# ai4colonoscopy/PraNet-V2

Hardware: AMD Instinct MI355X
Metric: images/sec (train fwd+bwd) at 352x352 bs=32/GPU (higher is better)
Workload: dtype bf16; 1 GPU; PraNet-V2 Res2Net50 training step (fwd+4x structure_loss+bwd+clamp+Adam), bs=32/GPU 352x352, random-init, synthetic ellipse masks; global_batch=32, parallelism=dp1, launch=hipGraph replay

## Files before the change

### include/pn2.h

```cpp
#ifndef PN2_H
#define PN2_H
#ifdef __cplusplus
extern "C" {
#endif

#define PN2_F32 0
#define PN2_BF16 1
#define PN2_F32F 2
#define PN2_F32X3 3
#define PN2_CONV_STATS 1
#define PN2_CONV_ACCUM 2
#define PN2_CONV_SPLITK(n) ((n) << 16)
#define PN2_CONV_ROWGATE 8
#define PN2_CONV_AFFINE 16
#define PN2_CONV_RELU 32
#define PN2_CONV_RELU6 64
#define PN2_CONV_BIAS 4

typedef struct pn2_conv_desc {
    int N, H, W;
    int OH, OW;
    int Cin_p, ld_in;
    int Cout, ld_out;
    int KH, KW, stride, pad_h, pad_w, dil_h, dil_w;
    int transposed;
    int Kp;
    int flags;
} pn2_conv_desc;

typedef struct pn2_wgrad_desc {
    int N, H, W, OH, OW;
    int Cin_p, ld_x;
    int Cout_p, ld_dy;
    int KH, KW, stride, pad_h, pad_w, dil_h, dil_w;
    int Rp, Kp;
    int tune;
} pn2_wgrad_desc;

typedef struct pn2_pack_desc {
    int Cout, Cin, KH, KW;
    int Cout_p, gw_out, gwp_out;
    int Cin_p, gw_in, gwp_in;
    int Rp, Kp;
    int transposed;
    int ld, koff;
} pn2_pack_desc;

int pn2_conv_tile_n(int cout);
int pn2_wgrad_tile_co(int cout_p);
int pn2_conv_tile_m(int m, int cout, int dtype);
int pn2_conv_stat_blocks(int m, int cout, int dtype);
int pn2_conv_gemm(int dtype, const void* in, const void* wp, void* out, float* psum, float* psq, const pn2_conv_desc* d, void* stream);
#define PN2_BNB_STATS 1
#define PN2_BNB_MASK_RAW 2
#define PN2_BNB_MASK_Y 4
#define PN2_BNB_STORE_MASKED 8
int pn2_conv_gemm_gated(int dtype, const void* in, const void* wp, void* out, float* psum, float* psq, const pn2_conv_desc* d, const float* gate, void* stream);
int pn2_conv_gemm_affine(int dtype, const void* in, const void* wp, void* out, const float* scale, const float* shift, const void* res, int ld_res,
                         const pn2_conv_desc* d, void* stream);
typedef struct pn2_bnb_target {
    void* out; int ld_out;
    int mode;
    const void* raw; int ld_raw;
    const void* y; int ld_y;
    const float* par; int ps;
    int split;
    const void* raw2; const float* par2;
    float* p1; float* p2; int ldp;
} pn2_bnb_target;
typedef struct pn2_conv_ep { pn2_bnb_target a, b; const void* pool; int ld_pool; int pad_; pn2_bnb_target c; } pn2_conv_ep;
int pn2_conv_gemm_ep(int dtype, const void* in, const void* wp, void* out, const pn2_conv_desc* d, const pn2_conv_ep* ep, void* stream);
typedef struct pn2_conv_job { const void* in; const void* wp; void* out; float* psum; float* psq; pn2_conv_desc d; int pad_; pn2_conv_ep ep; } pn2_conv_job;
int pn2_conv_gemm_tile(int dtype, const pn2_conv_desc* d);
int pn2_conv_gemm_job_blocks(int dtype, const pn2_conv_job* j, int bm, int bn);
int pn2_conv_gemm_multi(int dtype, int bm, int bn, int ep, const pn2_conv_job* jobs_dev, const int* block_start_dev, int njobs, int total_blocks, void* stream);
int pn2_conv_splitk_reduce(int dtype, const float* ws, int ksplit, int M, int Cout, void* out, int ld_out, const float* bias, float* psum, float* psq,
                           int accumulate, void* stream);
int pn2_conv_wgrad(int dtype, const void* dy, const void* x, float* slab, const pn2_wgrad_desc* d, int nsplit, void* stream);
typedef struct pn2_wgrad_job { const void* dy; const void* x; float* slab; pn2_wgrad_desc d; int nsplit;
    int rot;
} pn2_wgrad_job;
int pn2_conv_wgrad_variant(int dtype, const pn2_wgrad_desc* d);
int pn2_conv_wgrad_blocks(const pn2_wgrad_desc* d, int nsplit);
int pn2_conv_wgrad_multi(int dtype, int variant, const pn2_wgrad_job* jobs_dev, const int* block_start_dev, int njobs, int total_blocks, void* stream);
int pn2_pack_weight(int dtype, const float* w_oihw, void* wp, const pn2_pack_desc* p, void* stream);
int pn2_wgrad_reduce(const float* slab, float* gw_oihw, const pn2_pack_desc* p, int nsplit, int accumulate, void* stream);
int pn2_pack_patch_weight(int dtype, const float* w_oihw, void* wp, int Cout, int Cin, int KH, int KW, int Cin_p, int Rp, int Kp, void* stream);
int pn2_depth_to_space(int dtype, const void* t, int ld_t, void* dx, int ld_dx, int N, int H, int W, int OH, int OW, int S, int C, int accumulate, void* stream);
int pn2_conv_dgrad_small_cin(int dtype, const void* dy, int ld_dy, const float* w_oihw, void* dx, int ld_dx, int N, int H, int W, int OH, int OW,
                             int Cout, int Cin, int KH, int KW, int stride, int pad, int accumulate, void* stream);
typedef struct pn2_pack_job { const float* w; void* wp; pn2_pack_desc d; } pn2_pack_job;
int pn2_pack_blocks(const pn2_pack_desc* p);
int pn2_pack_weights_multi(int dtype, const pn2_pack_job* jobs_dev, const int* block_start_dev, int njobs, int total_blocks, void* stream);
typedef struct pn2_reduce_job { const float* slab; float* gw; pn2_pack_desc d; int nsplit; int accumulate; } pn2_reduce_job;
int pn2_wgrad_reduce_blocks(const pn2_pack_desc* p);
int pn2_wgrad_reduce_multi(const pn2_reduce_job* jobs_dev, const int* block_start_dev, int njobs, int total_blocks, void* stream);

typedef struct pn2_bn_desc {
    int M;
    int Cp;
    int C, gw, gwp;
    float eps, momentum;
    int ldp;
    int tile_rows;
} pn2_bn_desc;
int pn2_bn_finalize(const float* psum, const float* psq, int nblk, const pn2_bn_desc* d, const float* gamma, const float* beta,
                    float* running_mean, float* running_var, float* scale, float* shift, float* mean, float* invstd, void* stream);
int pn2_bn_eval_prepare(const pn2_bn_desc* d, const float* gamma, const float* beta, const float* running_mean, const float* running_var,
                        float* scale, float* shift, void* stream);
typedef struct pn2_bnprep_job { const float* gamma; const float* beta; const float* running_mean; const float* running_var; float* scale; float* shift; pn2_bn_desc d; int pad_; } pn2_bnprep_job;
int pn2_bn_eval_prepare_multi(const pn2_bnprep_job* jobs_dev, const int* block_start_dev, int njobs, int total_blocks, void* stream);
int pn2_affine_act(int dt_in, const void* x, int ld_x, int dt_out, void* y, int ld_y, int M, int Cout,
                   const float* scale, const float* shift, const void* res, int ld_res, int relu, void* stream);
int pn2_affine_act_sum(int dt, const void* x, int ld_x, void* y, int ld_y, int M, int C, const float* scale, const float* shift, int relu,
                       const void* add, int ld_add, void* y2, int ld_y2, void* stream);
int pn2_affine_act_tee(int dt, const void* x, int ld_x, void* y, int ld_y, int M, int C, const float* scale, const float* shift, int relu,
                       void* y3, int ld_y3, int c_lo, void* stream);
int pn2_bn_relu_maxpool_fwd(int dt, const void* raw, int ld_raw, const float* scale, const float* shift, void* y, int ld_y, unsigned char* idx,
                            int N, int H, int W, int C, int OH, int OW, void* stream);
int pn2_pool_bn_bwd_reduce(int dt, const void* dpool, int ld_dp, const unsigned char* idx, const void* raw, int ld_raw, int N, int H, int W, int C, int OH, int OW,
                           const float* mean, const float* invstd, const float* mask_scale, const float* mask_shift, float* p1, float* p2, int nblk, void* stream);
int pn2_pool_bn_bwd_apply(int dt, const void* dpool, int ld_dp, const unsigned char* idx, const void* raw, int ld_raw, int N, int H, int W, int C, int OH, int OW,
                          const float* mean, const float* invstd, const float* coef, const float* mask_scale, const float* mask_shift, void* dz, int ld_dz, void* stream);
int pn2_bn_bwd_reduce(int dt, int dt_dy, const void* dy, int ld_dy, int Cdy, const void* y, int ld_y, int dt_y, const void* x, int ld_x,
                      int M, int Cp, const float* mean, const float* invstd, float* p1, float* p2, int nblk,
                      const float* mask_scale, const float* mask_shift, int relu6, void* stream);
int pn2_bn_bwd_blocks(int M, int Cp, int dtype);
int pn2_bn_bwd_finalize(const float* p1, const float* p2, int nblk, const pn2_bn_desc* d, const float* gamma, const float* invstd,
                        float* dgamma, float* dbeta, int accumulate, float* coef, void* stream);
typedef struct pn2_bn_segs { int nseg; int c0[4]; int nblk[4]; int ldp[4]; const float* p1[4]; const float* p2[4]; } pn2_bn_segs;
int pn2_bn_bwd_finalize_seg(const pn2_bn_segs* segs, const pn2_bn_desc* d, const float* gamma, const float* invstd,
                            float* dgamma, float* dbeta, int accumulate, float* coef, void* stream);
typedef struct pn2_bnfin_job { const float* psum; const float* psq; const float* gamma; const float* beta; float* running_mean; float* running_var;
                               float* scale; float* shift; float* mean; float* invstd; pn2_bn_desc d; int nblk; int cpb; int pad_; } pn2_bnfin_job;
int pn2_bn_finalize_job_blocks(pn2_bnfin_job* j);
int pn2_bn_finalize_multi(const pn2_bnfin_job* jobs_dev, const int* block_start_dev, int njobs, int total_blocks, void* stream);
typedef struct pn2_affine_job { const void* x; void* y; const float* scale; const float* shift; const void* res; const void* add; void* y2;
                                int ld_x, ld_y, ld_res, ld_add, ld_y2, M, C, relu, rows_per_blk, cvp; } pn2_affine_job;
int pn2_affine_job_blocks(int dt, pn2_affine_job* j);
int pn2_affine_multi(int dt, const pn2_affine_job* jobs_dev, const int* block_start_dev, int njobs, int total_blocks, void* stream);
typedef struct pn2_bnbfin_job { pn2_bn_segs sg; const float* gamma; const float* invstd; float* dgamma; float* dbeta; float* coef; pn2_bn_desc d;
                                int accumulate; int cpb; int pad_; } pn2_bnbfin_job;
int pn2_bn_bwd_finalize_job_blocks(pn2_bnbfin_job* j);
int pn2_bn_bwd_finalize_multi(const pn2_bnbfin_job* jobs_dev, const int* block_start_dev, int njobs, int total_blocks, void* stream);
typedef struct pn2_bnapply_job { const void* dy; const void* y; const void* x; const float* mean; const float* invstd; const float* coef; void* dx; void* dres;
                                 const float* msc; const float* msh; int ld_dy, ld_y, ld_x, ld_dx, ld_dres, M, Cp, dres_accum, r6, rows_per_blk, cvp, pad_; } pn2_bnapply_job;
int pn2_bn_bwd_apply_job_blocks(int dt, pn2_bnapply_job* j);
#define PN2_MULTI_F32DY 0x200
#define PN2_MULTI_F32OUT 0x200
#define PN2_MULTI_LEAN 0x100
int pn2_bn_bwd_apply_multi(int dt, const pn2_bnapply_job* jobs_dev, const int* block_start_dev, int njobs, int total_blocks, void* stream);
typedef struct pn2_bnreduce_job { const void* dy; const void* y; const void* x; const float* mean; const float* invstd; float* p1; float* p2;
                                  const float* msc; const float* msh; int ld_dy, ld_y, ld_x, M, Cp, nblk, rows_per_blk, cvp, r6, pad_; } pn2_bnreduce_job;
int pn2_bn_bwd_reduce_job_blocks(int dt, pn2_bnreduce_job* j);
int pn2_bn_bwd_reduce_multi(int dt, const pn2_bnreduce_job* jobs_dev, const int* block_start_dev, int njobs, int total_blocks, void* stream);
int pn2_bn_bwd_apply(int dt, int dt_dy, const void* dy, int ld_dy, int Cdy, const void* y, int ld_y, int dt_y, const void* x, int ld_x,
                     int M, int Cp, const float* mean, const float* invstd, const float* coef, void* dx, int ld_dx,
                     void* dres, int ld_dres, int dres_accum, const float* mask_scale, const float* mask_shift, int relu6, void* stream);

int pn2_maxpool3x3s2_fwd(int dt, const void* x, int ld_x, void* y, int ld_y, unsigned char* idx, int N, int H, int W, int C, int OH, int OW, void* stream);
int pn2_maxpool3x3s2_bwd(int dt, const void* dy, int ld_dy, const unsigned char* idx, void* dx, int ld_dx, int N, int H, int W, int C, int OH, int OW, void* stream);
int pn2_avgpool_fwd(int dt, const void* x, int ld_x, void* y, int ld_y, int N, int H, int W, int C, int OH, int OW,
                    int k, int stride, int pad, int count_include_pad, void* stream);
int pn2_avgpool_bwd(int dt, const void* dy, int ld_dy, void* dx, int ld_dx, int N, int H, int W, int C, int OH, int OW,
                    int k, int stride, int pad, int count_include_pad, int accumulate, void* stream);

int pn2_bilinear_fwd(int dt, const void* x, int ld_x, void* y, int ld_y, int N, int H, int W, int C, int OH, int OW,
                     int align_corners, float rh, float rw, void* stream);
int pn2_bilinear_bwd(int dt, const void* dy, int ld_dy, void* dx, int ld_dx, int N, int H, int W, int C, int OH, int OW,
                     int align_corners, float rh, float rw, int accumulate, void* stream);

int pn2_dsra_fuse_fwd(const float* fg, const float* crop_fg, const float* crop_bg, float* out, int M, int K, int use_softmax, void* stream);
int pn2_dsra_fuse_bwd(const float* fg, const float* crop_fg, const float* crop_bg, const float* dout, float* dfg, float* dcrop_fg,
                      float* dcrop_bg, int M, int K, int use_softmax, void* stream);
int pn2_ra_gate_fwd(int dt, const void* x, int ld_x, const float* crop, void* out, int ld_out, int M, int C, void* stream);
int pn2_ra_gate_bwd(int dt, const void* x, int ld_x, const float* crop, const void* dout, int ld_dout, void* dx, int ld_dx, int dx_accum,
                    float* dcrop, int M, int C, void* stream);
int pn2_ra_gate_post_bwd(int dt, const void* raw, int ld_raw, const float* crop, const void* dz, int ld_dz, void* dzg, int ld_dzg, float* dcrop,
                         int M, int C, void* stream);

int pn2_loss_weights(const float* mask, float* weit, int N, int H, int W, int ksize, void* stream);
int pn2_loss_weights_clear(const float* mask, float* weit, int N, int H, int W, int ksize, long long* clear, int nclear, void* stream);
int pn2_loss_blocks(int HW);
int pn2_structure_loss_fwd(const float* preds, long long map_stride, int P, const float* mask, const float* weit, float* partial,
                           float* sums, float* wsum, float* loss, int N, int HW, void* stream);
int pn2_structure_loss_bwd(const float* preds, float* dpreds, long long map_stride, int P, const float* mask, const float* weit,
                           const float* wsum, const float* sums, float gscale, int N, int HW, void* stream);
int pn2_structure_loss_bwd_dev(const float* preds, float* dpreds, long long map_stride, long long dmap_stride, int P, const float* mask, const float* weit,
                               const float* wsum, const float* sums, const float* gscale_dev, float gscale, int N, int HW, void* stream);

#define PN2_TAIL_MAX_MAPS 16
typedef struct pn2_tail_map {
    const float* src;
    float* dsrc;
    int h, w;
    float rh, rw;
    int accumulate;
    int pad_;
} pn2_tail_map;
typedef struct pn2_tail_desc {
    int N, OH, OW, P, align_corners, pad_;
    pn2_tail_map maps[PN2_TAIL_MAX_MAPS];
} pn2_tail_desc;
int pn2_dsra_tail_blocks(int OH);
int pn2_dsra_tail_fwd(const pn2_tail_desc* d, float* lat, const float* mask, const float* weit, float* partial,
                      float* sums, float* wsum, float* loss, void* stream);
int pn2_dsra_tail_scratch(const pn2_tail_desc* d);
int pn2_dsra_tail_bwd(const pn2_tail_desc* d, const float* mask, const float* weit, const float* wsum, const float* sums,
                      float gscale, float* scratch, long long scratch_floats, void* stream);
int pn2_dsra_tail_fused_ok(const pn2_tail_desc* d);
int pn2_dsra_tail_fused_scratch(const pn2_tail_desc* d);
int pn2_dsra_tail_fwd_bwd(const pn2_tail_desc* d, float* lat, const float* mask, const float* weit, float* partial, float* sums, float* wsum,
                          float* per, float* loss, float gscale, float* scratch, long long scratch_floats, long long* isum, void* stream);

int pn2_layernorm_fwd(int dt, const void* x, int ld_x, void* y, int ld_y, int M, int C, const float* gamma, const float* beta, float eps,
                      float* mean, float* rstd, void* stream);
int pn2_ln_slots(int dt, int C);
int pn2_rows_blocks(int M, int unit);
int pn2_layernorm_bwd(int dt, const void* dy, int ld_dy, const void* x, int ld_x, int M, int C, const float* gamma, const float* mean, const float* rstd,
                      void* dx, int ld_dx, int accumulate_dx, float* pg, float* pb, int nblk, void* stream);
int pn2_colsum_unit(int dt, int C);
int pn2_colsum(int dt, const void* dy, int ld, int M, int C, float* partial, int nblk, void* stream);
int pn2_colsum_finalize(const float* partial, int nblk, int C, int ld, float* out, int accumulate, void* stream);
typedef struct pn2_colsum_in_job { const void* dy; float* partial; int ld, M, C, rows, cvp, pad_; } pn2_colsum_in_job;
int pn2_colsum_job_blocks(int dt, pn2_colsum_in_job* job);
int pn2_colsum_multi(int dt, const pn2_colsum_in_job* jobs_dev, const int* block_start_dev, int njobs, int total_blocks, void* stream);
typedef struct pn2_colsum_job { const float* partial; float* out; int nblk, C, ld, accumulate; } pn2_colsum_job;
int pn2_colsum_finalize_blocks(int C);
int pn2_colsum_finalize_multi(const pn2_colsum_job* jobs_dev, const int* block_start_dev, int njobs, int total_blocks, void* stream);
int pn2_dwconv3x3(int dt, const void* x, const float* w, const float* b, void* z, void* y_gelu, int N, int H, int W, int C, int flip, int accumulate, void* stream);
int pn2_dwconv3x3_colsum_blocks(int dt, int N, int H, int W, int C);
int pn2_dwconv3x3_colsum(int dt, const void* x, const float* w, const float* b, void* z, int N, int H, int W, int C, int flip, float* cpart, int nblk, void* stream);
int pn2_gelu_bwd(int dt, const void* dy, const void* z, void* dz, long long n, void* stream);
int pn2_dwconv3x3_wgrad_blocks(int dt, int N, int H, int W, int C);
int pn2_dwconv3x3_wgrad(int dt, const void* dz, const void* x, float* partial, int nblk, int N, int H, int W, int C, const void* zpre, void* dz_out, void* stream);
int pn2_scale_samples(int dt, const void* x, void* y, const float* scale, const void* res, int N, long long per_sample, void* stream);
int pn2_attn_fwd(int dt, const void* q, int ld_q, const void* kv, int ld_kv, void* out, int ld_o, float* lse, int B, int Nq, int Nkv, int heads, int head_dim,
                 float scale, void* stream);
int pn2_attn_bwd_blocks(int dt, int B, int heads, int Nq);
int pn2_attn_bwd(int dt, const void* q, int ld_q, const void* kv, int ld_kv, const void* out, int ld_o, const void* dout, int ld_do, const float* lse, void* dq, int ld_dq,
                 void* dkv, int ld_dkv, float* partial, float* delta, int B, int Nq, int Nkv, int heads, int head_dim, float scale, void* stream);

int pn2_dwconv_blocks(int dt, int N, int H, int W, int C, int K, int wgrad);
int pn2_dwconv(int dt, const void* x, const float* w, void* z, int N, int H, int W, int C, int K, int flip, int accumulate, float* psum, float* psq, void* stream);
int pn2_dwconv_wgrad(int dt, const void* dz, const void* x, float* partial, int N, int H, int W, int C, int K, void* stream);
int pn2_pairconv_blocks(int dt, int N, int H, int W, int F);
int pn2_pairconv3x3_fwd(int dt, const void* x, const float* w, void* z, int N, int H, int W, int F, float* psum, float* psq, void* stream);
int pn2_pairconv3x3_dgrad(int dt, const void* dz, const float* w, void* dx, int N, int H, int W, int F, int accumulate, void* stream);
int pn2_pairconv3x3_wgrad(int dt, const void* dz, const void* x, float* partial, int N, int H, int W, int F, void* stream);
// ... 64 lines not shown
```

### pranet-v2_amd/csrc/pn2_common.h

```cpp
#pragma once
#include <hip/hip_runtime.h>
#include <stdint.h>
#include <type_traits>
#include "../../include/pn2.h"

typedef unsigned short bf16_t;
typedef __attribute__((ext_vector_type(8))) short bf16x8_t;
typedef __attribute__((ext_vector_type(4))) short s16x4_t;
typedef __attribute__((ext_vector_type(4))) float f32x4_t;
typedef __attribute__((ext_vector_type(4))) double f64x4_t;

struct f32f_t { float v; };
struct f32x3_t { float v; };

__device__ __forceinline__ float bf2f(bf16_t h) { return __uint_as_float(((unsigned)h) << 16); }
__device__ __forceinline__ bf16_t f2bf(float f) {
    unsigned r;
    asm("v_cvt_pk_bf16_f32 %0, %1, %1" : "=v"(r) : "v"(f));
    return (bf16_t)r;
}

template <typename T> struct TT;
template <> struct TT<float> {
    static constexpr int VEC = 4;
    static constexpr int DT = PN2_F32;
    __device__ static __forceinline__ float ld(const float* p) { return *p; }
    __device__ static __forceinline__ void st(float* p, float v) { *p = v; }
    __device__ static __forceinline__ float round(float v) { return v; }
    __device__ static __forceinline__ void unpack(const uint4& v, float* f) {
        f[0] = __uint_as_float(v.x); f[1] = __uint_as_float(v.y); f[2] = __uint_as_float(v.z); f[3] = __uint_as_float(v.w);
    }
    __device__ static __forceinline__ uint4 pack(const float* f) {
        return make_uint4(__float_as_uint(f[0]), __float_as_uint(f[1]), __float_as_uint(f[2]), __float_as_uint(f[3]));
    }
};
template <> struct TT<f32f_t> : TT<float> {
    static constexpr int DT = PN2_F32F;
    __device__ static __forceinline__ float ld(const f32f_t* p) { return p->v; }
    __device__ static __forceinline__ void st(f32f_t* p, float v) { p->v = v; }
};
template <> struct TT<f32x3_t> : TT<float> {
    static constexpr int DT = PN2_F32X3;
    __device__ static __forceinline__ float ld(const f32x3_t* p) { return p->v; }
    __device__ static __forceinline__ void st(f32x3_t* p, float v) { p->v = v; }
};
template <> struct TT<bf16_t> {
    static constexpr int VEC = 8;
    static constexpr int DT = PN2_BF16;
    __device__ static __forceinline__ float ld(const bf16_t* p) { return bf2f(*p); }
    __device__ static __forceinline__ void st(bf16_t* p, float v) { *p = f2bf(v); }
    __device__ static __forceinline__ float round(float v) { return bf2f(f2bf(v)); }
    __device__ static __forceinline__ void unpack(const uint4& v, float* f) {
        f[0] = __uint_as_float(v.x << 16); f[1] = __uint_as_float(v.x & 0xffff0000u);
        f[2] = __uint_as_float(v.y << 16); f[3] = __uint_as_float(v.y & 0xffff0000u);
        f[4] = __uint_as_float(v.z << 16); f[5] = __uint_as_float(v.z & 0xffff0000u);
        f[6] = __uint_as_float(v.w << 16); f[7] = __uint_as_float(v.w & 0xffff0000u);
    }
    __device__ static __forceinline__ unsigned cvt2(float lo, float hi) {
        unsigned r;
        asm("v_cvt_pk_bf16_f32 %0, %1, %2" : "=v"(r) : "v"(lo), "v"(hi));
        return r;
    }
    __device__ static __forceinline__ uint4 pack(const float* f) {
        return make_uint4(cvt2(f[0], f[1]), cvt2(f[2], f[3]), cvt2(f[4], f[5]), cvt2(f[6], f[7]));
    }
};

__device__ __forceinline__ int phys2log(int p, int gw, int gwp, int C) {
    int g = p / gwp, o = p - g * gwp;
    int c = g * gw + o;
    return (o < gw && c < C) ? c : -1;
}

__device__ __forceinline__ int xcd_remap(int bid, int nblk) {
    const int q = nblk >> 3, r = nblk & 7, x = bid & 7;
    return (x < r ? x * (q + 1) : r * (q + 1) + (x - r) * q) + (bid >> 3);
}

__device__ __forceinline__ size_t divmod_idx(size_t idx, int d, int& rem) {
    if (idx >> 32) { const size_t q = idx / (size_t)d; rem = (int)(idx - q * (size_t)d); return q; }
    const unsigned i = (unsigned)idx, q = i / (unsigned)d;
    rem = (int)(i - q * (unsigned)d);
    return q;
}

__device__ __forceinline__ int find_job(const int* __restrict__ bstart, int njobs, int b) {
    int lo = 0, hi = njobs;
    while (hi - lo > 1) { const int mid = (lo + hi) >> 1; if (bstart[mid] <= b) lo = mid; else hi = mid; }
    return lo;
}

__device__ __forceinline__ float wave_sum(float v) {
#pragma unroll
    for (int o = 32; o > 0; o >>= 1) v += __shfl_xor(v, o);
    return v;
}

__device__ __forceinline__ void bl_src(int o, float r, int ac, int In, int& i0, int& i1, float& l0, float& l1) {
    float s = ac ? r * (float)o : fmaxf(r * ((float)o + 0.5f) - 0.5f, 0.f);
    i0 = (int)s; if (i0 > In - 1) i0 = In - 1;
    i1 = i0 + (i0 < In - 1 ? 1 : 0);
    l1 = s - (float)i0; l0 = 1.f - l1;
}

__device__ __forceinline__ void bl_range(int i, float r, int ac, int On, int& lo, int& hi) {
    float a, b;
    if (ac) { if (r <= 0.f) { lo = 0; hi = On - 1; return; } a = ((float)i - 1.f) / r; b = ((float)i + 1.f) / r; }
    else { a = ((float)i - 0.5f) / r - 0.5f; b = ((float)i + 1.5f) / r - 0.5f; }
    lo = (int)floorf(a) - 1; hi = (int)ceilf(b) + 1;
    if (lo < 0) lo = 0; if (hi > On - 1) hi = On - 1;
}

#define PN2_CHECK_LAUNCH() do { hipError_t e_ = hipGetLastError(); if (e_ != hipSuccess) return (int)e_; } while (0)

template <auto K>
inline void pn2_lds_opt_in(int lds_cap) {
    static bool done = false;
    if (!done) { (void)hipFuncSetAttribute(reinterpret_cast<const void*>(K), hipFuncAttributeMaxDynamicSharedMemorySize, lds_cap); done = true; }
}
template <auto K, typename... A>
inline int pn2_launch(dim3 grid, dim3 block, size_t lds, int lds_cap, hipStream_t st, const A&... args) {
    if (lds_cap > 64 * 1024) pn2_lds_opt_in<K>(lds_cap);
    hipLaunchKernelGGL(K, grid, block, lds, st, args...);
    PN2_CHECK_LAUNCH();
    return 0;
}

template <typename T> struct Ty { using type = T; };
template <typename X> using type_of = typename X::type;
template <int N> using Int = std::integral_constant<int, N>;
template <bool B> using Bool = std::integral_constant<bool, B>;
template <typename F>
int with_dtype(int dtype, F f) {
    if (dtype == PN2_BF16) return f(Ty<bf16_t>{});
    if (dtype == PN2_F32) return f(Ty<float>{});
    if (dtype == PN2_F32F) return f(Ty<f32f_t>{});
    if (dtype == PN2_F32X3) return f(Ty<f32x3_t>{});
    return -3;
}
template <typename F>
int with_storage_dtype(int dtype, F f) {
    if (dtype == PN2_BF16) return f(Ty<bf16_t>{});
    if (dtype == PN2_F32) return f(Ty<float>{});
    return -3;
}
template <typename F>
int with_dtype_pair(int dt, int dt_g, F f) {
    if (dt == PN2_BF16 && dt_g == PN2_BF16) return f(Ty<bf16_t>{}, Ty<bf16_t>{});
    if (dt == PN2_BF16 && dt_g == PN2_F32) return f(Ty<bf16_t>{}, Ty<float>{});
    if (dt == PN2_F32 && dt_g == PN2_F32) return f(Ty<float>{}, Ty<float>{});
    return -3;
}
inline int vec_of(int dt) { return dt == PN2_F32 ? 4 : 8; }
inline int pow2ceil(int v) { int p = 1; while (p < v) p <<= 1; return p; }
inline void rows_walk_geometry(int M, int CV, int min_mult, int max_mult, int& cvp, int& rows_per_blk, int& nblk) {
    cvp = pow2ceil(CV); if (cvp > 256) cvp = 256;
    const int R = 256 / cvp;
    constexpr int target = 1024;
    const int want = (M + target - 1) / target;
    rows_per_blk = ((want + R - 1) / R) * R;
    if (rows_per_blk < min_mult * R) rows_per_blk = min_mult * R;
    if (max_mult > 0 && rows_per_blk > max_mult * R) rows_per_blk = max_mult * R;
    nblk = (M + rows_per_blk - 1) / rows_per_blk;
}
inline bool table_ok(const void* jobs_dev, const int* block_start_dev, int njobs, int total_blocks) { return jobs_dev && block_start_dev && njobs >= 1 && total_blocks >= 1; }
namespace pn2_host {
inline int grid_for(size_t total, int cap) { size_t g = (total + 255) / 256; return (int)(g > (size_t)cap ? cap : (g < 1 ? 1 : g)); }
}
```

### pranet-v2_amd/csrc/pn2_conv.hip

```cpp
#include <cstring>
#include "pn2_common.h"
#include "../../include/pn2.h"

namespace {

constexpr int ROWB = 128;
constexpr int KSUB = ROWB / 64;
constexpr int RS = ROWB;

#ifdef PN2_STAMP
constexpr int PN2_STAMP_SLOTS = 16, PN2_STAMP_BLOCKS = 1 << 16;
__device__ unsigned long long pn2_stamp_buf[PN2_STAMP_BLOCKS * PN2_STAMP_SLOTS];
__device__ __forceinline__ void pn2_stamp(int i) {
    if (threadIdx.x == 0 && blockIdx.y == 0 && blockIdx.x < PN2_STAMP_BLOCKS) pn2_stamp_buf[blockIdx.x * PN2_STAMP_SLOTS + i] = __builtin_amdgcn_s_memtime();
}
__device__ __forceinline__ void pn2_stamp_hw() {
    if (threadIdx.x == 0 && blockIdx.y == 0 && blockIdx.x < PN2_STAMP_BLOCKS) {
        pn2_stamp_buf[blockIdx.x * PN2_STAMP_SLOTS + 10] = __builtin_amdgcn_s_getreg((31 << 11) | 4);
        pn2_stamp_buf[blockIdx.x * PN2_STAMP_SLOTS + 11] = __builtin_amdgcn_s_getreg((31 << 11) | 20);
    }
}
#define PN2_STAMP_AT(i) pn2_stamp(i)
#else
#define PN2_STAMP_AT(i)
// ... 1659 lines not shown
            xm[i] += PX;                                                                                               \
            __builtin_amdgcn_raw_ptr_buffer_load_lds(rs_x, (lptr_t)(sb_ + PX * RBY + (i * 256 + wch) * 16), 16, (int)vo_, 0, 0, 0); \
        }                                                                                                              \
    } while (0)

    f32x4_t acc[MT][NT];
#pragma unroll
    for (int i = 0; i < MT; ++i)
#pragma unroll
        for (int j = 0; j < NT; ++j) acc[i][j] = f32x4_t{0.f, 0.f, 0.f, 0.f};

    const unsigned lds0 = (unsigned)(size_t)(lptr_t)smem;
    const int prow = g * 4 + (l15 >> 2);
    const int keyy = (prow & KMY) << 1, keyx = (prow & KMX) << 1;
    unsigned offA[MT], offB[NT];
#pragma unroll
    for (int i = 0; i < MT; ++i) offA[i] = prow * RBY + ((((wm * WTM) >> 3) + i * 2 + ((l15 & 3) >> 1)) ^ keyy) * 16 + (l15 & 1) * 8;
#pragma unroll
    for (int j = 0; j < NT; ++j) offB[j] = PX * RBY + prow * RBX + ((((wn * WTN) >> 3) + j * 2 + ((l15 & 3) >> 1)) ^ keyx) * 16 + (l15 & 1) * 8;

    if (nsteps > 0) {
        PN2_WISSUE(s_begin, 0);
        if (nsteps > 1) PN2_WISSUE(s_begin + 1, 1);
        for (int t = 0; t < nsteps; ++t) {
            if (t + 1 < nsteps) asm volatile("s_waitcnt vmcnt(%0)" ::"n"(LPS) : "memory");
            else asm volatile("s_waitcnt vmcnt(0)" ::: "memory");
            __builtin_amdgcn_s_barrier();
            if (t + 2 < nsteps) {
                const int nb_ = (t + 2) % NS;
                PN2_WISSUE(s_begin + t + 2, nb_);
            }
            const unsigned sb = lds0 + (t % NS) * STAGE;
#pragma unroll
            for (int ks = 0; ks < PX / 32; ++ks) {
                u32x2_t a0[MT], a1[MT], b0[NT], b1[NT];
#pragma unroll
                for (int i = 0; i < MT; ++i) {
                    asm volatile("ds_read_b64_tr_b16 %0, %1" : "=v"(a0[i]) : "v"(sb + offA[i] + ks * 32 * RBY));
                    asm volatile("ds_read_b64_tr_b16 %0, %1" : "=v"(a1[i]) : "v"(sb + offA[i] + (ks * 32 + 16) * RBY));
                }
#pragma unroll
                for (int j = 0; j < NT; ++j) {
                    asm volatile("ds_read_b64_tr_b16 %0, %1" : "=v"(b0[j]) : "v"(sb + offB[j] + ks * 32 * RBX));
                    asm volatile("ds_read_b64_tr_b16 %0, %1" : "=v"(b1[j]) : "v"(sb + offB[j] + (ks * 32 + 16) * RBX));
                }
                asm volatile("s_waitcnt lgkmcnt(0)" ::: "memory");
                __builtin_amdgcn_sched_barrier(0);
#pragma unroll
                for (int i = 0; i < MT; ++i)
#pragma unroll
                    for (int j = 0; j < NT; ++j)
                        MMA<bf16_t>::run(acc[i][j], make_uint4(a0[i].x, a0[i].y, a1[i].x, a1[i].y), make_uint4(b0[j].x, b0[j].y, b1[j].x, b1[j].y));
            }
        }
    }
#undef PN2_WISSUE
    float* dst = slab + ((size_t)split * d.Rp + co0) * d.Kp + k0;
#pragma unroll
    for (int i = 0; i < MT; ++i)
#pragma unroll
        for (int j = 0; j < NT; ++j) {
            if (BNK > 128 && k0 + wn * WTN + j * 16 >= d.Kp) continue;
#pragma unroll
            for (int r = 0; r < 4; ++r)
                dst[(size_t)(wm * WTM + i * 16 + g * 4 + r) * d.Kp + wn * WTN + j * 16 + l15] = acc[i][j][r];
        }
}

template <typename T, int BMC, int BNK, int WM, int WN, bool PW>
__global__ __launch_bounds__(256) void conv_wgrad(const T* __restrict__ dy, const T* __restrict__ x, float* __restrict__ slab, pn2_wgrad_desc d, int nsplit) {
    conv_wgrad_body<T, BMC, BNK, WM, WN, PW>(dy, x, slab, d, nsplit, blockIdx.x);
}
template <typename T, int BMC, int BNK, int WM, int WN, bool PW>
__global__ __launch_bounds__(256) void conv_wgrad_tab(const pn2_wgrad_job* __restrict__ jobs, const int* __restrict__ bstart, int njobs) {
    const int total = bstart[njobs];
    for (int b = blockIdx.x; b < total; b += gridDim.x) {
        const int jb = find_job(bstart, njobs, b);
        const pn2_wgrad_job j = jobs[jb];
        const int bl = b - bstart[jb];
        conv_wgrad_body<T, BMC, BNK, WM, WN, PW>((const T*)j.dy, (const T*)j.x, j.slab, j.d, j.nsplit, (bl & ~7) | ((bl - j.rot) & 7));
        __syncthreads();
    }
}
template <int BMC, int WM, int WN, bool PW, int BNK = 128>
__global__ __launch_bounds__(256) void conv_wgrad_dma(const bf16_t* __restrict__ dy, const bf16_t* __restrict__ x, float* __restrict__ slab, pn2_wgrad_desc d, int nsplit) {
    conv_wgrad_dma_body<BMC, WM, WN, PW, BNK>(dy, x, slab, d, nsplit, blockIdx.x);
}
template <int BMC, int WM, int WN, bool PW, int BNK = 128>
__global__ __launch_bounds__(256) void conv_wgrad_dma_tab(const pn2_wgrad_job* __restrict__ jobs, const int* __restrict__ bstart, int njobs) {
    const int total = bstart[njobs];
    for (int b = blockIdx.x; b < total; b += gridDim.x) {
        const int jb = find_job(bstart, njobs, b);
        const pn2_wgrad_job j = jobs[jb];
        const int bl = b - bstart[jb];
        conv_wgrad_dma_body<BMC, WM, WN, PW, BNK>((const bf16_t*)j.dy, (const bf16_t*)j.x, j.slab, j.d, j.nsplit, (bl & ~7) | ((bl - j.rot) & 7));
        __syncthreads();
    }
}

template <int BMC, int WM, int WN, int BNK>
__global__ __launch_bounds__(256, 2) void conv_wgrad_dma_tab_mix(const pn2_wgrad_job* __restrict__ jobs, const int* __restrict__ bstart, int njobs) {
    const int total = bstart[njobs];
    for (int b = blockIdx.x; b < total; b += gridDim.x) {
        const int jb = find_job(bstart, njobs, b);
        const pn2_wgrad_job j = jobs[jb];
        const int bl = b - bstart[jb];
        const int lb = (bl & ~7) | ((bl - j.rot) & 7);
        if (j.d.KH == 1 && j.d.KW == 1 && j.d.stride == 1 && j.d.pad_h == 0 && j.d.pad_w == 0)
            conv_wgrad_dma_body<BMC, WM, WN, true, BNK>((const bf16_t*)j.dy, (const bf16_t*)j.x, j.slab, j.d, j.nsplit, lb);
        else
            conv_wgrad_dma_body<BMC, WM, WN, false, BNK>((const bf16_t*)j.dy, (const bf16_t*)j.x, j.slab, j.d, j.nsplit, lb);
        __syncthreads();
    }
}

template <typename T>
__global__ void pack_weight(const float* __restrict__ w, T* __restrict__ wp, pn2_pack_desc p) {
    const size_t total = (size_t)p.Rp * p.Kp;
    for (size_t idx = (size_t)blockIdx.x * blockDim.x + threadIdx.x; idx < total; idx += (size_t)gridDim.x * blockDim.x) {
        const int row = (int)(idx / p.Kp), k = (int)(idx - (size_t)row * p.Kp);
        const int taps = p.KH * p.KW;
        const int cg = p.transposed ? p.Cout_p : p.Cin_p;
        const int tap = k / cg, c = k - tap * cg;
        float v = 0.f;
        if (tap < taps) {
            int co, ci;
            if (!p.transposed) {
                co = row < p.Cout_p ? phys2log(row, p.gw_out, p.gwp_out, p.Cout) : -1;
                ci = phys2log(c, p.gw_in, p.gwp_in, p.Cin);
            } else {
                ci = row < p.Cin_p ? phys2log(row, p.gw_in, p.gwp_in, p.Cin) : -1;
                co = phys2log(c, p.gw_out, p.gwp_out, p.Cout);
            }
            if (co >= 0 && ci >= 0) v = w[((size_t)co * p.Cin + ci) * taps + tap];
        }
        TT<T>::st(wp + (size_t)row * (p.ld ? p.ld : p.Kp) + p.koff + k, v);
    }
}

__host__ __device__ inline int log2phys(int c, int gw, int gwp) { const int g = c / gw; return g * gwp + (c - g * gw); }

__host__ __device__ inline void pack_tile(int taps, int& CO, int& CI) {
    if (taps == 1) { CO = 64; CI = 64; }
    else if (taps <= 7) { CO = 32; CI = 32; }
    else if (taps <= 9) { CO = 16; CI = 32; }
    else if (taps <= 25) { CO = 16; CI = 16; }
    else { CO = 4; CI = 8; }
}
inline int pack_blocks(const pn2_pack_desc& p) {
    int CO, CI; pack_tile(p.KH * p.KW, CO, CI);
    return ((p.Cout + CO - 1) / CO) * ((p.Cin + CI - 1) / CI);
}

template <typename T>
__global__ __launch_bounds__(256) void pack_weight_multi(const pn2_pack_job* __restrict__ jobs, const int* __restrict__ bstart, int njobs) {
    __shared__ float tile[7296];
    const int jb = find_job(bstart, njobs, blockIdx.x);
    const pn2_pack_job j = jobs[jb];
    const pn2_pack_desc p = j.d;
    const float* __restrict__ w = j.w;
    T* __restrict__ wp = reinterpret_cast<T*>(j.wp);
    const int taps = p.KH * p.KW;
    int CO, CI; pack_tile(taps, CO, CI);
    const int local = blockIdx.x - bstart[jb];
    const int nci = (p.Cin + CI - 1) / CI;
    const int co0 = (local / nci) * CO, ci0 = (local - (local / nci) * nci) * CI;
    const int nco_t = min(CO, p.Cout - co0), nci_t = min(CI, p.Cin - ci0);
    const int run = nci_t * taps, rs = CI * taps + 1;
    const int tx = threadIdx.x & 63, ty = threadIdx.x >> 6;
    for (int col = ty; col < nco_t; col += 4) {
        const float* src = w + ((size_t)(co0 + col) * p.Cin + ci0) * taps;
        for (int r = tx; r < run; r += 64) tile[col * rs + r] = src[r];
    }
    __syncthreads();
    const size_t ld = p.ld ? p.ld : p.Kp;
    const float inv_gi = 1.f / (float)p.gw_in, inv_go = 1.f / (float)p.gw_out;
    auto phys_in = [&](int c) { const int g = (int)(((float)c + 0.5f) * inv_gi); return g * p.gwp_in + (c - g * p.gw_in); };
    auto phys_out = [&](int c) { const int g = (int)(((float)c + 0.5f) * inv_go); return g * p.gwp_out + (c - g * p.gw_out); };
    if (!p.transposed) {
        const int sh = 31 - __clz(CI);
        for (int col = ty; col < nco_t; col += 4) {
            T* dst = wp + (size_t)phys_out(co0 + col) * ld + p.koff;
            for (int cb = tx; cb < taps * CI; cb += 64) {
                const int tap = cb >> sh, cil = cb & (CI - 1);
                if (cil < nci_t) TT<T>::st(dst + tap * p.Cin_p + phys_in(ci0 + cil), tile[col * rs + cil * taps + tap]);
            }
        }
    } else {
        const int sh = 31 - __clz(CO);
        for (int cil = ty; cil < nci_t; cil += 4) {
            T* dst = wp + (size_t)phys_in(ci0 + cil) * ld + p.koff;
            for (int cb = tx; cb < taps * CO; cb += 64) {
                const int tap = cb >> sh, col = cb & (CO - 1);
                if (col < nco_t) TT<T>::st(dst + tap * p.Cout_p + phys_out(co0 + col), tile[col * rs + cil * taps + tap]);
            }
        }
    }
}

__device__ __forceinline__ void wgrad_reduce_body(const float* __restrict__ slab, float* __restrict__ gw, const pn2_pack_desc& p, int nsplit, int accumulate,
                                                  int blk, int nblk) {
    const int taps = p.KH * p.KW;
    const int ktot = taps * p.Cin_p;
    const int kv = ktot >> 2;
    const size_t total = (size_t)p.Cout_p * kv;
    const size_t sstride = (size_t)p.Rp * p.Kp;
    int S = 1;
    while (S < 16 && total * S < 32768 && 2 * S <= nsplit) S <<= 1;
    const int EPW = 64 / S;
    const int lane = threadIdx.x & 63, wave = threadIdx.x >> 6;
    const int sub = lane / EPW, ei = lane - sub * EPW;
    const size_t nwaves = (size_t)nblk * 4;
    for (size_t base = ((size_t)blk * 4 + wave) * EPW; base < total; base += nwaves * EPW) {
        const size_t idx = base + ei;
        const bool live = idx < total;
        const size_t ii = live ? idx : 0;
        const int prow = (int)(ii / kv), k = (int)(ii - (size_t)prow * kv) << 2;
        const float* s = slab + (size_t)prow * p.Kp + k;
        float4 v0 = make_float4(0.f, 0.f, 0.f, 0.f), v1 = v0, v2 = v0, v3 = v0;
        int i = sub;
        for (; i + 3 * S < nsplit; i += 4 * S) {
            const float4 a0 = *reinterpret_cast<const float4*>(s + (size_t)i * sstride), a1 = *reinterpret_cast<const float4*>(s + (size_t)(i + S) * sstride);
            const float4 a2 = *reinterpret_cast<const float4*>(s + (size_t)(i + 2 * S) * sstride), a3 = *reinterpret_cast<const float4*>(s + (size_t)(i + 3 * S) * sstride);
            v0.x += a0.x; v0.y += a0.y; v0.z += a0.z; v0.w += a0.w; v1.x += a1.x; v1.y += a1.y; v1.z += a1.z; v1.w += a1.w;
            v2.x += a2.x; v2.y += a2.y; v2.z += a2.z; v2.w += a2.w; v3.x += a3.x; v3.y += a3.y; v3.z += a3.z; v3.w += a3.w;
        }
        for (; i < nsplit; i += S) { const float4 a0 = *reinterpret_cast<const float4*>(s + (size_t)i * sstride); v0.x += a0.x; v0.y += a0.y; v0.z += a0.z; v0.w += a0.w; }
        float v[4] = {(v0.x + v1.x) + (v2.x + v3.x), (v0.y + v1.y) + (v2.y + v3.y), (v0.z + v1.z) + (v2.z + v3.z), (v0.w + v1.w) + (v2.w + v3.w)};
        for (int off = EPW; off < 64; off <<= 1) {
#pragma unroll
            for (int e = 0; e < 4; ++e) v[e] += __shfl_xor(v[e], off);
        }
        if (sub == 0 && live) {
            const int tap = k / p.Cin_p, pc = k - tap * p.Cin_p;
            const int co = phys2log(prow, p.gw_out, p.gwp_out, p.Cout);
            if (co >= 0) {
#pragma unroll
                for (int e = 0; e < 4; ++e) {
                    const int ci = phys2log(pc + e, p.gw_in, p.gwp_in, p.Cin);
                    if (ci >= 0) {
                        float* d = gw + ((size_t)co * p.Cin + ci) * taps + tap;
                        *d = accumulate ? *d + v[e] : v[e];
                    }
                }
            }
        }
    }
}

__global__ __launch_bounds__(256) void wgrad_reduce_unpack(const float* __restrict__ slab, float* __restrict__ gw, pn2_pack_desc p, int nsplit, int accumulate) {
    wgrad_reduce_body(slab, gw, p, nsplit, accumulate, blockIdx.x, gridDim.x);
}

__global__ __launch_bounds__(256) void wgrad_reduce_multi(const pn2_reduce_job* __restrict__ jobs, const int* __restrict__ bstart, int njobs) {
    const int jb = find_job(bstart, njobs, blockIdx.x);
    const pn2_reduce_job j = jobs[jb];
    wgrad_reduce_body(j.slab, j.gw, j.d, j.nsplit, j.accumulate, blockIdx.x - bstart[jb], bstart[jb + 1] - bstart[jb]);
}

inline int reduce_blocks(const pn2_pack_desc& p) {
    const size_t nthr = (size_t)p.Cout_p * p.Cin_p * p.KH * p.KW * 4;
    const size_t b = (nthr + 255) / 256;
    return (int)(b > 2048 ? 2048 : (b < 1 ? 1 : b));
}

constexpr int TUNE_KS2 = 0x40, TUNE_KS4 = 0x80;
constexpr int TILE_KS2 = 0x100;
inline int conv_tune(const pn2_conv_desc& d) { return (d.flags >> 8) & 0xff; }
inline int conv_ksplit(const pn2_conv_desc& d) { return (d.flags >> 16) & 15; }
inline bool conv_desc_ok(const pn2_conv_desc& d) {
    return !(d.Cin_p % 8 || d.ld_in % 8 || d.Kp % 128 || (d.stride != 1 && d.stride != 2 && d.stride != 4 && d.stride != 8));
}
template <typename D> inline bool is_pointwise(const D& d) { return d.KH == 1 && d.KW == 1 && d.stride == 1 && d.pad_h == 0 && d.pad_w == 0; }
inline int conv_grid(const pn2_conv_desc& d, int bm, int bn) { return ((d.N * d.OH * d.OW + bm - 1) / bm) * ((d.Cout + bn - 1) / bn); }

template <int BM, int BN>
inline int ep2_lds(const pn2_conv_desc& d, const pn2_conv_ep& ep) {
    bool stat_a, y_a, acc, stat_b;
    ep2_needs(d, ep, stat_a, y_a, acc, stat_b);
    return ep2_layout<BM, BN>(stat_a, y_a, acc, stat_b, ep2_stat_c(ep)).total;
}
template <int BM, int BN>
inline int ep2_lds(int bits) {
    if (!(bits & 15)) bits = 15;
    return ep2_layout<BM, BN>(bits & 1, bits & 2, bits & 4, bits & 8).total;
}
template <typename T, int BM, int BN, int WM>
struct ConvLds {
    static constexpr int stage = (BM + BN) * 128;
    static constexpr int gather = 2 * (BM + BN) * (RS + lo_row<T>);
    static constexpr int epi = BM * (BN * (int)sizeof(T) + 16) + 3 * WM * BN * 4;
    static constexpr int xch(int ks) { return (ks - 1) * BM * BN * 4; }
    static constexpr bool E2 = sizeof(T) == 2 && ep2_tile(BM, BN);
    template <bool EP, typename... Need>
    static int with_ep(int lds, const Need&... need) {
        if constexpr (EP && E2) { const int e2 = ep2_lds<BM, BN>(need...); return e2 > lds ? e2 : lds; }
        else if constexpr (EP) return lds < ep_lds_bytes(TT<T>::VEC) ? ep_lds_bytes(TT<T>::VEC) : lds;
        else return lds;
    }
};
constexpr int LDS_MAX = 160 * 1024;
constexpr int imax(int a, int b) { return a > b ? a : b; }

template <typename T, int BM, int BN, int WM, int WN, bool EP>
int launch_gemm(const void* in, const void* wp, void* out, float* psum, float* psq, const pn2_conv_desc& d, const pn2_conv_ep& ep, hipStream_t st) {
    using L = ConvLds<T, BM, BN, WM>;
    const int lds = L::template with_ep<EP>(imax(L::gather, L::epi), d, ep);
    if (lds > LDS_MAX) return -4;
    const int cap = EP && L::E2 ? LDS_MAX : lds;
    const dim3 grid(conv_grid(d, BM, BN));
    if (is_pointwise(d)) return pn2_launch<conv_gather_gemm<T, BM, BN, WM, WN, true, EP>>(grid, dim3(256), lds, cap, st, (const T*)in, (const T*)wp, (T*)out, psum, psq, d, ep);
    return pn2_launch<conv_gather_gemm<T, BM, BN, WM, WN, false, EP>>(grid, dim3(256), lds, cap, st, (const T*)in, (const T*)wp, (T*)out, psum, psq, d, ep);
}

template <bool EP, int BM, int BN, int WM, int WN, int NS = 3>
int launch_dma(const void* in, const void* wp, void* out, float* psum, float* psq, const pn2_conv_desc& d, const pn2_conv_ep& ep, hipStream_t st) {
    using L = ConvLds<bf16_t, BM, BN, WM>;
    const int ksteps = (d.KH * d.KW * d.Cin_p + 63) / 64;
    const int lds = L::template with_ep<EP>(imax((ksteps < NS ? ksteps : NS) * L::stage, L::epi), d, ep);
    if (lds > LDS_MAX) return -4;
    constexpr int cap = EP && L::E2 ? LDS_MAX : imax(NS * L::stage, L::epi);
    const int ksplit = conv_ksplit(d);
    const dim3 grid(conv_grid(d, BM, BN), ksplit > 1 ? ksplit : 1);
    if (is_pointwise(d)) return pn2_launch<conv_dma_gemm<BM, BN, WM, WN, true, NS, EP>>(grid, dim3(256), lds, cap, st, (const bf16_t*)in, (const bf16_t*)wp, (bf16_t*)out, psum, psq, d, ep);
    return pn2_launch<conv_dma_gemm<BM, BN, WM, WN, false, NS, EP>>(grid, dim3(256), lds, cap, st, (const bf16_t*)in, (const bf16_t*)wp, (bf16_t*)out, psum, psq, d, ep);
}

template <bool EP, int BM, int BN, int WM, int WN, int NS, int KS>
int launch_dma_ks(const void* in, const void* wp, void* out, float* psum, float* psq, const pn2_conv_desc& d, const pn2_conv_ep& ep, hipStream_t st) {
    using L = ConvLds<bf16_t, BM, BN, WM>;
    static_assert(KS * NS * L::stage <= LDS_MAX && L::xch(KS) <= LDS_MAX, "tile does not fit");
    const int lds = L::template with_ep<EP>(imax(imax(KS * NS * L::stage, L::epi), L::xch(KS)), d, ep);
    if (lds > LDS_MAX || conv_ksplit(d) > 1) return -4;
    const dim3 grid(conv_grid(d, BM, BN));
    if (is_pointwise(d)) return pn2_launch<conv_dma_gemm_ks<BM, BN, WM, WN, true, NS, EP, KS>>(grid, dim3(256 * KS), lds, LDS_MAX, st, (const bf16_t*)in, (const bf16_t*)wp, (bf16_t*)out, psum, psq, d, ep);
    return pn2_launch<conv_dma_gemm_ks<BM, BN, WM, WN, false, NS, EP, KS>>(grid, dim3(256 * KS), lds, LDS_MAX, st, (const bf16_t*)in, (const bf16_t*)wp, (bf16_t*)out, psum, psq, d, ep);
}

inline bool dma_extent_ok(const pn2_conv_desc& d) {
    return ((size_t)d.N * d.H * d.W - 1) * (size_t)d.ld_in * 2 + (size_t)d.Cin_p * 2 < 0x80000000ull;
}
inline void pick_tiles(int M, int cout, bool f32, int& bm, int& bn) {
    bn = pn2_conv_tile_n(cout);
    if (f32 && bn == 128) bn = 64;
    bm = 128;
    auto blocks = [&]() { return ((M + bm - 1) / bm) * ((cout + bn - 1) / bn); };
    if (blocks() < 384) bm = 64;
    if (blocks() < 256 && bn == 128) bn = 64;
    if (blocks() < 160 && bn == 64 && cout > 32) bn = 32;
}

template <int BM_, int BN_, int WM_, int WN_> struct Tile { static constexpr int BM = BM_, BN = BN_, WM = WM_, WN = WN_; };
template <typename F>
int with_tile(int bm, int bn, F f) {
    if (bm == 128 && bn == 128) return f(Tile<128, 128, 2, 2>{});
    if (bm == 128 && bn == 64) return f(Tile<128, 64, 2, 2>{});
    if (bm == 128 && bn == 32) return f(Tile<128, 32, 4, 1>{});
    if (bm == 64 && bn == 128) return f(Tile<64, 128, 2, 2>{});
    if (bm == 64 && bn == 64) return f(Tile<64, 64, 2, 2>{});
    if (bm == 64 && bn == 32) return f(Tile<64, 32, 4, 1>{});
    return -2;
}
template <typename F>
int with_wgrad_tile(int bmc, F f) {
    if (bmc == 128) return f(Tile<128, 0, 2, 2>{});
    if (bmc == 64) return f(Tile<64, 0, 2, 2>{});
    if (bmc == 32) return f(Tile<32, 0, 1, 4>{});
    return -2;
}

template <typename T, int BMC, int WM, int WN>
int launch_wgrad(const void* dy, const void* x, float* slab, const pn2_wgrad_desc& d, int nsplit, hipStream_t st) {
    constexpr int BNK = 128;
    constexpr int lds = 2 * wg_stage_bytes<T>(BMC, BNK), cap = X3<T> ? lds : 0;
    const dim3 grid(8 * ((nsplit + 7) / 8) * (d.Rp / BMC) * (d.Kp / BNK));
    if (is_pointwise(d)) return pn2_launch<conv_wgrad<T, BMC, BNK, WM, WN, true>>(grid, dim3(256), lds, cap, st, (const T*)dy, (const T*)x, slab, d, nsplit);
    return pn2_launch<conv_wgrad<T, BMC, BNK, WM, WN, false>>(grid, dim3(256), lds, cap, st, (const T*)dy, (const T*)x, slab, d, nsplit);
}

template <typename T>
void gemm_select(const pn2_conv_desc& d, int& kern, int& bm, int& bn) {
    pick_tiles(d.N * d.OH * d.OW, d.Cout, sizeof(T) == 4, bm, bn);
    const int tune = (sizeof(T) == 2 || !MMA<T>::F64ROWS) ? conv_tune(d) : 0;
    const int tk_ = dma_extent_ok(d) ? (tune & 3) : 1, tbm = (tune >> 2) & 3, tbn = (tune >> 4) & 3;
    if (tbm) bm = tbm == 1 ? 64 : 128;
    if (tbn) bn = tbn == 1 ? 32 : (tbn == 2 ? 64 : 128);
    kern = 0;
    if (sizeof(T) == 2) kern = tk_ == 3 ? 3 : ((tk_ ? tk_ == 2 : true) ? 2 : 0);
    if (sizeof(T) == 4 && bn == 128) bn = 64;
}

template <typename T, bool EP>
int gemm_dispatch(const void* in, const void* wp, void* out, float* psum, float* psq, const pn2_conv_desc& d, const pn2_conv_ep& ep, hipStream_t st) {
    int kern, bm, bn;
    gemm_select<T>(d, kern, bm, bn);
    return with_tile(bm, bn, [&](auto tile) {
        using L = decltype(tile);
        constexpr int BM = L::BM, BN = L::BN, WM = L::WM, WN = L::WN;
        if constexpr (sizeof(T) == 2) {
            const int ks = kern >= 2 ? conv_tune(d) & (TUNE_KS2 | TUNE_KS4) : 0;
            if constexpr (BM == 64 && BN == 64) {
                if (ks & TUNE_KS4) return launch_dma_ks<EP, 64, 64, 2, 2, 2, 4>(in, wp, out, psum, psq, d, ep, st);
            }
            if constexpr (BN >= 64) {
                if ((ks & TUNE_KS2) && kern == 3) return launch_dma_ks<EP, BM, BN, WM, WN, 2, 2>(in, wp, out, psum, psq, d, ep, st);
                if constexpr (BM == 128 && BN == 128) { if (ks & TUNE_KS2) return -4; }
                else if (ks & TUNE_KS2) return launch_dma_ks<EP, BM, BN, WM, WN, 3, 2>(in, wp, out, psum, psq, d, ep, st);
            }
            if (kern == 3) return launch_dma<EP, BM, BN, WM, WN, 2>(in, wp, out, psum, psq, d, ep, st);
            if (kern == 2) return launch_dma<EP, BM, BN, WM, WN>(in, wp, out, psum, psq, d, ep, st);
        }
        if constexpr (BN == 128 && MMA<T>::F64ROWS) return -2;
        else return launch_gemm<T, BM, BN, WM, WN, EP>(in, wp, out, psum, psq, d, ep, st);
    });
}

template <bool EP, int BM, int BN, int WM, int WN>
int launch_dma_tab(const pn2_conv_job* jobs, const int* bstart, int njobs, int total, int bits, hipStream_t st) {
// ... 318 lines not shown
int pn2_conv_gemm_affine(int dtype, const void* in, const void* wp, void* out, const float* scale, const float* shift, const void* res, int ld_res, const pn2_conv_desc* d,
                         void* stream) {
    if (!d || !scale || !shift) return -1;
    if (!(d->flags & PN2_CONV_AFFINE) || (d->flags & (PN2_CONV_STATS | PN2_CONV_BIAS | PN2_CONV_ACCUM | PN2_CONV_ROWGATE)) || conv_ksplit(*d) > 1) return -2;
    const int vec_ = dtype == PN2_BF16 ? 8 : 4;
    if (res && (d->Cout % vec_ || d->ld_out % vec_ || ld_res % vec_)) return -2;
    pn2_conv_ep ep;
    memset(&ep, 0, sizeof(ep));
    ep.a.y = res; ep.a.ld_y = ld_res;
    if (!in || !wp || !out) return -1;
    if (!conv_desc_ok(*d)) return -2;
    return with_dtype(dtype, [&](auto ty) {
        return gemm_dispatch<typename decltype(ty)::type, false>(in, wp, out, const_cast<float*>(scale), const_cast<float*>(shift), *d, ep, (hipStream_t)stream);
    });
}

int pn2_conv_gemm_gated(int dtype, const void* in, const void* wp, void* out, float* psum, float* psq, const pn2_conv_desc* d, const float* gate, void* stream) {
    if (!d || !gate) return -1;
    pn2_conv_desc dg = *d;
    dg.flags |= PN2_CONV_ROWGATE;
    pn2_conv_ep ep;
    memset(&ep, 0, sizeof(ep));
    ep.a.par = gate;
    return conv_gemm_impl(dtype, in, wp, out, psum, psq, &dg, ep, stream);
}

int pn2_conv_gemm_ep(int dtype, const void* in, const void* wp, void* out, const pn2_conv_desc* d, const pn2_conv_ep* ep, void* stream) {
    if (!d || !ep) return -1;
    const int vec = dtype == PN2_BF16 ? 8 : 4;
    if ((d->flags & (PN2_CONV_STATS | PN2_CONV_BIAS)) || conv_ksplit(*d) > 1) return -2;
    if (d->Cout % vec || d->ld_out % vec) return -2;
    if (ep->c.mode) {
        if (dtype != PN2_BF16 || ep->c.mode != PN2_BNB_STATS || !(ep->a.mode & PN2_BNB_STATS) || ep->b.out || ep->c.split) return -2;
        if (!ep->c.raw || !ep->c.par || !ep->c.p1 || !ep->c.p2 || ep->c.ldp < 1 || ep->c.ld_raw % vec || ep->c.ps < 1) return -1;
        int kern_, bm_, bn_;
        gemm_select<bf16_t>(*d, kern_, bm_, bn_);
        if (!ep2_tile(bm_, bn_)) return -2;
    }
    if (ep->pool && (!(d->flags & PN2_CONV_ACCUM) || !(ep->a.mode & PN2_BNB_STATS) || ep->b.out || (d->OH & 1) || (d->OW & 1) || ep->ld_pool % vec || ep->ld_pool < d->Cout)) return -2;
    int rc = bnb_check(ep->a, vec, false);
    if (rc) return rc;
    rc = bnb_check(ep->b, vec, true);
    if (rc) return rc;
    return conv_gemm_impl(dtype, in, wp, out, nullptr, nullptr, d, *ep, stream);
}

int pn2_conv_gemm_tile(int dtype, const pn2_conv_desc* d) {
    if (!d) return -1;
    if (!conv_desc_ok(*d)) return -2;
    if (conv_ksplit(*d) > 1) return -2;
    const int ksb = conv_tune(*d) & (TUNE_KS2 | TUNE_KS4);
    if (ksb & TUNE_KS4) return -2;
    int kern, bm, bn;
    const int rc = with_dtype(dtype, [&](auto ty) {
        using T = typename decltype(ty)::type;
        gemm_select<T>(*d, kern, bm, bn);
        return sizeof(T) == 2 && !dma_extent_ok(*d) ? -2 : 0;
    });
    if (rc) return rc;
    if (ksb) {
        if (dtype != PN2_BF16 || bn < 64 || (bm == 128 && bn == 128)) return -2;
        return ((bm | TILE_KS2) << 8) | bn;
    }
    return (bm << 8) | bn;
}

int pn2_conv_gemm_job_blocks(int dtype, const pn2_conv_job* j, int bm, int bn) {
    bm &= 0xff;
    if (!j || !j->in || !j->wp || !j->out || bm < 1 || bn < 1) return -1;
    const pn2_conv_desc& d = j->d;
    if ((d.flags & PN2_CONV_STATS) && (!j->psum || !j->psq)) return -1;
    if ((d.flags & PN2_CONV_BIAS) && !j->psum) return -1;
    if (d.flags & PN2_CONV_AFFINE) {
        const int v_ = dtype == PN2_BF16 ? 8 : 4;
        if (!j->psum || !j->psq || (d.flags & (PN2_CONV_STATS | PN2_CONV_BIAS | PN2_CONV_ACCUM | PN2_CONV_ROWGATE)) || j->ep.a.mode || j->ep.b.mode || j->ep.b.out) return -1;
        if (j->ep.a.y && (d.Cout % v_ || d.ld_out % v_ || j->ep.a.ld_y % v_)) return -2;
    }
    const bool use_ep = (j->ep.a.mode | j->ep.b.mode) != 0 || j->ep.b.out != nullptr;
    const int vec = dtype == PN2_BF16 ? 8 : 4;
    if (use_ep && (d.Cout % vec || d.ld_out % vec || (d.flags & (PN2_CONV_STATS | PN2_CONV_BIAS)))) return -2;
    return ((d.N * d.OH * d.OW + bm - 1) / bm) * ((d.Cout + bn - 1) / bn);
}

int pn2_conv_gemm_multi(int dtype, int bm, int bn, int ep, const pn2_conv_job* jobs_dev, const int* block_start_dev, int njobs, int total_blocks, void* stream) {
    if (!jobs_dev || !block_start_dev || njobs < 1 || total_blocks < 1) return -1;
    return (ep & 1) ? gemm_multi_dispatch<true>(dtype, bm, bn, ep >> 1, jobs_dev, block_start_dev, njobs, total_blocks, (hipStream_t)stream)
                    : gemm_multi_dispatch<false>(dtype, bm, bn, 0, jobs_dev, block_start_dev, njobs, total_blocks, (hipStream_t)stream);
}

int pn2_conv_wgrad(int dtype, const void* dy, const void* x, float* slab, const pn2_wgrad_desc* d, int nsplit, void* stream) {
    if (!dy || !x || !slab || !d || nsplit < 1) return -1;
    if (d->Cin_p % 8 || d->ld_x % 8 || d->ld_dy % 8 || d->Cout_p % 8) return -2;
    if (dtype != PN2_BF16 && d->tune >= 2) return -2;
    return with_dtype(dtype, [&](auto ty) { return wgrad_dispatch<typename decltype(ty)::type>(dy, x, slab, *d, nsplit, (hipStream_t)stream); });
}

int pn2_conv_wgrad_variant(int dtype, const pn2_wgrad_desc* d) {
    if (!d) return -1;
    return with_dtype(dtype, [&](auto ty) { return sizeof(typename decltype(ty)::type) == 2 ? wgrad_variant<bf16_t>(*d) : wgrad_variant<float>(*d); });
}

int pn2_conv_wgrad_blocks(const pn2_wgrad_desc* d, int nsplit) {
    if (!d || nsplit < 1) return -1;
    const int bmc = pn2_wgrad_tile_co(d->Cout_p);
    if (d->Rp % bmc || d->Kp % 128) return -2;
    return wgrad_blocks_t<bf16_t>(*d, nsplit);
}

int pn2_conv_wgrad_multi(int dtype, int variant, const pn2_wgrad_job* jobs_dev, const int* block_start_dev, int njobs, int total_blocks, void* stream) {
    if (!jobs_dev || !block_start_dev || njobs < 1 || total_blocks < 1 || variant < 0 || variant >= 15) return -1;
    return with_dtype(dtype, [&](auto ty) { return wgrad_multi_dispatch<typename decltype(ty)::type>(variant, jobs_dev, block_start_dev, njobs, total_blocks, (hipStream_t)stream); });
}

int pn2_pack_weight(int dtype, const float* w, void* wp, const pn2_pack_desc* p, void* stream) {
    if (!w || !wp || !p) return -1;
    const size_t total = (size_t)p->Rp * p->Kp;
    const int grid = (int)((total + 255) / 256 > 4096 ? 4096 : (total + 255) / 256);
    if (dtype == PN2_BF16) hipLaunchKernelGGL(pack_weight<bf16_t>, dim3(grid), dim3(256), 0, (hipStream_t)stream, w, (bf16_t*)wp, *p);
    else if (dtype == PN2_F32) hipLaunchKernelGGL(pack_weight<float>, dim3(grid), dim3(256), 0, (hipStream_t)stream, w, (float*)wp, *p);
    else return -3;
    PN2_CHECK_LAUNCH();
    return 0;
}

int pn2_pack_blocks(const pn2_pack_desc* p) { return (p && p->KH * p->KW <= 225) ? pack_blocks(*p) : -1; }

int pn2_pack_weights_multi(int dtype, const pn2_pack_job* jobs_dev, const int* block_start_dev, int njobs, int total_blocks, void* stream) {
    if (!jobs_dev || !block_start_dev || njobs < 1 || total_blocks < 1) return -1;
    if (dtype == PN2_BF16) hipLaunchKernelGGL(pack_weight_multi<bf16_t>, dim3(total_blocks), dim3(256), 0, (hipStream_t)stream, jobs_dev, block_start_dev, njobs);
    else if (dtype == PN2_F32) hipLaunchKernelGGL(pack_weight_multi<float>, dim3(total_blocks), dim3(256), 0, (hipStream_t)stream, jobs_dev, block_start_dev, njobs);
    else return -3;
    PN2_CHECK_LAUNCH();
    return 0;
}

int pn2_wgrad_reduce(const float* slab, float* gw, const pn2_pack_desc* p, int nsplit, int accumulate, void* stream) {
    if (!slab || !gw || !p) return -1;
    const int grid = reduce_blocks(*p);
    hipLaunchKernelGGL(wgrad_reduce_unpack, dim3(grid), dim3(256), 0, (hipStream_t)stream, slab, gw, *p, nsplit, accumulate);
    PN2_CHECK_LAUNCH();
    return 0;
}

int pn2_wgrad_reduce_blocks(const pn2_pack_desc* p) { return p ? reduce_blocks(*p) : -1; }

int pn2_wgrad_reduce_multi(const pn2_reduce_job* jobs_dev, const int* block_start_dev, int njobs, int total_blocks, void* stream) {
    if (!jobs_dev || !block_start_dev || njobs < 1 || total_blocks < 1) return -1;
    hipLaunchKernelGGL(wgrad_reduce_multi, dim3(total_blocks), dim3(256), 0, (hipStream_t)stream, jobs_dev, block_start_dev, njobs);
    PN2_CHECK_LAUNCH();
    return 0;
}


int pn2_pack_patch_weight(int dtype, const float* w_oihw, void* wp, int Cout, int Cin, int KH, int KW, int Cin_p, int Rp, int Kp, void* stream) {
    if (!w_oihw || !wp || Cin_p < Cin || Rp < KH * KW * Cin_p || Kp < Cout) return -1;
    const size_t total = (size_t)Rp * Kp;
    const unsigned grid = (unsigned)((total + 255) / 256 > 4096 ? 4096 : (total + 255) / 256);
    if (dtype == PN2_BF16) hipLaunchKernelGGL(pack_patch_k<bf16_t>, dim3(grid), dim3(256), 0, (hipStream_t)stream, w_oihw, (bf16_t*)wp, Cout, Cin, KH, KW, Cin_p, Rp, Kp);
    else if (dtype == PN2_F32) hipLaunchKernelGGL(pack_patch_k<float>, dim3(grid), dim3(256), 0, (hipStream_t)stream, w_oihw, (float*)wp, Cout, Cin, KH, KW, Cin_p, Rp, Kp);
    else return -3;
    PN2_CHECK_LAUNCH();
    return 0;
}

int pn2_depth_to_space(int dtype, const void* t, int ld_t, void* dx, int ld_dx, int N, int H, int W, int OH, int OW, int S, int C, int accumulate, void* stream) {
    if (!t || !dx || N < 1 || S < 1) return -1;
    const int V = dtype == PN2_F32 ? 4 : 8;
    if (C % V || ld_t % V || ld_dx % V || OH * S > H || OW * S > W) return -2;
    const size_t total = (size_t)N * H * W * (C / V);
    const unsigned grid = (unsigned)((total + 255) / 256 > 16384 ? 16384 : (total + 255) / 256);
    if (dtype == PN2_BF16) hipLaunchKernelGGL(depth_to_space_k<bf16_t>, dim3(grid), dim3(256), 0, (hipStream_t)stream, (const bf16_t*)t, ld_t, (bf16_t*)dx, ld_dx, N, H, W, OH, OW, S, C, accumulate);
    else if (dtype == PN2_F32) hipLaunchKernelGGL(depth_to_space_k<float>, dim3(grid), dim3(256), 0, (hipStream_t)stream, (const float*)t, ld_t, (float*)dx, ld_dx, N, H, W, OH, OW, S, C, accumulate);
    else return -3;
    PN2_CHECK_LAUNCH();
    return 0;
}


int pn2_conv_dgrad_small_cin(int dtype, const void* dy, int ld_dy, const float* w_oihw, void* dx, int ld_dx, int N, int H, int W, int OH, int OW,
                             int Cout, int Cin, int KH, int KW, int stride, int pad, int accumulate, void* stream) {
    if (!dy || !w_oihw || !dx || N < 1 || stride < 1) return -1;
    const int V = dtype == PN2_F32 ? 4 : 8;
    const size_t lds = (size_t)KH * KW * Cout * sizeof(float4);
    if (Cin < 1 || Cin > 4 || Cout % V || ld_dy % V || ld_dx % V || ld_dx < V || lds > 64 * 1024) return -2;
    const size_t M = (size_t)N * H * W;
    const int pix = 1024;
    const unsigned grid = (unsigned)((M + pix - 1) / pix);
    if (dtype == PN2_BF16) hipLaunchKernelGGL(dgrad_small_cin_k<bf16_t>, dim3(grid), dim3(256), lds, (hipStream_t)stream, (const bf16_t*)dy, ld_dy, w_oihw, (bf16_t*)dx, ld_dx,
                                              N, H, W, OH, OW, Cout, Cin, KH, KW, stride, pad, accumulate, pix);
    else if (dtype == PN2_F32) hipLaunchKernelGGL(dgrad_small_cin_k<float>, dim3(grid), dim3(256), lds, (hipStream_t)stream, (const float*)dy, ld_dy, w_oihw, (float*)dx, ld_dx,
                                                  N, H, W, OH, OW, Cout, Cin, KH, KW, stride, pad, accumulate, pix);
    else return -3;
    PN2_CHECK_LAUNCH();
    return 0;
}


int pn2_conv_splitk_reduce(int dtype, const float* ws, int ksplit, int M, int Cout, void* out, int ld_out, const float* bias, float* psum, float* psq, int accumulate,
                           void* stream) {
    if (!ws || !out || ksplit < 1 || M < 1 || Cout < 1 || ((psum == nullptr) != (psq == nullptr))) return -1;
    if (Cout % 4) return -2;
    int lanes = 1; while (lanes < Cout / 4 && lanes < 16) lanes <<= 1;
    if (dtype == PN2_BF16 && ld_out % 4) return -2;
    const dim3 grid((M + 63) / 64, (Cout / 4 + lanes - 1) / lanes);
    if (dtype == PN2_BF16) hipLaunchKernelGGL(splitk_reduce_k<bf16_t>, grid, dim3(256), 0, (hipStream_t)stream, ws, ksplit, M, Cout, (bf16_t*)out, ld_out, bias, psum, psq, accumulate, lanes);
    else if (dtype == PN2_F32) hipLaunchKernelGGL(splitk_reduce_k<float>, grid, dim3(256), 0, (hipStream_t)stream, ws, ksplit, M, Cout, (float*)out, ld_out, bias, psum, psq, accumulate, lanes);
    else return -3;
    PN2_CHECK_LAUNCH();
    return 0;
}

}

#ifdef PN2_STAMP
extern "C" int pn2_debug_stamps(unsigned long long* dst_host, int nblk) {
    if (nblk > PN2_STAMP_BLOCKS) nblk = PN2_STAMP_BLOCKS;
    return (int)hipMemcpyFromSymbol(dst_host, HIP_SYMBOL(pn2_stamp_buf), (size_t)nblk * PN2_STAMP_SLOTS * sizeof(unsigned long long));
}
#endif
```

### pranet-v2_amd/csrc/pn2_tail.hip

```cpp
#include "pn2_common.h"
#include "../../include/pn2.h"

namespace {

constexpr int MAXK = 32;
inline int grid_for(size_t total, int cap = 16384) { size_t g = (total + 255) / 256; return (int)(g > (size_t)cap ? cap : (g < 1 ? 1 : g)); }

__device__ __forceinline__ float sigmoidf_(float x) { return 1.f / (1.f + __expf(-x)); }

__global__ __launch_bounds__(256) void dsra_fwd_k(const float* __restrict__ fg, const float* __restrict__ cf, const float* __restrict__ cb,
                                                  float* __restrict__ out, int M, int K, int sm) {
    for (int m = blockIdx.x * 256 + threadIdx.x; m < M; m += gridDim.x * 256) {
        const size_t o = (size_t)m * K;
        if (sm) {
            float mx = -INFINITY;
            for (int k = 0; k < K; ++k) mx = fmaxf(mx, cf[o + k] - cb[o + k]);
            float e[MAXK], s = 0.f;
            for (int k = 0; k < K; ++k) { e[k] = expf(cf[o + k] - cb[o + k] - mx); s += e[k]; }
            for (int k = 0; k < K; ++k) { const float f = fg[o + k]; out[o + k] = f + f * (e[k] / s); }
        } else
            for (int k = 0; k < K; ++k) { const float f = fg[o + k]; out[o + k] = f + f * (cf[o + k] - cb[o + k]); }
    }
}

// ... 922 lines not shown
            const float a3 = row16_sum(A3.x + A3.y);
            if (rlead) red[p * 4 + 3][rrow] = a3;
        }
        __syncthreads();
        {
            const int mag = A.mag[p], nrows_ = A.shp[p] == p ? 18 : 12;
            if (mag == 8) tail_gather<2>(cc, sbt + p * TRB, R, RPT, LV, w, mag, nrows_, pb + A.poff[p]);
            else if (mag == 16) tail_gather<4>(cc, sbt + p * TRB, R, RPT, LV, w, mag, nrows_, pb + A.poff[p]);
            else tail_gather<8>(cc, sbt + p * TRB, R, RPT, LV, w, mag, nrows_, pb + A.poff[p]);
        }
        __syncthreads();
    }
    if (threadIdx.x < 5 * P) {
        const int p = threadIdx.x / 5, k = threadIdx.x - p * 5;
        auto tot = [&](int row) { float s_ = red[row][0]; for (int i = 1; i < nrow; ++i) s_ += red[row][i]; return s_; };
        const float HW_ = tot(4 * P), C1_ = tot(4 * P + 1), MW_ = HW_ - C1_;
        float val;
        if (k == 0) val = tot(p * 4);
        else if (k == 1) val = tot(p * 4 + 3);
        else if (k == 2) val = 0.5f * MW_ + (tot(p * 4 + 1) - tot(p * 4 + 2));
        else if (k == 3) val = (HW_ + 2.f * tot(p * 4 + 1)) + MW_;
        else val = 2.f * HW_;
        partial[(((size_t)p * d.N + n) * nb + band) * 5 + k] = val;
        if (isum) tail_isum_add(isum + (((size_t)p * d.N + n) * 5 + k) * 2, val);
    }
}

constexpr int TLB_MAXPN = 1024;
__device__ __forceinline__ void tail_loss_block(const pn2_tail_desc& d, const long long* __restrict__ isum, float* __restrict__ loss) {
    __shared__ float s_per[TLB_MAXPN], s_lp[8];
    const int P = d.P, N = d.N, PN = P * N;
    for (int pair = threadIdx.x; pair < PN; pair += 256) {
        const long long* a = isum + (size_t)pair * 10;
        const double a0 = tail_isum_get(a), a1 = tail_isum_get(a + 2), a2 = tail_isum_get(a + 4), a3 = tail_isum_get(a + 6), a4 = tail_isum_get(a + 8);
        const float wbce = (float)(a0 / a4), wbce2 = (float)(a1 / a4);
        const float wiou = 1.f - ((float)a2 + 1.f) / ((float)a3 - (float)a2 + 1.f);
        s_per[pair] = wbce + wiou + 0.8f * wbce2;
    }
    __syncthreads();
    if ((int)threadIdx.x < P) {
        const int p = threadIdx.x;
        float s_ = 0.f;
        for (int i = 0; i < N; ++i) s_ += s_per[p * N + i];
        s_lp[p] = s_ / (float)N; loss[p] = s_lp[p];
    }
    __syncthreads();
    if (threadIdx.x == 0) { float tot = 0.f; for (int k = 0; k < P; ++k) tot += s_lp[k]; loss[P] = tot; }
}

constexpr int TFI = 64;
__global__ __launch_bounds__(256) void tail_one_fin_k(pn2_tail_desc d, tail_one_aux A, const float* __restrict__ pbuf, const float* __restrict__ partial,
                                                      float gscale, float* __restrict__ sums_out, float* __restrict__ wsum_out, float* __restrict__ per, float* __restrict__ loss,
                                                      const long long* __restrict__ isum) {
    const int lossrow = (int)gridDim.y == 2 * d.P + 1 ? 1 : 0;
    if (lossrow && blockIdx.y == 0) {
        if (blockIdx.x == 0) tail_loss_block(d, isum, loss);
        return;
    }
    __shared__ double s_d[TFI * 5];
    const int j = (int)blockIdx.y - lossrow, P = d.P, p = j >= P ? j - P : j, nb = A.nb;
    const pn2_tail_map& mp = d.maps[j];
    const int h = mp.h, w = mp.w, hw_ = h * w, total = d.N * hw_;
    const int first = blockIdx.x * 256;
    if (first >= total) return;
    const int last = min(first + 255, total - 1), n0 = first / hw_, n1 = last / hw_, ni = n1 - n0 + 1;
    const int local = min(first + (int)threadIdx.x, total - 1);
    const int n = local / hw_, rem = local - n * hw_, y = rem / w, x = rem - y * w;
    float t1 = 0.f, t2 = 0.f, t3 = 0.f, th = 0.f, tc = 0.f;
    {
        int oy0, oy1;
        bl_range(y, mp.rh, 0, d.OH, oy0, oy1);
        for (int b = oy0 / TRB; b <= oy1 / TRB; ++b) {
            const int oyA = b * TRB, oyB = min(oyA + TRB - 1, d.OH - 1);
            int ylo, yhi, t; float u0, u1;
            bl_src(oyA, mp.rh, 0, h, ylo, t, u0, u1);
            bl_src(oyB, mp.rh, 0, h, t, yhi, u0, u1);
            if (y >= ylo && y <= yhi) {
                const float* bq = pbuf + ((size_t)n * nb + b) * A.ptot + (y - ylo) * w + x;
                const float* q = bq + A.poff[p]; const float* qs = bq + A.poff[A.shp[p]];
                const int cs = 3 * w;
                if (j < P) { t1 += q[0]; t2 += q[cs]; t3 += q[2 * cs]; th += qs[4 * cs]; } else t1 += q[3 * cs];
                tc += qs[5 * cs];
            }
        }
    }
    if (isum) {
        for (int c = threadIdx.x; c < 5 * ni; c += 256) s_d[c] = tail_isum_get(isum + (((size_t)p * d.N + n0) * 5 + c) * 2);
    } else {
        const int grp = threadIdx.x >> 4, l = threadIdx.x & 15;
        for (int c = grp; c < 5 * ni; c += 16) {
            const int i = c / 5, k = c - i * 5;
            const float* src = partial + ((size_t)p * d.N + (n0 + i)) * nb * 5 + k;
            double a = 0.0;
            for (int b0 = l; b0 < nb; b0 += 128) {
                float vv[8];
#pragma unroll
                for (int u = 0; u < 8; ++u) { const int b = b0 + 16 * u; vv[u] = b < nb ? src[(size_t)b * 5] : 0.f; }
#pragma unroll
                for (int u = 0; u < 8; ++u) a += (double)vv[u];
            }
            a += __shfl_xor(a, 8); a += __shfl_xor(a, 4); a += __shfl_xor(a, 2); a += __shfl_xor(a, 1);
            if (l == 0) s_d[c] = a;
        }
    }
    __syncthreads();
    if (j < P && (int)threadIdx.x < ni) {
        const int ni_ = n0 + threadIdx.x;
        if (ni_ * hw_ >= first) {
            const double* a = s_d + threadIdx.x * 5;
            float* so = sums_out + ((size_t)p * d.N + ni_) * 4;
            so[0] = (float)a[0]; so[1] = (float)a[1]; so[2] = (float)a[2]; so[3] = (float)a[3];
            if (p == 0) wsum_out[ni_] = (float)a[4];
            const float wbce = (float)(a[0] / a[4]), wbce2 = (float)(a[1] / a[4]);
            const float wiou = 1.f - ((float)a[2] + 1.f) / ((float)a[3] - (float)a[2] + 1.f);
            per[(size_t)p * d.N + ni_] = wbce + wiou + 0.8f * wbce2;
        }
    }
    if (first + (int)threadIdx.x >= total) return;
    const double* a = s_d + (n - n0) * 5;
    const float gs_ = gscale / (float)d.N, I = (float)a[2], U = (float)a[3], D = U - I + 1.f;
    const float gw = gs_ / (float)a[4], cA = gs_ * (I + 1.f) / (D * D), cB = gs_ / D;
    const float g = j < P ? gw * (2.f * t1 + tc) + cA * (0.5f * th - 2.f * t2) - (cA + cB) * (0.25f * (th - tc) - t2 + t3)
                          : 0.8f * gw * (2.f * t1 - tc);
    float* dst = mp.dsrc + local;
    *dst = mp.accumulate ? *dst + g : g;
}

__global__ void loss_total_k(const float* __restrict__ per, int P, int N, float* __restrict__ loss) {
    __shared__ float lp[8];
    const int p = threadIdx.x;
    if (p < P) {
        float s = 0.f;
        int i = 0;
        for (; i + 8 <= N; i += 8) {
            float v[8];
#pragma unroll
            for (int u = 0; u < 8; ++u) v[u] = per[(size_t)p * N + i + u];
#pragma unroll
            for (int u = 0; u < 8; ++u) s += v[u];
        }
        for (; i < N; ++i) s += per[(size_t)p * N + i];
        lp[p] = s / (float)N; loss[p] = lp[p];
    }
    __syncthreads();
    if (p == 0) { float tot = 0.f; for (int k = 0; k < P; ++k) tot += lp[k]; loss[P] = tot; }
}

__global__ void adam_tick_k(float* bc, float b1, float b2) {
    bc[2] *= b1; bc[3] *= b2; bc[0] = 1.f - bc[2]; bc[1] = 1.f - bc[3];
}

__global__ __launch_bounds__(256) void clamp_adam_k(float* __restrict__ p, float* __restrict__ g, float* __restrict__ m, float* __restrict__ v, long long n,
                                                    float lr, float b1, float b2, float eps, float clip, float gsc, const float* __restrict__ bc, float wd) {
    if (bc[7] != 0.f) { lr = bc[4]; clip = bc[5]; wd = bc[6]; }
    const float step = lr / bc[0], rs2 = 1.f / sqrtf(bc[1]), keep = 1.f - lr * wd;
    const long long n4 = n >> 2;
    for (long long i = (long long)blockIdx.x * 256 + threadIdx.x; i < n4; i += (long long)gridDim.x * 256) {
        float4 P = reinterpret_cast<float4*>(p)[i], G = reinterpret_cast<float4*>(g)[i], Mv = reinterpret_cast<float4*>(m)[i], V = reinterpret_cast<float4*>(v)[i];
        float* pp = &P.x; float* gg = &G.x; float* mm = &Mv.x; float* vv = &V.x;
#pragma unroll
        for (int e = 0; e < 4; ++e) {
            const float ge = fminf(fmaxf(gg[e] * gsc, -clip), clip);
            gg[e] = ge;
            mm[e] = b1 * mm[e] + (1.f - b1) * ge;
            vv[e] = b2 * vv[e] + (1.f - b2) * ge * ge;
            pp[e] = pp[e] * keep - step * mm[e] / (sqrtf(vv[e]) * rs2 + eps);
        }
        reinterpret_cast<float4*>(p)[i] = P; reinterpret_cast<float4*>(g)[i] = G; reinterpret_cast<float4*>(m)[i] = Mv; reinterpret_cast<float4*>(v)[i] = V;
    }
    for (long long i = (n4 << 2) + (long long)blockIdx.x * 256 + threadIdx.x; i < n; i += (long long)gridDim.x * 256) {
        const float ge = fminf(fmaxf(g[i] * gsc, -clip), clip);
        g[i] = ge;
        m[i] = b1 * m[i] + (1.f - b1) * ge;
        v[i] = b2 * v[i] + (1.f - b2) * ge * ge;
        p[i] = p[i] * keep - step * m[i] / (sqrtf(v[i]) * rs2 + eps);
    }
}

__global__ __launch_bounds__(256) void eval_hist_k(const unsigned char* __restrict__ pred, const float* __restrict__ gt, long long n, unsigned* __restrict__ hist) {
    __shared__ unsigned h[512];
    h[threadIdx.x] = 0; h[threadIdx.x + 256] = 0;
    __syncthreads();
    for (long long i = (long long)blockIdx.x * 256 + threadIdx.x; i < n; i += (long long)gridDim.x * 256) {
        const unsigned v = pred[i];
        atomicAdd(&h[v], 1u);
        if (gt[i] > 0.5f) atomicAdd(&h[256 + v], 1u);
    }
    __syncthreads();
    if (h[threadIdx.x]) atomicAdd(&hist[threadIdx.x], h[threadIdx.x]);
    if (h[threadIdx.x + 256]) atomicAdd(&hist[threadIdx.x + 256], h[threadIdx.x + 256]);
}

__global__ __launch_bounds__(256) void minmax_k(const float* __restrict__ x, long long n, float* __restrict__ part) {
    __shared__ float smn[4], smx[4];
    float mn = INFINITY, mx = -INFINITY;
    for (long long i = (long long)blockIdx.x * 256 + threadIdx.x; i < n; i += (long long)gridDim.x * 256) {
        const float s = 1.f / (1.f + expf(-x[i])); mn = fminf(mn, s); mx = fmaxf(mx, s);
    }
    for (int o = 32; o > 0; o >>= 1) { mn = fminf(mn, __shfl_xor(mn, o)); mx = fmaxf(mx, __shfl_xor(mx, o)); }
    if ((threadIdx.x & 63) == 0) { smn[threadIdx.x >> 6] = mn; smx[threadIdx.x >> 6] = mx; }
    __syncthreads();
    if (threadIdx.x == 0) {
        part[2 + blockIdx.x * 2] = fminf(fminf(smn[0], smn[1]), fminf(smn[2], smn[3]));
        part[3 + blockIdx.x * 2] = fmaxf(fmaxf(smx[0], smx[1]), fmaxf(smx[2], smx[3]));
    }
}
__global__ void minmax_final_k(float* part, int nb) {
    if (threadIdx.x == 0) {
        float mn = INFINITY, mx = -INFINITY;
        for (int b = 0; b < nb; ++b) { mn = fminf(mn, part[2 + 2 * b]); mx = fmaxf(mx, part[3 + 2 * b]); }
        part[0] = mn; part[1] = mx;
    }
}
__global__ __launch_bounds__(256) void eval_u8_k(const float* __restrict__ x, unsigned char* __restrict__ out, const float* __restrict__ mm, long long n) {
    const float mn = mm[0], den = mm[1] - mm[0] + 1e-8f;
    for (long long i = (long long)blockIdx.x * 256 + threadIdx.x; i < n; i += (long long)gridDim.x * 256) {
        const float s = 1.f / (1.f + expf(-x[i]));
        out[i] = (unsigned char)(((s - mn) / den) * 255.f);
    }
}

}

extern "C" {

int pn2_dsra_fuse_fwd(const float* fg, const float* cf, const float* cb, float* out, int M, int K, int sm, void* stream) {
    if (!fg || !cf || !cb || !out) return -1;
    if (K > MAXK) return -2;
    hipLaunchKernelGGL(dsra_fwd_k, dim3(grid_for(M)), dim3(256), 0, (hipStream_t)stream, fg, cf, cb, out, M, K, sm);
    PN2_CHECK_LAUNCH();
    return 0;
}
int pn2_dsra_fuse_bwd(const float* fg, const float* cf, const float* cb, const float* dout, float* dfg, float* dcf, float* dcb, int M, int K, int sm, void* stream) {
    if (!fg || !cf || !cb || !dout || !dfg || !dcf || !dcb) return -1;
    if (K > MAXK) return -2;
    hipLaunchKernelGGL(dsra_bwd_k, dim3(grid_for(M)), dim3(256), 0, (hipStream_t)stream, fg, cf, cb, dout, dfg, dcf, dcb, M, K, sm);
    PN2_CHECK_LAUNCH();
    return 0;
}

int pn2_ra_gate_fwd(int dt, const void* x, int ld_x, const float* crop, void* out, int ld_out, int M, int C, void* stream) {
    if (!x || !crop || !out) return -1;
    if (C % 8 || ld_x % 8 || ld_out % 8) return -2;
    hipStream_t st = (hipStream_t)stream;
    if (dt == PN2_BF16) hipLaunchKernelGGL(ra_gate_fwd_k<bf16_t>, dim3(grid_for((size_t)M * C / 8)), dim3(256), 0, st, (const bf16_t*)x, ld_x, crop, (bf16_t*)out, ld_out, M, C);
    else if (dt == PN2_F32) hipLaunchKernelGGL(ra_gate_fwd_k<float>, dim3(grid_for((size_t)M * C / 4)), dim3(256), 0, st, (const float*)x, ld_x, crop, (float*)out, ld_out, M, C);
    else return -3;
    PN2_CHECK_LAUNCH();
    return 0;
}
int pn2_ra_gate_bwd(int dt, const void* x, int ld_x, const float* crop, const void* dout, int ld_dout, void* dx, int ld_dx, int dx_accum, float* dcrop, int M, int C, void* stream) {
    if (!x || !crop || !dout || !dx || !dcrop) return -1;
    if (C % 8 || ld_x % 8 || ld_dout % 8 || ld_dx % 8) return -2;
    hipStream_t st = (hipStream_t)stream;
    const int grid = (M + 3) / 4 > 8192 ? 8192 : (M + 3) / 4;
    if (dt == PN2_BF16) hipLaunchKernelGGL((ra_gate_bwd_k<bf16_t, false>), dim3(grid), dim3(256), 0, st, (const bf16_t*)x, ld_x, crop, (const bf16_t*)dout, ld_dout, (bf16_t*)dx, ld_dx, dx_accum, dcrop, M, C);
    else if (dt == PN2_F32) hipLaunchKernelGGL((ra_gate_bwd_k<float, false>), dim3(grid), dim3(256), 0, st, (const float*)x, ld_x, crop, (const float*)dout, ld_dout, (float*)dx, ld_dx, dx_accum, dcrop, M, C);
    else return -3;
    PN2_CHECK_LAUNCH();
    return 0;
}
int pn2_ra_gate_post_bwd(int dt, const void* raw, int ld_raw, const float* crop, const void* dz, int ld_dz, void* dzg, int ld_dzg, float* dcrop, int M, int C, void* stream) {
    if (!raw || !crop || !dz || !dzg || !dcrop) return -1;
    if (C % 8 || ld_raw % 8 || ld_dz % 8 || ld_dzg % 8) return -2;
    hipStream_t st = (hipStream_t)stream;
    const int grid = (M + 3) / 4 > 8192 ? 8192 : (M + 3) / 4;
    if (dt == PN2_BF16) hipLaunchKernelGGL((ra_gate_bwd_k<bf16_t, true>), dim3(grid), dim3(256), 0, st, (const bf16_t*)raw, ld_raw, crop, (const bf16_t*)dz, ld_dz, (bf16_t*)dzg, ld_dzg, 0, dcrop, M, C);
    else if (dt == PN2_F32) hipLaunchKernelGGL((ra_gate_bwd_k<float, true>), dim3(grid), dim3(256), 0, st, (const float*)raw, ld_raw, crop, (const float*)dz, ld_dz, (float*)dzg, ld_dzg, 0, dcrop, M, C);
    else return -3;
    PN2_CHECK_LAUNCH();
    return 0;
}

static constexpr size_t loss_weights_lds(int ks) { return (size_t)((LTY + ks - 1) * ((LTX + ks - 1) | 1) + (LTY + ks - 1) * (LTX + 1)) * 4; }

int pn2_loss_weights_clear(const float* mask, float* weit, int N, int H, int W, int ksize, long long* clear, int nclear, void* stream) {
    if (!mask || !weit || (nclear > 0 && !clear) || nclear < 0) return -1;
    if (ksize < 1 || !(ksize & 1) || ksize > 63) return -2;
    return pn2_launch<loss_weights_k>(dim3((W + LTX - 1) / LTX, (H + LTY - 1) / LTY, N), dim3(256), loss_weights_lds(ksize), (int)loss_weights_lds(63), (hipStream_t)stream,
                                      mask, weit, H, W, ksize, clear, nclear);
}

int pn2_loss_weights(const float* mask, float* weit, int N, int H, int W, int ksize, void* stream) {
    return pn2_loss_weights_clear(mask, weit, N, H, W, ksize, nullptr, 0, stream);
}

int pn2_loss_blocks(int HW) { int b = (HW + 4095) / 4096; return b > 64 ? 64 : (b < 1 ? 1 : b); }

int pn2_structure_loss_fwd(const float* preds, long long map_stride, int P, const float* mask, const float* weit, float* partial,
                           float* sums, float* wsum, float* loss, int N, int HW, void* stream) {
    if (!preds || !mask || !weit || !partial || !sums || !wsum || !loss) return -1;
    if (P * N > 512 || P > 8) return -2;
    const int nb = pn2_loss_blocks(HW);
    hipLaunchKernelGGL(loss_fwd_k, dim3(nb, N, P), dim3(256), 0, (hipStream_t)stream, preds, map_stride, P, mask, weit, partial, N, HW);
    hipLaunchKernelGGL(loss_finalize_k, dim3(1), dim3(1024), 0, (hipStream_t)stream, partial, P, N, nb, sums, wsum, loss);
    PN2_CHECK_LAUNCH();
    return 0;
}

int pn2_structure_loss_bwd(const float* preds, float* dpreds, long long map_stride, int P, const float* mask, const float* weit, const float* wsum,
                           const float* sums, float gscale, int N, int HW, void* stream) {
    if (!preds || !dpreds || !mask || !weit || !wsum || !sums) return -1;
    int nb = (HW + 1023) / 1024; if (nb > 256) nb = 256;
    hipLaunchKernelGGL(loss_bwd_k, dim3(nb, N, P), dim3(256), 0, (hipStream_t)stream, preds, dpreds, map_stride, P, mask, weit, wsum, sums, gscale, N, HW);
    PN2_CHECK_LAUNCH();
    return 0;
}

int pn2_structure_loss_bwd_dev(const float* preds, float* dpreds, long long map_stride, long long dmap_stride, int P, const float* mask, const float* weit, const float* wsum,
                               const float* sums, const float* gscale_dev, float gscale, int N, int HW, void* stream) {
    if (!preds || !dpreds || !mask || !weit || !wsum || !sums) return -1;
    if (map_stride < 0 || dmap_stride < 0) return -2;
    int nb = (HW + 1023) / 1024; if (nb > 256) nb = 256;
    hipLaunchKernelGGL(loss_bwd_k, dim3(nb, N, P), dim3(256), 0, (hipStream_t)stream, preds, dpreds, map_stride, P, mask, weit, wsum, sums, gscale, N, HW, dmap_stride, gscale_dev);
    PN2_CHECK_LAUNCH();
    return 0;
}

int pn2_adam_tick(float* bc, float beta1, float beta2, void* stream) {
    if (!bc) return -1;
    hipLaunchKernelGGL(adam_tick_k, dim3(1), dim3(1), 0, (hipStream_t)stream, bc, beta1, beta2);
    PN2_CHECK_LAUNCH();
    return 0;
}

int pn2_clamp_adam(float* param, float* grad, float* exp_avg, float* exp_avg_sq, long long n, float lr, float beta1, float beta2,
                   float eps, float clip, float grad_scale, const float* bias_corr, float weight_decay, void* stream) {
    if (!param || !grad || !exp_avg || !exp_avg_sq || !bias_corr) return -1;
    if (((uintptr_t)param | (uintptr_t)grad | (uintptr_t)exp_avg | (uintptr_t)exp_avg_sq) & 15) return -2;
// ... 223 lines not shown
```

### pranet-v2_amd/pn2/capi.py

```python
import ctypes as C
import os

_HERE = os.path.dirname(os.path.abspath(__file__))
LIB_PATH = os.environ.get("PN2_LIB") or os.path.join(os.path.dirname(_HERE), "csrc", "libpn2_hip.so")

F32, BF16 = 0, 1
F32F = 2
F32X3 = 3
CONV_STATS, CONV_ACCUM, CONV_BIAS = 1, 2, 4
CONV_AFFINE, CONV_RELU, CONV_RELU6 = 16, 32, 64


class ConvDesc(C.Structure):
    _fields_ = [(n, C.c_int) for n in ("N", "H", "W", "OH", "OW", "Cin_p", "ld_in", "Cout", "ld_out", "KH", "KW", "stride",
                                       "pad_h", "pad_w", "dil_h", "dil_w", "transposed", "Kp", "flags")]


class WgradDesc(C.Structure):
    _fields_ = [(n, C.c_int) for n in ("N", "H", "W", "OH", "OW", "Cin_p", "ld_x", "Cout_p", "ld_dy", "KH", "KW", "stride",
                                       "pad_h", "pad_w", "dil_h", "dil_w", "Rp", "Kp", "tune")]


class PackDesc(C.Structure):
    _fields_ = [(n, C.c_int) for n in ("Cout", "Cin", "KH", "KW", "Cout_p", "gw_out", "gwp_out", "Cin_p", "gw_in", "gwp_in",
                                       "Rp", "Kp", "transposed", "ld", "koff")]


class PackJob(C.Structure):
    _fields_ = [("w", C.c_void_p), ("wp", C.c_void_p), ("d", PackDesc)]


class WgradJob(C.Structure):
    _fields_ = [("dy", C.c_void_p), ("x", C.c_void_p), ("slab", C.c_void_p), ("d", WgradDesc), ("nsplit", C.c_int), ("rot", C.c_int)]


class ReduceJob(C.Structure):
    _fields_ = [("slab", C.c_void_p), ("gw", C.c_void_p), ("d", PackDesc), ("nsplit", C.c_int), ("accumulate", C.c_int)]


class ColsumInJob(C.Structure):
    _fields_ = [("dy", C.c_void_p), ("partial", C.c_void_p), ("ld", C.c_int), ("M", C.c_int), ("C", C.c_int), ("rows", C.c_int), ("cvp", C.c_int), ("pad_", C.c_int)]


class ColsumJob(C.Structure):
    _fields_ = [("partial", C.c_void_p), ("out", C.c_void_p), ("nblk", C.c_int), ("C", C.c_int), ("ld", C.c_int), ("accumulate", C.c_int)]


class TailMap(C.Structure):
    _fields_ = [("src", C.c_void_p), ("dsrc", C.c_void_p), ("h", C.c_int), ("w", C.c_int), ("rh", C.c_float), ("rw", C.c_float),
                ("accumulate", C.c_int), ("pad_", C.c_int)]


class TailDesc(C.Structure):
    _fields_ = [("N", C.c_int), ("OH", C.c_int), ("OW", C.c_int), ("P", C.c_int), ("align_corners", C.c_int), ("pad_", C.c_int),
                ("maps", TailMap * 16)]


class BnDesc(C.Structure):
    _fields_ = [("M", C.c_int), ("Cp", C.c_int), ("C", C.c_int), ("gw", C.c_int), ("gwp", C.c_int),
                ("eps", C.c_float), ("momentum", C.c_float), ("ldp", C.c_int), ("tile_rows", C.c_int)]


BNB_STATS, BNB_MASK_RAW, BNB_MASK_Y, BNB_STORE_MASKED = 1, 2, 4, 8


class BnbTarget(C.Structure):
    _fields_ = [("out", C.c_void_p), ("ld_out", C.c_int), ("mode", C.c_int), ("raw", C.c_void_p), ("ld_raw", C.c_int),
                ("y", C.c_void_p), ("ld_y", C.c_int), ("par", C.c_void_p), ("ps", C.c_int), ("split", C.c_int),
                ("raw2", C.c_void_p), ("par2", C.c_void_p), ("p1", C.c_void_p), ("p2", C.c_void_p), ("ldp", C.c_int)]


class ConvEp(C.Structure):
    _fields_ = [("a", BnbTarget), ("b", BnbTarget), ("pool", C.c_void_p), ("ld_pool", C.c_int), ("pad_", C.c_int), ("c", BnbTarget)]


class BnSegs(C.Structure):
    _fields_ = [("nseg", C.c_int), ("c0", C.c_int * 4), ("nblk", C.c_int * 4), ("ldp", C.c_int * 4), ("p1", C.c_void_p * 4), ("p2", C.c_void_p * 4)]


class CopyJob(C.Structure):
    _fields_ = [("src", C.c_void_p), ("dst", C.c_void_p), ("ld_s", C.c_int), ("ld_d", C.c_int), ("M", C.c_int), ("C", C.c_int), ("accumulate", C.c_int), ("pad_", C.c_int)]


class ConvJob(C.Structure):
    _fields_ = [("in_", C.c_void_p), ("wp", C.c_void_p), ("out", C.c_void_p), ("psum", C.c_void_p), ("psq", C.c_void_p), ("d", ConvDesc), ("pad_", C.c_int), ("ep", ConvEp)]


class BnFinJob(C.Structure):
    _fields_ = [(n, C.c_void_p) for n in ("psum", "psq", "gamma", "beta", "running_mean", "running_var", "scale", "shift", "mean", "invstd")] + \
               [("d", BnDesc), ("nblk", C.c_int), ("cpb", C.c_int), ("pad_", C.c_int)]


class BnPrepJob(C.Structure):
    _fields_ = [(n, C.c_void_p) for n in ("gamma", "beta", "running_mean", "running_var", "scale", "shift")] + [("d", BnDesc), ("pad_", C.c_int)]


class AffineJob(C.Structure):
    _fields_ = [(n, C.c_void_p) for n in ("x", "y", "scale", "shift", "res", "add", "y2")] + \
               [(n, C.c_int) for n in ("ld_x", "ld_y", "ld_res", "ld_add", "ld_y2", "M", "C", "relu", "rows_per_blk", "cvp")]


class BnBFinJob(C.Structure):
    _fields_ = [("sg", BnSegs)] + [(n, C.c_void_p) for n in ("gamma", "invstd", "dgamma", "dbeta", "coef")] + \
               [("d", BnDesc), ("accumulate", C.c_int), ("cpb", C.c_int), ("pad_", C.c_int)]


class BnApplyJob(C.Structure):
    _fields_ = [(n, C.c_void_p) for n in ("dy", "y", "x", "mean", "invstd", "coef", "dx", "dres", "msc", "msh")] + \
               [(n, C.c_int) for n in ("ld_dy", "ld_y", "ld_x", "ld_dx", "ld_dres", "M", "Cp", "dres_accum", "r6", "rows_per_blk", "cvp", "pad_")]


class BnReduceJob(C.Structure):
    _fields_ = [(n, C.c_void_p) for n in ("dy", "y", "x", "mean", "invstd", "p1", "p2", "msc", "msh")] + \
               [(n, C.c_int) for n in ("ld_dy", "ld_y", "ld_x", "M", "Cp", "nblk", "rows_per_blk", "cvp", "r6", "pad_")]


P, I, LL, FL = C.c_void_p, C.c_int, C.c_longlong, C.c_float

SIGNATURES = {
    "pn2_conv_tile_n": [I],
    "pn2_wgrad_tile_co": [I],
    "pn2_conv_tile_m": [I, I, I],
    "pn2_conv_stat_blocks": [I, I, I],
    "pn2_conv_gemm": [I, P, P, P, P, P, C.POINTER(ConvDesc), P],
    "pn2_conv_gemm_ep": [I, P, P, P, C.POINTER(ConvDesc), C.POINTER(ConvEp), P],
    "pn2_conv_gemm_tile": [I, C.POINTER(ConvDesc)],
    "pn2_conv_gemm_job_blocks": [I, C.POINTER(ConvJob), I, I],
    "pn2_conv_gemm_multi": [I, I, I, I, P, P, I, I, P],
    "pn2_bn_finalize_job_blocks": [C.POINTER(BnFinJob)],
    "pn2_bn_finalize_multi": [P, P, I, I, P],
    "pn2_affine_job_blocks": [I, C.POINTER(AffineJob)],
    "pn2_affine_multi": [I, P, P, I, I, P],
    "pn2_bn_bwd_finalize_job_blocks": [C.POINTER(BnBFinJob)],
    "pn2_bn_bwd_finalize_multi": [P, P, I, I, P],
    "pn2_bn_bwd_apply_job_blocks": [I, C.POINTER(BnApplyJob)],
    "pn2_bn_bwd_apply_multi": [I, P, P, I, I, P],
    "pn2_bn_bwd_reduce_job_blocks": [I, C.POINTER(BnReduceJob)],
    "pn2_bn_bwd_reduce_multi": [I, P, P, I, I, P],
    "pn2_conv_wgrad": [I, P, P, P, C.POINTER(WgradDesc), I, P],
    "pn2_conv_wgrad_variant": [I, C.POINTER(WgradDesc)],
    "pn2_conv_wgrad_blocks": [C.POINTER(WgradDesc), I],
    "pn2_conv_wgrad_multi": [I, I, P, P, I, I, P],
    "pn2_pack_weight": [I, P, P, C.POINTER(PackDesc), P],
    "pn2_conv_dgrad_small_cin": [I, P, I, P, P, I, I, I, I, I, I, I, I, I, I, I, I, I, P],
    "pn2_conv_splitk_reduce": [I, P, I, I, I, P, I, P, P, P, I, P],
    "pn2_pack_patch_weight": [I, P, P, I, I, I, I, I, I, I, P],
    "pn2_depth_to_space": [I, P, I, P, I, I, I, I, I, I, I, I, I, P],
    "pn2_wgrad_reduce": [P, P, C.POINTER(PackDesc), I, I, P],
    "pn2_pack_blocks": [C.POINTER(PackDesc)],
    "pn2_pack_weights_multi": [I, P, P, I, I, P],
    "pn2_wgrad_reduce_blocks": [C.POINTER(PackDesc)],
    "pn2_wgrad_reduce_multi": [P, P, I, I, P],
    "pn2_bn_finalize": [P, P, I, C.POINTER(BnDesc), P, P, P, P, P, P, P, P, P],
    "pn2_bn_eval_prepare": [C.POINTER(BnDesc), P, P, P, P, P, P, P],
    "pn2_bn_eval_prepare_multi": [P, P, I, I, P],
    "pn2_affine_act_sum": [I, P, I, P, I, I, I, P, P, I, P, I, P, I, P],
    "pn2_affine_act_tee": [I, P, I, P, I, I, I, P, P, I, P, I, I, P],
    "pn2_bn_relu_maxpool_fwd": [I, P, I, P, P, P, I, P, I, I, I, I, I, I, P],
    "pn2_pool_bn_bwd_reduce": [I, P, I, P, P, I, I, I, I, I, I, I, P, P, P, P, P, P, I, P],
    "pn2_pool_bn_bwd_apply": [I, P, I, P, P, I, I, I, I, I, I, I, P, P, P, P, P, P, I, P],
    "pn2_affine_act": [I, P, I, I, P, I, I, I, P, P, P, I, I, P],
    "pn2_bn_bwd_reduce": [I, I, P, I, I, P, I, I, P, I, I, I, P, P, P, P, I, P, P, I, P],
    "pn2_bn_bwd_blocks": [I, I, I],
    "pn2_bn_bwd_finalize": [P, P, I, C.POINTER(BnDesc), P, P, P, P, I, P, P],
    "pn2_bn_bwd_finalize_seg": [C.POINTER(BnSegs), C.POINTER(BnDesc), P, P, P, P, I, P, P],
    "pn2_bn_bwd_apply": [I, I, P, I, I, P, I, I, P, I, I, I, P, P, P, P, I, P, I, I, P, P, I, P],
    "pn2_maxpool3x3s2_fwd": [I, P, I, P, I, P, I, I, I, I, I, I, P],
    "pn2_maxpool3x3s2_bwd": [I, P, I, P, P, I, I, I, I, I, I, I, P],
    "pn2_avgpool_fwd": [I, P, I, P, I, I, I, I, I, I, I, I, I, I, I, P],
    "pn2_avgpool_bwd": [I, P, I, P, I, I, I, I, I, I, I, I, I, I, I, I, P],
    "pn2_bilinear_fwd": [I, P, I, P, I, I, I, I, I, I, I, I, FL, FL, P],
    "pn2_bilinear_bwd": [I, P, I, P, I, I, I, I, I, I, I, I, FL, FL, I, P],
    "pn2_dsra_fuse_fwd": [P, P, P, P, I, I, I, P],
    "pn2_dsra_fuse_bwd": [P, P, P, P, P, P, P, I, I, I, P],
    "pn2_ra_gate_fwd": [I, P, I, P, P, I, I, I, P],
    "pn2_ra_gate_bwd": [I, P, I, P, P, I, P, I, I, P, I, I, P],
    "pn2_ra_gate_post_bwd": [I, P, I, P, P, I, P, I, P, I, I, P],
    "pn2_conv_gemm_gated": [I, P, P, P, P, P, P, P, P],
    "pn2_conv_gemm_affine": [I, P, P, P, P, P, P, I, P, P],
    "pn2_loss_weights": [P, P, I, I, I, I, P],
    "pn2_loss_weights_clear": [P, P, I, I, I, I, P, I, P],
    "pn2_loss_blocks": [I],
    "pn2_structure_loss_fwd": [P, LL, I, P, P, P, P, P, P, I, I, P],
    "pn2_structure_loss_bwd": [P, P, LL, I, P, P, P, P, FL, I, I, P],
    "pn2_structure_loss_bwd_dev": [P, P, LL, LL, I, P, P, P, P, P, FL, I, I, P],
    "pn2_dsra_tail_blocks": [I],
    "pn2_dsra_tail_fwd": [C.POINTER(TailDesc), P, P, P, P, P, P, P, P],
    "pn2_dsra_tail_scratch": [C.POINTER(TailDesc)],
    "pn2_dsra_tail_bwd": [C.POINTER(TailDesc), P, P, P, P, FL, P, LL, P],
    "pn2_dsra_tail_fused_ok": [C.POINTER(TailDesc)],
    "pn2_dsra_tail_fused_scratch": [C.POINTER(TailDesc)],
    "pn2_dsra_tail_fwd_bwd": [C.POINTER(TailDesc), P, P, P, P, P, P, P, P, FL, P, LL, P, P],
    "pn2_layernorm_fwd": [I, P, I, P, I, I, I, P, P, FL, P, P, P],
    "pn2_ln_slots": [I, I],
    "pn2_rows_blocks": [I, I],
    "pn2_layernorm_bwd": [I, P, I, P, I, I, I, P, P, P, P, I, I, P, P, I, P],
    "pn2_colsum_unit": [I, I],
    "pn2_colsum": [I, P, I, I, I, P, I, P],
    "pn2_colsum_finalize": [P, I, I, I, P, I, P],
    "pn2_colsum_job_blocks": [I, C.POINTER(ColsumInJob)],
    "pn2_colsum_multi": [I, P, P, I, I, P],
    "pn2_colsum_finalize_blocks": [I],
    "pn2_colsum_finalize_multi": [P, P, I, I, P],
    "pn2_dwconv3x3": [I, P, P, P, P, P, I, I, I, I, I, I, P],
    "pn2_dwconv3x3_colsum_blocks": [I, I, I, I, I],
    "pn2_dwconv3x3_colsum": [I, P, P, P, P, I, I, I, I, I, P, I, P],
    "pn2_gelu_bwd": [I, P, P, P, LL, P],
    "pn2_dwconv3x3_wgrad_blocks": [I, I, I, I, I],
    "pn2_dwconv3x3_wgrad": [I, P, P, P, I, I, I, I, I, P, P, P],
    "pn2_scale_samples": [I, P, P, P, P, I, LL, P],
    "pn2_attn_fwd": [I, P, I, P, I, P, I, P, I, I, I, I, I, FL, P],
    "pn2_attn_bwd_blocks": [I, I, I, I],
    "pn2_attn_bwd": [I, P, I, P, I, P, I, P, I, P, P, I, P, I, P, P, I, I, I, I, I, FL, P],
    "pn2_dwconv_blocks": [I, I, I, I, I, I, I],
    "pn2_dwconv": [I, P, P, P, I, I, I, I, I, I, I, P, P, P],
    "pn2_dwconv_wgrad": [I, P, P, P, I, I, I, I, I, P],
    "pn2_pairconv_blocks": [I, I, I, I, I],
    "pn2_pairconv3x3_fwd": [I, P, P, P, I, I, I, I, P, P, P],
    "pn2_pairconv3x3_dgrad": [I, P, P, P, I, I, I, I, I, P],
    "pn2_pairconv3x3_wgrad": [I, P, P, P, I, I, I, I, P],
    "pn2_gate_mul": [I, P, P, P, I, I, I, I, I, P],
    "pn2_gate_blocks": [I, I, I],
    "pn2_gate_bwd": [I, P, P, P, I, I, I, I, P],
    "pn2_global_pool": [I, P, P, P, P, I, I, I, P],
    "pn2_global_pool_bwd": [I, P, P, P, P, I, I, I, I, P],
    "pn2_chan_stats": [I, P, P, P, LL, I, P],
    "pn2_chan_stats_bwd": [I, P, P, P, LL, I, I, P],
    "pn2_upsample_nearest2x": [I, P, P, I, I, I, I, P],
    "pn2_upsample_nearest2x_bwd": [I, P, P, I, I, I, I, I, P],
    "pn2_gather_sum": [I, P, P, P, P, P, LL, I, P],
    "pn2_sigmoid": [I, P, I, I, P, LL, P],
    "pn2_sigmoid_bwd": [I, P, P, P, I, I, LL, I, P],
    "pn2_mutation_loss_blocks": [LL],
    "pn2_mutation_loss_width": [I],
    "pn2_mutation_loss_fwd": [P, P, P, P, I, LL, I, FL, FL, FL, P, P, P, P],
    "pn2_mutation_loss_bwd": [P, P, P, P, P, P, I, LL, I, FL, FL, FL, P, FL, P],
    "pn2_seg_loss_width": [I],
    "pn2_seg_loss_fwd": [P, C.c_uint, P, I, LL, I, FL, FL, P, P, P, P],
    "pn2_seg_loss_bwd": [P, P, C.c_uint, P, I, LL, I, FL, FL, P, FL, P],
    "pn2_binary": [I, I, P, I, P, I, P, I, I, I, I, P],
    "pn2_mul_bwd": [I, P, I, P, I, P, I, P, I, I, P, I, I, I, I, P],
    "pn2_copy": [I, P, I, I, P, I, I, I, I, P],
    "pn2_copy_job_blocks": [I, C.POINTER(CopyJob)],
    "pn2_copy_multi": [I, P, P, I, I, P],
    "pn2_nchw_to_nhwc": [I, P, P, I, I, I, I, I, P],
    "pn2_bias_grad": [P, I, I, P, I, P],
    "pn2_resize_ksize": [I, I],
    "pn2_resize_coeffs": [I, I, P, P, P],
    "pn2_resize_u8_pass": [P, P, I, I, I, I, I, P, P, P, I, P],
    "pn2_u8_to_tensor": [P, P, I, I, I, P, P, P],
    "pn2_clamp_adam": [P, P, P, P, LL, FL, FL, FL, FL, FL, FL, P, FL, P],
    "pn2_adam_tick": [P, FL, FL, P],
    "pn2_eval_tail": [P, P, P, LL, P],
    "pn2_eval_hist": [P, P, LL, P, P],
    "pn2_eval_region_sums": [P, P, I, I, P, P],
    "pn2_eval_wfm_blocks": [I, I],
    "pn2_eval_wfm": [P, P, I, I, P, C.c_double, P, P, P, P],
    "pn2_seg_labels": [P, I, I, I, I, I, I, P, P],
    "pn2_seg_counts": [P, P, LL, I, P, P],
    "pn2_seg_surface_workspace": [I, I, I, I, C.POINTER(LL)],
    "pn2_seg_surface_hist_len": [I, I, I],
    "pn2_seg_surface_hist": [P, P, I, I, I, I, I, P, P, P, P],
}
_VALUE_FUNCS = {"pn2_copy_job_blocks", "pn2_conv_gemm_tile", "pn2_conv_gemm_job_blocks", "pn2_bn_finalize_job_blocks", "pn2_affine_job_blocks", "pn2_bn_bwd_finalize_job_blocks",
                "pn2_bn_bwd_apply_job_blocks", "pn2_bn_bwd_reduce_job_blocks", "pn2_dwconv3x3_colsum_blocks", "pn2_resize_ksize", "pn2_colsum_job_blocks", "pn2_colsum_finalize_blocks", "pn2_dwconv3x3_wgrad_blocks", "pn2_conv_tile_n", "pn2_wgrad_tile_co", "pn2_conv_stat_blocks", "pn2_conv_tile_m", "pn2_bn_bwd_blocks", "pn2_loss_blocks",
                "pn2_pack_blocks", "pn2_wgrad_reduce_blocks", "pn2_conv_wgrad_variant", "pn2_conv_wgrad_blocks",
                "pn2_dsra_tail_blocks", "pn2_dsra_tail_scratch", "pn2_dsra_tail_fused_ok", "pn2_dsra_tail_fused_scratch", "pn2_ln_slots", "pn2_rows_blocks", "pn2_colsum_unit", "pn2_attn_bwd_blocks", "pn2_mutation_loss_blocks", "pn2_mutation_loss_width", "pn2_seg_loss_width",
                "pn2_dwconv_blocks", "pn2_pairconv_blocks", "pn2_gate_blocks", "pn2_eval_wfm_blocks", "pn2_seg_surface_hist_len"}

_lib = None
WORK = {}


def load():
    global _lib
    if _lib is not None:
        return _lib
    if not os.path.exists(LIB_PATH):
        raise RuntimeError(f"{LIB_PATH} not found: build it with `make -C pranet-v2_amd/csrc` (or __graft_entry__.build()); "
                           "pranet-v2_amd has no CPU / PyTorch fallback path")
    lib = C.CDLL(LIB_PATH)
    for name, args in SIGNATURES.items():
        fn = getattr(lib, name)
        fn.argtypes = args
        fn.restype = C.c_int
    _lib = lib
    return lib


class _Caller:

    def __getattr__(self, name):
        fn = getattr(load(), name)
        if name in _VALUE_FUNCS:
            return fn

        def checked(*a):
            rc = fn(*a)
            if rc != 0:
                raise RuntimeError(f"{name} failed with status {rc}")
        setattr(self, name, checked)
        return checked


call = _Caller()
```

### pranet-v2_amd/pn2/core.py

```python
import ctypes as C
import math
import os

import torch

from . import capi
from .capi import call, F32, BF16

TORCH_DT = {F32: torch.float32, BF16: torch.bfloat16}
_PERMS = {}
TUNER = {}


def load_tuner(path):
    import ast
    import json
    try:
        with open(path) as f:
            for k, v in json.load(f).items():
                TUNER.setdefault(ast.literal_eval(k), tuple(v) if isinstance(v, list) else v)
    except (OSError, ValueError):
        pass


# ... 222 lines not shown

    def __reduce__(self):
        return (BnFoldCache, ())

    def __deepcopy__(self, memo):
        return BnFoldCache()

    def stale(self):
        return any(j.gamma != bn.weight.data_ptr() or j.running_mean != bn.running_mean.data_ptr() for j, bn in zip(self.jobs, self.keep))

    def add(self, key, bn, par, bd, off=0):
        self.entries[key] = par
        j = capi.BnPrepJob()
        j.gamma, j.beta, j.running_mean, j.running_var = bn.weight.data_ptr(), bn.bias.data_ptr(), bn.running_mean.data_ptr(), bn.running_var.data_ptr()
        j.scale, j.shift = par[0][off:].data_ptr(), par[1][off:].data_ptr()
        C.memmove(C.byref(j.d), C.byref(bd), C.sizeof(capi.BnDesc))
        self.jobs.append(j)
        self.keep.append(bn)
        if self.table is not None:
            self.retired.append((self.table, self.bstart))
        self.table = None
        self.version += 1

    def refresh(self):
        if not self.jobs:
            return
        if self.table is None:
            self.table, self.bstart, self.nblocks = _job_table(capi.BnPrepJob, self.jobs, [(j.d.Cp + 255) // 256 for j in self.jobs])
        call.pn2_bn_eval_prepare_multi(_p(self.table), _p(self.bstart), len(self.jobs), self.nblocks, _stream())


def _job_table(struct, jobs, blocks):
    if min(blocks) < 1:
        raise RuntimeError("job with an unsupported geometry in a table-driven launch")
    arr = (struct * len(jobs))(*jobs)
    table = torch.frombuffer(bytearray(bytes(memoryview(arr).cast("B"))), dtype=torch.uint8).cuda()
    start = [0]
    for b in blocks:
        start.append(start[-1] + b)
    return table, torch.tensor(start, dtype=torch.int32).cuda(), start[-1]


class StepArena:

    def __init__(self):
        self.buf, self.off, self.need = None, 0, 0

    def begin_step(self, dev):
        want = self.need
        if want and (self.buf is None or self.buf.numel() < want) and not torch.cuda.is_current_stream_capturing():
            self.buf = None
            self.buf = torch.empty(want, dtype=torch.uint8, device=dev)
        self.off, self.need = 0, 0

    def alloc(self, shape, dtype, dev):
        n = dtype.itemsize
        for d in shape:
            n *= d
        na = (n + 255) // 256 * 256
        self.need += na
        if self.buf is not None and self.off + na <= self.buf.numel():
            t = self.buf[self.off:self.off + n].view(dtype).view(shape)
            self.off += na
            return t
        return torch.empty(shape, dtype=dtype, device=dev)


TUNE_COLD = os.environ.get("PN2_TUNE_COLD", "1") == "1"
WGRAD_WGS = 640
WGRAD_SLAB_MB = 24
WGRAD_MIX = float(os.environ.get("PN2_WGRAD_MIX", "2"))
WGRAD_SLAB_CAP = float(os.environ.get("PN2_WGRAD_SLAB_CAP", "0.35"))
WGRAD_ROTATE = os.environ.get("PN2_WGRAD_ROTATE", "1") == "1"
_THRASH = {}


def _thrash():
    dev = torch.cuda.current_device()
    t = _THRASH.get(dev)
    if t is None:
        t = _THRASH[dev] = torch.empty(512 << 20, dtype=torch.uint8, device="cuda")
    t.fill_(1)


DEFER_COLSUM = os.environ.get("PN2_DEFER_COLSUM", "1") == "1"
SMALL_CIN_DGRAD = os.environ.get("PN2_SMALL_CIN_DGRAD", "1") == "1"
GRAD_ALIAS = os.environ.get("PN2_GRAD_ALIAS", "1") == "1"
SPLITK = os.environ.get("PN2_SPLITK", "1") == "1"
TUNE_LOG = None
KS2 = os.environ.get("PN2_KS2", "1") == "1"
KSPLIT_MINK = 4096
PATCH_DGRAD = os.environ.get("PN2_PATCH_DGRAD", "1") == "1"
FUSE_BIAS = os.environ.get("PN2_FUSE_BIAS", "1") == "1"
BNB_EPILOGUE = os.environ.get("PN2_BNB_EPILOGUE", "1") == "1"
LOCKSTEP = os.environ.get("PN2_LOCKSTEP", "1") == "1"
DW_COLSUM = os.environ.get("PN2_DW_COLSUM", "1") == "1"
MASKED_STORE = os.environ.get("PN2_MASKED_STORE", "1") == "1"
POOL_BWD_QUAD = os.environ.get("PN2_POOL_BWD_QUAD", "1") == "1"
RES_STATS = os.environ.get("PN2_RES_STATS", "1") == "1"
MUL_BWD = os.environ.get("PN2_MUL_BWD", "1") == "1"
POOL_FOLD = os.environ.get("PN2_POOL_FOLD", "1") == "1"
POOL_FUSE = os.environ.get("PN2_POOL_FUSE", "1") == "1"
TEE_CONCAT = os.environ.get("PN2_TEE_CONCAT", "1") == "1"
EVAL_FUSE = True
ZERO_CROP_SKIP = os.environ.get("PN2_ZERO_CROP_SKIP", "1") == "1"


class GradQueue:

    def __init__(self, defer_wgrad=True, slab_cap=None):
        self.defer_wgrad = defer_wgrad
        self.slab_cap = slab_cap
        self.slabs = {}
        self.cache = {}
        self.ccache = {}
        self.begin_step()

    def begin_step(self):
        self.seg = 0
        self.wjobs, self.rjobs, self.keep = [], [], []
        self.uses, self.levels = {}, {}

    def slab(self, key, shape, dev):
        n = self.uses.get(key, 0)
        self.uses[key] = n + 1
        key = key + (n,)
        t = self.slabs.get(key)
        if t is None or tuple(t.shape) != tuple(shape):
            if t is not None:
                raise RuntimeError("wgrad slab geometry changed between steps; build a new Trainer for a new input shape")
            if torch.cuda.is_current_stream_capturing():
                raise RuntimeError("run eager steps before capturing (persistent wgrad slabs are allocated then)")
            t = self.slabs[key] = torch.empty(shape, dtype=torch.float32, device=dev)
        return t

    def table_splits(self, nsplit, M, chans, wd, esize=2):
        cap = self.slab_cap if self.slab_cap is not None else WGRAD_SLAB_CAP
        if cap <= 0:
            return nsplit
        return min(nsplit, max(1, int(cap * M * chans * esize // (wd.Rp * wd.Kp * 4))))

    def add_wgrad(self, dt, dy, x_ptr, x_keep, slab, wd, nsplit, flops=0):
        self.wjobs.append((dt, dy.data_ptr(), x_ptr.value, slab.data_ptr(), wd, nsplit, flops))
        self.keep.append((dy, x_keep))

    def add_reduce(self, slab, gw, rd, nsplit, accumulate):
        lvl = self.levels.get(gw.data_ptr(), 0)
        if accumulate and lvl == 0:
            self.flush()
            lvl = 0
        self.levels[gw.data_ptr()] = lvl + 1
        self.rjobs.append((slab.data_ptr(), gw.data_ptr(), rd, nsplit, accumulate, lvl))

    def _build(self):
        launches = []
        groups = {}
        for dt, dy, x, slab, wd, ns, fl in self.wjobs:
            v = call.pn2_conv_wgrad_variant(dt, C.byref(wd))
            if v < 0:
                raise RuntimeError("unsupported wgrad geometry")
            groups.setdefault((dt, v), []).append((dy, x, slab, wd, ns, fl))
        order = lambda js: sorted(js, key=lambda j: -((j[3].N * j[3].OH * j[3].OW + j[4] - 1) // j[4]) * j[3].KH * j[3].KW)
        mixed = {}
        if WGRAD_MIX > 0:
            for dt in {k[0] for k in groups}:
                a, b = groups.get((dt, 12)), groups.get((dt, 13))
                if a and b:
                    a, b = order(a), order(b)
                    real = lambda j: j[4] * call.pn2_conv_wgrad_blocks(C.byref(j[3]), j[4]) // (8 * ((j[4] + 7) // 8))
                    ta, tb = sum(real(j) for j in a) or 1, sum(real(j) for j in b) or 1
                    out, ia, ib, ca, cb = [], 0, 0, 0, 0
                    while ia < len(a) or ib < len(b):
                        if ib >= len(b) or (ia < len(a) and ca / (ta / WGRAD_MIX) <= cb / tb):
                            out.append(a[ia]); ca += real(a[ia]); ia += 1
                        else:
                            out.append(b[ib]); cb += real(b[ib]); ib += 1
                    del groups[(dt, 12)], groups[(dt, 13)]
                    groups[(dt, 14)] = out
                    mixed[(dt, 14)] = True
        for (dt, v), js in sorted(groups.items()):
            if (dt, v) not in mixed:
                js = order(js)
            arr, load = [], [0] * 8
            for dy, x, slab, wd, ns, fl in js:
                j = capi.WgradJob()
                j.dy, j.x, j.slab, j.nsplit = dy, x, slab, ns
                if WGRAD_ROTATE:
                    w = ((wd.N * wd.OH * wd.OW + 31) // 32 + ns - 1) // ns * (call.pn2_conv_wgrad_blocks(C.byref(wd), ns) // (8 * ((ns + 7) // 8)))
                    per = [(ns - x_ + 7) // 8 for x_ in range(8)]
                    best = min(range(8), key=lambda r: (max(load[(x_ + r) & 7] + per[x_] * w for x_ in range(8)), r))
                    for x_ in range(8):
                        load[(x_ + best) & 7] += per[x_] * w
                    j.rot = best
                C.memmove(C.byref(j.d), C.byref(wd), C.sizeof(capi.WgradDesc))
                arr.append(j)
            table, bstart, nblocks = _job_table(capi.WgradJob, arr, [call.pn2_conv_wgrad_blocks(C.byref(j.d), j.nsplit) for j in arr])
            launches.append(("w", dt, v, table, bstart, len(arr), nblocks, sum(j[5] for j in js)))
        for lvl in sorted({j[5] for j in self.rjobs}):
            arr = []
            for slab, gw, rd, ns, acc, l_ in self.rjobs:
                if l_ != lvl:
                    continue
                j = capi.ReduceJob()
                j.slab, j.gw, j.nsplit, j.accumulate = slab, gw, ns, acc
                C.memmove(C.byref(j.d), C.byref(rd), C.sizeof(capi.PackDesc))
                arr.append(j)
            table, bstart, nblocks = _job_table(capi.ReduceJob, arr, [call.pn2_wgrad_reduce_blocks(C.byref(j.d)) for j in arr])
            launches.append(("r", 0, 0, table, bstart, len(arr), nblocks, 0))
        return launches

    def flush(self):
        if not self.wjobs and not self.rjobs:
            return
        sig = (tuple(j[:4] + (j[5],) for j in self.wjobs), tuple(j[:2] + j[3:] for j in self.rjobs))
        hit = self.cache.get(self.seg)
        if hit is None or hit[0] != sig:
            if torch.cuda.is_current_stream_capturing():
                raise RuntimeError("run two eager steps before capturing (the deferred-launch tables are built then)")
            hit = self.cache[self.seg] = (sig, self._build())
        st = _stream()
        for kind, dt, v, table, bstart, njobs, nblocks, flops in hit[1]:
            if kind == "w":
                capi.WORK.update(flops=flops, tag="", shape=f"variant{v} jobs{njobs}")
                call.pn2_conv_wgrad_multi(dt, v, _p(table), _p(bstart), njobs, nblocks, st)
            else:
                call.pn2_wgrad_reduce_multi(_p(table), _p(bstart), njobs, nblocks, st)
        self.seg += 1
        self.wjobs, self.rjobs, self.keep = [], [], []
        self.levels = {}
```

### pranet-v2_amd/pn2/profile.py

```python
import time

import torch

from . import capi

_EL = {0: 4, 1: 2}
ACTUAL = {}


def _bytes(name, a):
    try:
        if name == "pn2_affine_act":
            dt_in, _, _, dt_out, _, _, M, C, _, _, res = a[:11]
            return M * C * (_EL[dt_in] * (2 if res.value else 1) + _EL[dt_out])
        if name == "pn2_bn_bwd_reduce":
            dt, dt_dy, _, _, Cdy, y = a[0], a[1], a[2], a[3], a[4], a[5]
            M, Cp = a[10], a[11]
            return M * (Cdy * _EL[dt_dy] + Cp * _EL[dt] * (2 if y.value else 1))
        if name == "pn2_bn_bwd_apply":
            dt, dt_dy, Cdy, y, M, Cp, dres = a[0], a[1], a[4], a[5], a[10], a[11], a[17]
            return M * (Cdy * _EL[dt_dy] + Cp * _EL[dt] * (2 + (1 if y.value else 0) + (1 if dres.value else 0)))
        if name == "pn2_affine_act_sum":
            dt, M, C = a[0], a[5], a[6]
            return M * C * _EL[dt] * 4
        if name in ("pn2_bilinear_fwd", "pn2_bilinear_bwd", "pn2_avgpool_fwd", "pn2_avgpool_bwd"):
            dt, N, H, W, C, OH, OW = a[0], a[5], a[6], a[7], a[8], a[9], a[10]
            return N * C * _EL[dt] * (H * W + OH * OW)
        if name in ("pn2_maxpool3x3s2_fwd", "pn2_maxpool3x3s2_bwd"):
            dt, N, H, W, C, OH, OW = a[0], a[6], a[7], a[8], a[9], a[10], a[11]
            return N * C * (_EL[dt] * (H * W + OH * OW) + OH * OW)
        if name in ("pn2_dsra_tail_fwd", "pn2_dsra_tail_bwd"):
            d = a[0]._obj
            S = d.N * d.OH * d.OW * 4
            ACTUAL["tail"] = ACTUAL.get("tail", 0) + (S * (2 * d.P + 2) if name.endswith("fwd") else S * 2)
            return S * (2 * d.P + 1) if name.endswith("fwd") else S * 2 * d.P
        if name == "pn2_dsra_tail_fwd_bwd":
            d = a[0]._obj
            S = d.N * d.OH * d.OW * 4
            ACTUAL["tail"] = ACTUAL.get("tail", 0) + S * (2 * d.P + 4)
            return S * (4 * d.P + 1)
        if name == "pn2_structure_loss_fwd":
            P, N, HW = a[2], a[9], a[10]
            return N * HW * 4 * (2 * P + 2)
        if name == "pn2_structure_loss_bwd":
            P, N, HW = a[3], a[9], a[10]
            return N * HW * 4 * (4 * P + 2)
        if name == "pn2_clamp_adam":
            return int(a[4]) * 4 * 7
        if name == "pn2_binary":
            dt, M, C = a[0], a[8], a[9]
            return M * C * _EL[dt] * 3
        if name == "pn2_copy":
            return a[6] * a[7] * (_EL[a[0]] + _EL[a[3]])
        if name == "pn2_nchw_to_nhwc":
            return a[4] * a[6] * (a[5] * 4 + a[7] * _EL[a[0]])
    except Exception:
        return 0
    return 0


def _shape(name, a):
    try:
        if name == "pn2_affine_act":
            return f"M{a[6]} C{a[7]} ldx{a[2]} ldy{a[5]} res{1 if a[10].value else 0}"
        if name in ("pn2_bn_bwd_reduce", "pn2_bn_bwd_apply"):
            return f"M{a[10]} C{a[11]} lddy{a[3]} ldx{a[9]} y{1 if a[5].value else 0}"
        if name == "pn2_wgrad_reduce":
            d = a[2]._obj
            return f"{d.Cin}->{d.Cout} k{d.KH}x{d.KW} Rp{d.Rp} Kp{d.Kp} ns{a[3]}"
        if name in ("pn2_bilinear_fwd", "pn2_bilinear_bwd", "pn2_avgpool_fwd", "pn2_avgpool_bwd"):
            return f"dt{a[0]} N{a[5]} {a[6]}x{a[7]} C{a[8]} -> {a[9]}x{a[10]}"
        if name == "pn2_binary":
            return f"dt{a[0]} op{a[1]} M{a[8]} C{a[9]} acc{a[10]}"
        if name == "pn2_copy":
            return f"dt{a[0]}->{a[3]} M{a[6]} C{a[7]} lds{a[2]} ldd{a[5]} acc{a[8]}"
        if name in ("pn2_bn_finalize", "pn2_bn_bwd_finalize"):
            return f"nblk{a[2]} Cp{a[3]._obj.Cp}"
        if name == "pn2_dwconv":
            return f"{a[4]}x{a[5]}x{a[6]}x{a[7]} k{a[8]} flip{a[9]} acc{a[10]} stats{1 if a[11].value else 0}"
        if name == "pn2_dwconv_wgrad":
            return f"{a[4]}x{a[5]}x{a[6]}x{a[7]} k{a[8]}"
        if name == "pn2_dwconv3x3":
            return f"{a[6]}x{a[7]}x{a[8]}x{a[9]} flip{a[10]} acc{a[11]} gelu{1 if a[5].value else 0}"
        if name == "pn2_dwconv3x3_wgrad":
            return f"{a[5]}x{a[6]}x{a[7]}x{a[8]} gelu{1 if a[9].value else 0}"
        if name == "pn2_attn_fwd":
            return f"B{a[8]} Nq{a[9]} Nkv{a[10]} h{a[11]}"
        if name == "pn2_attn_bwd":
            return f"B{a[16]} Nq{a[17]} Nkv{a[18]} h{a[19]}"
        if name in ("pn2_layernorm_fwd", "pn2_layernorm_bwd"):
            return f"M{a[5]} C{a[6]}"
        if name == "pn2_colsum":
            return f"M{a[3]} C{a[4]}"
        if name == "pn2_colsum_finalize":
            return f"nblk{a[1]} C{a[2]}"
        if name == "pn2_gather_sum":
            return f"n{a[6]} k{a[7]}"
        if name in ("pn2_upsample_nearest2x", "pn2_upsample_nearest2x_bwd"):
            return f"{a[3]}x{a[4]}x{a[5]}x{a[6]}"
    except Exception:
        pass
    return ""


class Recorder:
    def __init__(self):
        self.rows = []
        self.saved = {}

    def __enter__(self):
        lib = capi.load()
        for name in capi.SIGNATURES:
            if name in capi._VALUE_FUNCS:
                continue
            fn = getattr(lib, name)

            def wrapped(*a, _fn=fn, _name=name):
                by_ = 0
                if _name in ("pn2_conv_gemm", "pn2_conv_gemm_ep", "pn2_conv_gemm_multi", "pn2_conv_wgrad", "pn2_conv_wgrad_multi"):
                    fl, tag, shape = capi.WORK.pop("flops", 0), capi.WORK.pop("tag", ""), capi.WORK.pop("shape", "")
                    es = 2 if int(a[0]) == capi.BF16 else 4
                    by_ = sum(_conv_bytes(s_, es) for s_ in (capi.WORK.pop("shapes", None) or [shape]))
                else:
                    fl, tag, shape = 0, "", _shape(_name, a)
                    by_ = capi.WORK.pop("bytes", 0) if _name.endswith("_multi") else _bytes(_name, a)
                e0 = torch.cuda.Event(enable_timing=True); e1 = torch.cuda.Event(enable_timing=True)
                e0.record()
                rc = _fn(*a)
                e1.record()
                if rc != 0:
                    raise RuntimeError(f"{_name} failed with status {rc}")
                if _name == "pn2_conv_gemm_ep":
                    _name = "pn2_conv_gemm"
                self.rows.append((_name + tag, fl, by_, e0, e1, shape))
            self.saved[name] = capi.call.__dict__.get(name)
            setattr(capi.call, name, wrapped)
        return self

    def __exit__(self, *exc):
        for name, old in self.saved.items():
            if old is None:
                capi.call.__dict__.pop(name, None)
            else:
                setattr(capi.call, name, old)

    def summary(self, detail=False):
        torch.cuda.synchronize()
        agg = {}
        for name, fl, by, e0, e1, shape in self.rows:
            if detail and shape:
                name = name + " " + shape
            d = agg.setdefault(name, {"ms": 0.0, "launches": 0, "flops": 0, "bytes": 0})
            d["ms"] += e0.elapsed_time(e1); d["launches"] += 1; d["flops"] += fl; d["bytes"] += by if not fl else 0
        return agg


def _conv_bytes(shape, es):
    try:
        io, k, s_, _, dims = shape.split(" ")[:5]
        cin = int(io.split("->")[0]); cout = sum(int(v) for v in io.split("->")[1].split("+"))
        kh, kw = (int(v) for v in k[1:].split("x")); st = int(s_[1:])
        n, oh, ow = (int(v) for v in dims.split("x"))
        return es * (n * oh * st * ow * st * cin + n * oh * ow * cout + cin * cout * kh * kw)
    except Exception:
        return 0


PMC_FILE = "r06_pmc_hbm_traffic.json"


def _pmc_traffic(symbols, config):
    import json, os
    path = os.path.join(os.path.dirname(os.path.dirname(os.path.dirname(os.path.abspath(__file__)))), "profiles", PMC_FILE)
    try:
        doc = json.load(open(path))
        ks = doc["kernels"]
    except Exception:
        return None
    if any(doc.get("config", {}).get(k) != v for k, v in config.items()):
        return None
    rows = [ks[k] for k in symbols if k in ks]
    if not rows:
        return None
    n = sum(r["launches"] for r in rows)
    return {"bytes_per_launch": int(sum(r["hbm_bytes_per_launch"] * r["launches"] for r in rows) / n), "source": "profiles/" + PMC_FILE,
            "commit": doc.get("commit"), "step_total_bytes": doc.get("step_total_bytes")}


def _conv_class(shape):
    try:
        io, k = shape.split(" ")[0], shape.split(" ")[1]
        cin = int(io.split("->")[0]); cout = sum(int(v) for v in io.split("->")[1].split("+"))
        if k == "k1x1":
            return "1x1 wide (>= 416 ch)" if max(cin, cout) >= 416 else "1x1 narrow (< 416 ch)"
        if k == "k3x3" and cin == cout and cin in (26, 52, 104, 208):
            return "3x3 Res2Net branch (26/52/104/208 ch)"
        if k == "k5x5":
            return "5x5 (ra4)"
        return "3x3 / 1xk / kx1 other (stem, RFB, aggregation, heads)"
    except Exception:
        return "other"
# ... 81 lines not shown
```

### pranet-v2_amd/pn2/trainer.py

```python
import ctypes as C
import os

import torch

from .capi import call, F32
from .engine import Engine, Act, PackCache, GradQueue, StepArena, TUNER, _p, _stream
from .graph import get_compute_dtype
from .dp import GradBuckets
from . import loss as L


def _r4(n):
    return (n + 3) // 4 * 4


CAPTURE_MODE = os.environ.get("PN2_CAPTURE_MODE", "thread_local")
DP_SEGMENTS = os.environ.get("PN2_DP_SEGMENTS", "1") == "1"
_DP_CAPTURE_ENV = os.environ.get("PN2_DP_CAPTURE", "")


def dp_capture_wanted(world):
    return _DP_CAPTURE_ENV == "1" or (_DP_CAPTURE_ENV == "" and world == 1)


_CAP_GROUPS = {}


class Trainer:
    def __init__(self, model, lr=1e-4, clip=0.5, betas=(0.9, 0.999), eps=1e-8, dtype=None, process_group=None, bucket_bytes=100 << 20,
                 loss="structure", loss_weights=None, weight_decay=0.0, hot=None, force_dp=False, supervision="mutation"):
        self.model = model
        if loss not in ("structure", "mutation"):
            raise ValueError(f"unknown loss {loss!r}")
        self.single = loss == "mutation" and getattr(model, "dual", True) is False
        if supervision not in L.SEG_SUBSETS:
            raise ValueError(f"unknown supervision {supervision!r} (one of {sorted(L.SEG_SUBSETS)})")
        if supervision != "mutation" and not self.single:
            raise ValueError(f"supervision={supervision!r} needs loss='mutation' and a single-supervision EMCADNet (dual=False): the dual loss is built for 'mutation' only")
        if loss_weights is None:
            loss_weights = (0.3, 0.7) if self.single else (0.5, 0.7, 0.3)
        self.loss_kind, self.supervision, self.loss_weights, self.weight_decay = loss, supervision, tuple(float(v) for v in loss_weights), float(weight_decay)
        clip = 3.0e38 if clip is None else clip
        self.lr, self.clip, self.betas, self.eps = lr, clip, betas, eps
        self.dtype = get_compute_dtype() if dtype is None else dtype
        self.pg = process_group
        self.world = torch.distributed.get_world_size(process_group) if process_group is not None else 1
        self.dp = process_group is not None and (self.world > 1 or force_dp or os.environ.get("PN2_DP_FORCE", "0") == "1")
        hot = list(model.hot_parameters()) if hot is None else list(hot)
        hot_ids = {id(p) for p in hot}
        cold = [p for p in model.parameters() if id(p) not in hot_ids]
        dev = hot[0].device
        if dev.type != "cuda":
            raise RuntimeError("Trainer needs the model on the GPU (no CPU path)")
        self.n_hot = sum(_r4(p.numel()) for p in hot)
        n_all = self.n_hot + sum(_r4(p.numel()) for p in cold)
        self.flat = torch.zeros(n_all, dtype=torch.float32, device=dev)
        self.gflat = torch.zeros(self.n_hot, dtype=torch.float32, device=dev)
        self.exp_avg = torch.zeros(self.n_hot, dtype=torch.float32, device=dev)
        self.exp_avg_sq = torch.zeros(self.n_hot, dtype=torch.float32, device=dev)
        self.bias_corr = torch.tensor([0.0, 0.0, 1.0, 1.0, lr, clip, float(weight_decay), 1.0], dtype=torch.float32, device=dev)
        self.off = {}
        o = 0
        for p in hot + cold:
            n = p.numel()
            self.flat[o:o + n].copy_(p.data.reshape(-1))
            p.data = self.flat[o:o + n].view(p.shape)
            self.off[id(p)] = (o, n)
            o += _r4(n)
        self.hot = hot
        bucket_bytes = int(os.environ.get("PN2_DP_BUCKET_MB", "0")) << 20 or bucket_bytes
        self.buckets = GradBuckets(self.gflat, [(id(p), self.off[id(p)][0], _r4(self.off[id(p)][1])) for p in hot], bucket_bytes, process_group,
                                   wire_dtype=torch.bfloat16 if os.environ.get("PN2_DP_WIRE", "fp32") == "bf16" else None)
        self.pg_cap, self._cap_warm_t = None, 0.0
        if self.dp and dp_capture_wanted(self.world):
            import time
            import torch.distributed as dist
            ranks = dist.get_process_group_ranks(process_group)
            if dist.get_backend(process_group) == "nccl" and len(ranks) == dist.get_world_size():
                if process_group not in _CAP_GROUPS:
                    cap = dist.new_group(ranks=ranks, backend="nccl")
                    warm = torch.zeros(4, dtype=torch.float32, device=dev)
                    dist.all_reduce(warm, group=cap)
                    torch.cuda.synchronize()
                    _CAP_GROUPS[process_group] = (cap, time.monotonic())
                self.pg_cap, self._cap_warm_t = _CAP_GROUPS[process_group]
        self._seg = None
        self._expected = None
        self.last_outs = None
        self.pack_cache = PackCache()
        self._states = {}
        self._cur = None
        self.fuse_tail = os.environ.get("PN2_FUSED_TAIL", "1") == "1"
        self.tuner = TUNER if os.environ.get("PN2_AUTOTUNE", "1") == "1" else None
        self._tuned = len(self.tuner) if self.tuner is not None else 0

    def set_lr(self, lr):
        self.lr = float(lr)
        self.bias_corr[4] = self.lr

    def set_clip(self, clip):
        self.clip = 3.0e38 if clip is None else float(clip)
        self.bias_corr[5] = self.clip

    @property
    def param_groups(self):
        tr = self

        class _Group(dict):
            def __setitem__(g, k, v):
                dict.__setitem__(g, k, v)
                if k == 'lr':
                    tr.set_lr(v)
        return [_Group(lr=self.lr, params=self.hot, betas=self.betas, eps=self.eps, weight_decay=self.weight_decay)]

    def _grad_view(self, p):
        off, n = self.off[id(p)]
        return self.gflat[off:off + n].view(p.shape)

    def _state(self, images, size=None):
        N, _, H, W = images.shape
        key = (N, H, W, size if size is not None else H)
        st = self._states.get(key)
        if st is None:
            from types import SimpleNamespace
            mode = os.environ.get("PN2_DEFER_WGRAD", "2")
            st = self._states[key] = SimpleNamespace(
                key=key, steps_run=0, graph=None, graph_opt=None, segments=None, s_images=None, s_gts=None, s_loss=None,
                lock_cache={},
                grad_queue=GradQueue(defer_wgrad=mode == "2") if mode in ("1", "2") else None,
                arena=StepArena() if os.environ.get("PN2_STEP_ARENA", "1") == "1" else None)
        self._cur = st
        return st

    arena = property(lambda self: self._cur.arena if self._cur else None)
    grad_queue = property(lambda self: self._cur.grad_queue if self._cur else None)
    steps_run = property(lambda self: self._cur.steps_run if self._cur else 0)

    def forward_backward(self, images, gts, reduce_hook=True, size=None):
        st = self._state(images, size)
        self.pack_cache.refresh()
        if st.arena is not None:
            st.arena.begin_step(self.flat.device)
        st.steps_run += 1
        eng = Engine(self.dtype, True, grad_provider=self._grad_view, need_grad=True, pack_cache=self.pack_cache, tuner=self.tuner, grad_queue=st.grad_queue, arena=st.arena,
                     lock_cache=st.lock_cache if (st.arena is not None and st.arena.buf is not None) else None)
        eng.fuse_tail = self.fuse_tail and self.loss_kind == "structure"
        if size is not None and (size != images.shape[2] or size != images.shape[3]):
            x = eng.cast(eng.resize_to(eng.from_nchw(images, dt=F32), size, size, align_corners=True), eng.dt)
            n_, _, h_, w_ = gts.shape
            g = Act(eng, gts.reshape(n_, h_, w_, 1).float().contiguous(), 1, 1, 1, F32, requires_grad=False)
            gts = eng.resize_to(g, size, size, align_corners=True).t
        else:
            x = eng.from_nchw(images)
        outs = self.model._build(eng, x)
        eng.finish_forward()
        if self.single:
            label = gts[0] if isinstance(gts, (tuple, list)) else gts
            loss = L.seg_forward_backward(eng, outs, label, self.supervision, self.loss_weights)
            return self._backward(eng, st, loss, None, reduce_hook)
        if self.loss_kind == "mutation":
            label, bg_mask = gts
            loss = L.mutation_forward_backward(eng, outs, label, bg_mask, self.loss_weights)
            return self._backward(eng, st, loss, None, reduce_hook)
        N, H, W = outs[0].N, outs[0].H, outs[0].W
        P = len(outs) // 2
        lat = eng.lateral_block()
        if lat is None or any(o.t.data_ptr() != lat[j].data_ptr() for j, o in enumerate(outs)):
            lat = torch.stack([o.t for o in outs])
        HW = H * W
        mask = gts.reshape(N, HW).float().contiguous()
        fused = len(eng.tail) == len(outs) and outs[0].C == 1
        if eng.tail and not fused:
            raise RuntimeError("only some lateral maps were deferred to the fused DSRA tail")
        if fused:
            loss = L.tail_forward_backward(eng, eng.tail, lat, P, mask, N, H, W) if os.environ.get("PN2_TAIL_FUSED_ENTRY", "1") == "1" else None
            if loss is None:
                loss, saved = L.tail_forward(eng, eng.tail, lat, P, mask, N, H, W)
                L.tail_backward(eng, eng.tail, P, mask, saved, 1.0)
        else:
            loss, saved = L.loss_forward(lat, P, mask, N, HW, H, W)
            dlat = eng.alloc(lat.shape, lat.dtype)
            L.loss_backward(lat, dlat, P, mask, saved, N, HW, 1.0)
            for j, o in enumerate(outs):
                o.grad = dlat[j]
                o.grad_written = True
        return self._backward(eng, st, loss, lat, reduce_hook)

    def _backward(self, eng, st, loss, lat, reduce_hook):
        if self.dp:
            self.buckets.reset()
        rq = st.grad_queue
        if rq is not None:
            rq.begin_step()

        def grads_complete():
            eng.flush_colsum()
            if rq is not None:
                rq.flush()
        hook = self.dp and reduce_hook
        expected = self._expected
        if hook and expected is not None:
            self.buckets.expect(expected)

            def late(k, c, bk=self.buckets):
                if k in bk.launched_keys:
                    raise RuntimeError("a gradient contribution arrived after its bucket was all-reduced (the model's use of its parameters changed "
                                       "between steps): build a new Trainer")
                bk.contribution(k)
            eng.pgrads.on_sink = late
        for fn in reversed(eng.tape):
            fn()
            if hook and expected is not None:
                self.buckets.launch_ready(eng.pgrads.counts, before_launch=grads_complete, expected=expected)
                if self._seg is not None and self.buckets.record:
                    self._cut_segment()
        eng.tape = []
        if eng._pending_pool:
            raise RuntimeError("a deferred AvgPool2d backward was never applied (see Engine.backward)")
        eng.pgrads.on_sink = None
        if len(eng.pgrads.written) != len(self.hot):
            missing = [n for n, p in self.model.named_parameters() if id(p) in {id(q) for q in self.hot} and id(p) not in eng.pgrads.written]
            raise RuntimeError(f"{len(missing)} trained parameters received no gradient this step (first: {missing[:3]}): exclude them from `hot`")
        grads_complete()
        if self.dp:
            if reduce_hook and expected is None:
                self._expected = dict(eng.pgrads.counts)
            self.buckets.finish()
        self.last_outs = lat
        eng.tail.clear()
        eng._lat = None
        eng.pgrads.provider = None
        eng.lock_cache = eng.grad_queue = eng.arena = eng.pack_cache = None
        if self.tuner is not None and len(self.tuner) != self._tuned and os.environ.get("PN2_TUNE_CACHE"):
            from .engine import save_tuner
            save_tuner(os.environ["PN2_TUNE_CACHE"])
        self._tuned = len(self.tuner) if self.tuner is not None else 0
        return loss

    def optimizer_step(self):
        st = _stream()
        call.pn2_adam_tick(_p(self.bias_corr), self.betas[0], self.betas[1], st)
        call.pn2_clamp_adam(_p(self.flat), _p(self.gflat), _p(self.exp_avg), _p(self.exp_avg_sq), self.n_hot, self.lr, self.betas[0], self.betas[1],
                            self.eps, self.clip, 1.0 / self.world, _p(self.bias_corr), self.weight_decay, st)

    def step(self, images, gts, size=None):
        loss = self.forward_backward(images, gts, size=size)
        self.optimizer_step()
        return loss

    def state_dict(self):
        return {"model": {k: v.detach().clone() for k, v in self.model.state_dict().items()},
                "optimizer": {"exp_avg": self.exp_avg.clone(), "exp_avg_sq": self.exp_avg_sq.clone(), "bias_corr": self.bias_corr.clone(),
                              "lr": self.lr, "betas": tuple(self.betas), "eps": self.eps, "clip": self.clip, "weight_decay": self.weight_decay,
                              "layout": [(n, self.off[id(p)][0], p.numel()) for n, p in self.model.named_parameters() if id(p) in self.off]}}

    def load_state_dict(self, sd):
        layout = [(n, self.off[id(p)][0], p.numel()) for n, p in self.model.named_parameters() if id(p) in self.off]
        o = sd["optimizer"]
        if [tuple(x) for x in o["layout"]] != layout:
            raise RuntimeError("optimizer state was saved for a different parameter layout")
        self.model.load_state_dict(sd["model"], strict=True)
        with torch.no_grad():
            self.exp_avg.copy_(o["exp_avg"]); self.exp_avg_sq.copy_(o["exp_avg_sq"]); self.bias_corr[:4].copy_(o["bias_corr"][:4])
        self.lr, self.betas, self.eps, self.clip, self.weight_decay = o["lr"], tuple(o["betas"]), o["eps"], o["clip"], o["weight_decay"]
        with torch.no_grad():
            self.bias_corr[4:7] = torch.tensor([self.lr, self.clip, self.weight_decay], device=self.bias_corr.device)
        for st in self._states.values():
            st.graph = st.graph_opt = st.segments = None
        return self

    def capture(self, images, gts, warmup=3, size=None):
        st = self._state(images, size)
        if st.steps_run + warmup < 2:
            raise RuntimeError("capture() needs at least 2 eager steps before the captured one (warmup >= 2 on a fresh Trainer)")
        st.s_images = images.clone()
        st.s_gts = tuple(g.clone() for g in gts) if isinstance(gts, (tuple, list)) else gts.clone()
        side = torch.cuda.Stream()
        side.wait_stream(torch.cuda.current_stream())
        with torch.cuda.stream(side):
            for _ in range(warmup):
                self.step(st.s_images, st.s_gts, size=size)
            if self.dp and not DP_SEGMENTS:
                self.forward_backward_local(st.s_images, st.s_gts, size=size)
        torch.cuda.current_stream().wait_stream(side)
        torch.cuda.synchronize()
        import gc
        st.graph = torch.cuda.CUDAGraph()
        gc_was = gc.isenabled()
        gc.collect()
        gc.disable()
        try:
            if not self.dp:
                with torch.cuda.graph(st.graph, capture_error_mode=CAPTURE_MODE):
                    st.s_loss = self.step(st.s_images, st.s_gts, size=size)
                st.graph_opt = None
            elif self._agree(self._capture_with_collectives(st, size)):
                st.graph_opt, st.segments = None, None
            else:
                st.graph = torch.cuda.CUDAGraph()
                if DP_SEGMENTS and self._expected is not None:
                    st.segments = self._capture_segments(st, size)
                    st.graph = st.segments[0][0]
                else:
                    st.segments = None
                    with torch.cuda.graph(st.graph, capture_error_mode=CAPTURE_MODE):
                        st.s_loss = self.forward_backward_local(st.s_images, st.s_gts, size=size)
                st.graph_opt = torch.cuda.CUDAGraph()
                with torch.cuda.graph(st.graph_opt, capture_error_mode=CAPTURE_MODE):
                    self.optimizer_step()
        finally:
            if gc_was:
                gc.enable()
        return self

    def _capture_with_collectives(self, st, size):
        if self.pg_cap is None or self._expected is None:
            return False
        import time
        torch.cuda.synchronize()
        dt = 0.5 - (time.monotonic() - self._cap_warm_t)
        if dt > 0:
            time.sleep(dt)
        g = torch.cuda.CUDAGraph()
        main_pg, self.buckets.pg = self.buckets.pg, self.pg_cap
        try:
            with torch.cuda.graph(g, capture_error_mode=CAPTURE_MODE):
                st.s_loss = self.step(st.s_images, st.s_gts, size=size)
        except Exception as e:
            import warnings
            warnings.warn(f"capturing the RCCL collectives into the step graph failed ({type(e).__name__}: {e}); falling back to graph segments")
            self.buckets.works = []
            torch.cuda.synchronize()
            return False
        finally:
            self.buckets.pg = main_pg
        st.graph = g
        return True

    def _agree(self, ok):
        if self.world > 1:
            import torch.distributed as dist
            torch.cuda.synchronize()
            flag = torch.tensor([1 if ok else 0], dtype=torch.int32, device=self.flat.device)
            dist.all_reduce(flag, op=dist.ReduceOp.MIN, group=self.pg)
            agreed = bool(int(flag.item()))
            if ok and not agreed:
                import warnings
                warnings.warn("another rank could not capture the RCCL collectives into its step graph; every rank falls back to graph segments")
            return agreed
        return ok

    def _cut_segment(self):
        seg = self._seg
        seg["g"].capture_end()
        seg["list"].append((seg["g"], list(self.buckets.record)))
        del self.buckets.record[:]
        seg["g"] = torch.cuda.CUDAGraph()
        seg["g"].capture_begin(pool=seg["pool"], capture_error_mode=CAPTURE_MODE)

    def _capture_segments(self, st, size):
        segs = []
        cs = torch.cuda.Stream()
        cs.wait_stream(torch.cuda.current_stream())
        torch.cuda.synchronize()
        with torch.cuda.stream(cs):
            g = torch.cuda.CUDAGraph()
            self._seg = {"g": g, "pool": torch.cuda.graph_pool_handle(), "list": segs}
            self.buckets.record = []
            g.capture_begin(pool=self._seg["pool"], capture_error_mode=CAPTURE_MODE)
            try:
                st.s_loss = self.forward_backward(st.s_images, st.s_gts, size=size)
                self._seg["g"].capture_end()
                segs.append((self._seg["g"], list(self.buckets.record)))
            except BaseException:
                try:
                    self._seg["g"].capture_end()
                except Exception:
                    pass
                del segs[:]
                st.segments = st.graph = None
                raise
            finally:
                self._seg = None
                self.buckets.record = None
        torch.cuda.current_stream().wait_stream(cs)
        torch.cuda.synchronize()
        return segs

    def forward_backward_local(self, images, gts, size=None):
        w, self.dp = self.dp, False
        try:
            return self.forward_backward(images, gts, size=size)
        finally:
            self.dp = w

    def replay(self, images=None, gts=None, size=None):
        st = self._cur if images is None else self._state(images, size)
        if st is None or st.graph is None:
            raise RuntimeError("capture() this batch shape / train size first")
        if images is not None:
            st.s_images.copy_(images, non_blocking=True)
            if isinstance(gts, (tuple, list)):
                for d_, s_ in zip(st.s_gts, gts):
                    d_.copy_(s_, non_blocking=True)
            else:
                st.s_gts.copy_(gts, non_blocking=True)
        if st.graph_opt is None:
            st.graph.replay()
        elif st.segments:
            self.buckets.reset()
            for g, bs in st.segments:
                g.replay()
                self.buckets.launch_async(bs)
            self.buckets.wait()
            st.graph_opt.replay()
        else:
            st.graph.replay()
            self.buckets.reduce_all()
            st.graph_opt.replay()
        return st.s_loss
```

Measured before the change: 2323 images/sec.

## Fuse wgrad slab reduce, Adam update, and weight repacking into one step-tail kernel

Adds a step_tail kernel that, per conv weight tile, sums the deferred wgrad split-K slabs, applies clamp+Adam, and writes the repacked bf16 weight panels straight from shared memory. Non-conv parameter ranges get a chunked Adam path inside the same launch. The host side plans which parameters are covered, builds job tables during eager steps, and tracks a weight revision so the separate pack-cache refresh can be skipped on graph replay. This is meant to remove the separate reduce, optimizer, and repack launches and their extra HBM round trips of gradients and weights. In exchange it adds a lot of bookkeeping complexity and constraints on capture ordering.

```diff
diff --git a/include/pn2.h b/include/pn2.h
--- a/include/pn2.h
+++ b/include/pn2.h
@@ -95,6 +95,10 @@
 typedef struct pn2_reduce_job { const float* slab; float* gw; pn2_pack_desc d; int nsplit; int accumulate; } pn2_reduce_job;
 int pn2_wgrad_reduce_blocks(const pn2_pack_desc* p);
 int pn2_wgrad_reduce_multi(const pn2_reduce_job* jobs_dev, const int* block_start_dev, int njobs, int total_blocks, void* stream);
+typedef struct pn2_tail_job { const float* slab; float* g; float* w; float* m; float* v; pn2_pack_desc d; int nsplit, accumulate, pack0, npack; long long n; } pn2_tail_job;
+int pn2_step_tail_blocks(const pn2_tail_job* j);
+int pn2_step_tail(int dtype, const pn2_tail_job* jobs_dev, const pn2_pack_job* packs_dev, const int* block_start_dev, int njobs, int total_blocks,
+                  float lr, float beta1, float beta2, float eps, float clip, float grad_scale, const float* bias_corr, float weight_decay, void* stream);
 
 typedef struct pn2_bn_desc {
     int M;
diff --git a/pranet-v2_amd/csrc/pn2_common.h b/pranet-v2_amd/csrc/pn2_common.h
--- a/pranet-v2_amd/csrc/pn2_common.h
+++ b/pranet-v2_amd/csrc/pn2_common.h
@@ -90,6 +90,31 @@
     return lo;
 }
 
+struct adam_consts { float b1, b2, eps, clip, gsc, step, rs2, keep; };
+__device__ __forceinline__ adam_consts adam_setup(float lr, float b1, float b2, float eps, float clip, float gsc, const float* __restrict__ bc, float wd) {
+    if (bc[7] != 0.f) { lr = bc[4]; clip = bc[5]; wd = bc[6]; }
+    return {b1, b2, eps, clip, gsc, lr / bc[0], 1.f / sqrtf(bc[1]), fmaf(-lr, wd, 1.f)};
+}
+__device__ __forceinline__ void adam_elem(float& p, float& g, float& m, float& v, const adam_consts& c) {
+    const float ge = fminf(fmaxf(g * c.gsc, -c.clip), c.clip);
+    g = ge;
+    m = fmaf(c.b1, m, (1.f - c.b1) * ge);
+    v = fmaf(c.b2, v, ((1.f - c.b2) * ge) * ge);
+    p = fmaf(p, c.keep, -((c.step * m) / fmaf(sqrtf(v), c.rs2, c.eps)));
+}
+__device__ __forceinline__ void clamp_adam_range(float* __restrict__ p, float* __restrict__ g, float* __restrict__ m, float* __restrict__ v, long long n,
+                                                 int blk, int nblk, const adam_consts& c) {
+    const long long n4 = n >> 2;
+    for (long long i = (long long)blk * 256 + threadIdx.x; i < n4; i += (long long)nblk * 256) {
+        float4 P = reinterpret_cast<float4*>(p)[i], G = reinterpret_cast<float4*>(g)[i], Mv = reinterpret_cast<float4*>(m)[i], V = reinterpret_cast<float4*>(v)[i];
+        float* pp = &P.x; float* gg = &G.x; float* mm = &Mv.x; float* vv = &V.x;
+#pragma unroll
+        for (int e = 0; e < 4; ++e) adam_elem(pp[e], gg[e], mm[e], vv[e], c);
+        reinterpret_cast<float4*>(p)[i] = P; reinterpret_cast<float4*>(g)[i] = G; reinterpret_cast<float4*>(m)[i] = Mv; reinterpret_cast<float4*>(v)[i] = V;
+    }
+    for (long long i = (n4 << 2) + (long long)blk * 256 + threadIdx.x; i < n; i += (long long)nblk * 256) adam_elem(p[i], g[i], m[i], v[i], c);
+}
+
 __device__ __forceinline__ float wave_sum(float v) {
 #pragma unroll
     for (int o = 32; o > 0; o >>= 1) v += __shfl_xor(v, o);
diff --git a/pranet-v2_amd/csrc/pn2_conv.hip b/pranet-v2_amd/csrc/pn2_conv.hip
--- a/pranet-v2_amd/csrc/pn2_conv.hip
+++ b/pranet-v2_amd/csrc/pn2_conv.hip
@@ -1835,31 +1835,27 @@
     return ((p.Cout + CO - 1) / CO) * ((p.Cin + CI - 1) / CI);
 }
 
+struct pack_tile_geom { int taps, CO, CI, co0, ci0, nco_t, nci_t, run, rs; };
+__device__ __forceinline__ pack_tile_geom pack_tile_of(const pn2_pack_desc& p, int local) {
+    pack_tile_geom t;
+    t.taps = p.KH * p.KW;
+    pack_tile(t.taps, t.CO, t.CI);
+    const int nci = (p.Cin + t.CI - 1) / t.CI;
+    t.co0 = (local / nci) * t.CO; t.ci0 = (local - (local / nci) * nci) * t.CI;
+    t.nco_t = min(t.CO, p.Cout - t.co0); t.nci_t = min(t.CI, p.Cin - t.ci0);
+    t.run = t.nci_t * t.taps; t.rs = t.CI * t.taps + 1;
+    return t;
+}
+__device__ __forceinline__ int log2phys_f(int c, int gw, int gwp, float inv_gw) { const int g = (int)(((float)c + 0.5f) * inv_gw); return g * gwp + (c - g * gw); }
+
 template <typename T>
-__global__ __launch_bounds__(256) void pack_weight_multi(const pn2_pack_job* __restrict__ jobs, const int* __restrict__ bstart, int njobs) {
-    __shared__ float tile[7296];
-    const int jb = find_job(bstart, njobs, blockIdx.x);
-    const pn2_pack_job j = jobs[jb];
-    const pn2_pack_desc p = j.d;
-    const float* __restrict__ w = j.w;
-    T* __restrict__ wp = reinterpret_cast<T*>(j.wp);
-    const int taps = p.KH * p.KW;
-    int CO, CI; pack_tile(taps, CO, CI);
-    const int local = blockIdx.x - bstart[jb];
-    const int nci = (p.Cin + CI - 1) / CI;
-    const int co0 = (local / nci) * CO, ci0 = (local - (local / nci) * nci) * CI;
-    const int nco_t = min(CO, p.Cout - co0), nci_t = min(CI, p.Cin - ci0);
-    const int run = nci_t * taps, rs = CI * taps + 1;
+__device__ __forceinline__ void pack_tile_store(const float* tile, const pn2_pack_desc& p, T* __restrict__ wp, const pack_tile_geom& t) {
     const int tx = threadIdx.x & 63, ty = threadIdx.x >> 6;
-    for (int col = ty; col < nco_t; col += 4) {
-        const float* src = w + ((size_t)(co0 + col) * p.Cin + ci0) * taps;
-        for (int r = tx; r < run; r += 64) tile[col * rs + r] = src[r];
-    }
-    __syncthreads();
+    const int taps = t.taps, CO = t.CO, CI = t.CI, co0 = t.co0, ci0 = t.ci0, nco_t = t.nco_t, nci_t = t.nci_t, rs = t.rs;
     const size_t ld = p.ld ? p.ld : p.Kp;
     const float inv_gi = 1.f / (float)p.gw_in, inv_go = 1.f / (float)p.gw_out;
-    auto phys_in = [&](int c) { const int g = (int)(((float)c + 0.5f) * inv_gi); return g * p.gwp_in + (c - g * p.gw_in); };
-    auto phys_out = [&](int c) { const int g = (int)(((float)c + 0.5f) * inv_go); return g * p.gwp_out + (c - g * p.gw_out); };
+    auto phys_in = [&](int c) { return log2phys_f(c, p.gw_in, p.gwp_in, inv_gi); };
+    auto phys_out = [&](int c) { return log2phys_f(c, p.gw_out, p.gwp_out, inv_go); };
     if (!p.transposed) {
         const int sh = 31 - __clz(CI);
         for (int col = ty; col < nco_t; col += 4) {
@@ -1879,6 +1875,23 @@
             }
         }
     }
+}
+
+template <typename T>
+__global__ __launch_bounds__(256) void pack_weight_multi(const pn2_pack_job* __restrict__ jobs, const int* __restrict__ bstart, int njobs) {
+    __shared__ float tile[7296];
+    const int jb = find_job(bstart, njobs, blockIdx.x);
+    const pn2_pack_job j = jobs[jb];
+    const pn2_pack_desc p = j.d;
+    const float* __restrict__ w = j.w;
+    const pack_tile_geom t = pack_tile_of(p, blockIdx.x - bstart[jb]);
+    const int tx = threadIdx.x & 63, ty = threadIdx.x >> 6;
+    for (int col = ty; col < t.nco_t; col += 4) {
+        const float* src = w + ((size_t)(t.co0 + col) * p.Cin + t.ci0) * t.taps;
+        for (int r = tx; r < t.run; r += 64) tile[col * t.rs + r] = src[r];
+    }
+    __syncthreads();
+    pack_tile_store<T>(tile, p, reinterpret_cast<T*>(j.wp), t);
 }
 
 __device__ __forceinline__ void wgrad_reduce_body(const float* __restrict__ slab, float* __restrict__ gw, const pn2_pack_desc& p, int nsplit, int accumulate,
@@ -1947,6 +1960,88 @@
     return (int)(b > 2048 ? 2048 : (b < 1 ? 1 : b));
 }
 
+__device__ __forceinline__ float slab_partial(const float* __restrict__ s, size_t sstride, int nsplit, int sub, int S) {
+    float v0 = 0.f, v1 = 0.f, v2 = 0.f, v3 = 0.f;
+    int i = sub;
+    for (; i + 3 * S < nsplit; i += 4 * S) {
+        const float a0 = s[(size_t)i * sstride], a1 = s[(size_t)(i + S) * sstride], a2 = s[(size_t)(i + 2 * S) * sstride], a3 = s[(size_t)(i + 3 * S) * sstride];
+        v0 += a0; v1 += a1; v2 += a2; v3 += a3;
+    }
+    for (; i < nsplit; i += S) v0 += s[(size_t)i * sstride];
+    return (v0 + v1) + (v2 + v3);
+}
+__device__ __forceinline__ float slab_sum(const float* __restrict__ s, size_t sstride, int nsplit, int S) {
+    if (S == 1) return slab_partial(s, sstride, nsplit, 0, 1);
+    float l1 = 0.f, l2 = 0.f, l4 = 0.f, l8 = 0.f, x = 0.f;
+#pragma unroll 1
+    for (int sub = 0; sub < S; ++sub) {
+        x = slab_partial(s, sstride, nsplit, sub, S);
+        if (!(sub & 1)) { l1 = x; continue; }
+        x = l1 + x;
+        if (!(sub & 2)) { l2 = x; continue; }
+        x = l2 + x;
+        if (!(sub & 4)) { l4 = x; continue; }
+        x = l4 + x;
+        if (!(sub & 8)) { l8 = x; continue; }
+        x = l8 + x;
+    }
+    return x;
+}
+
+constexpr int STEP_TAIL_RANGE = 8192;
+
+template <typename T>
+__global__ __launch_bounds__(256) void step_tail(const pn2_tail_job* __restrict__ jobs, const pn2_pack_job* __restrict__ packs, const int* __restrict__ bstart, int njobs,
+                                                 float lr, float b1, float b2, float eps, float clip, float gsc, const float* __restrict__ bc, float wd) {
+    __shared__ float tile[7296];
+    const int jb = find_job(bstart, njobs, blockIdx.x);
+    const pn2_tail_job j = jobs[jb];
+    const int local = blockIdx.x - bstart[jb];
+    const adam_consts c = adam_setup(lr, b1, b2, eps, clip, gsc, bc, wd);
+    if (j.n > 0) {
+        const long long o = (long long)local * STEP_TAIL_RANGE;
+        const long long len = j.n - o < STEP_TAIL_RANGE ? j.n - o : STEP_TAIL_RANGE;
+        clamp_adam_range(j.w + o, j.g + o, j.m + o, j.v + o, len, 0, 1, c);
+        return;
+    }
+    const pn2_pack_desc p = j.d;
+    const pack_tile_geom t = pack_tile_of(p, local);
+    const int tx = threadIdx.x & 63, ty = threadIdx.x >> 6;
+    if (j.nsplit > 0) {
+        const int kv = (t.taps * p.Cin_p) >> 2;
+        const size_t total = (size_t)p.Cout_p * kv, sstride = (size_t)p.Rp * p.Kp;
+        int S = 1;
+        while (S < 16 && total * S < 32768 && 2 * S <= j.nsplit) S <<= 1;
+        const float inv_gi = 1.f / (float)p.gw_in, inv_go = 1.f / (float)p.gw_out;
+        const int sh = 31 - __clz(t.CI);
+        for (int col = ty; col < t.nco_t; col += 4) {
+            const float* srow = j.slab + (size_t)log2phys_f(t.co0 + col, p.gw_out, p.gwp_out, inv_go) * p.Kp;
+            for (int cb = tx; cb < t.taps * t.CI; cb += 64) {
+                const int tap = cb >> sh, cil = cb & (t.CI - 1);
+                if (cil < t.nci_t)
+                    tile[col * t.rs + cil * t.taps + tap] = slab_sum(srow + tap * p.Cin_p + log2phys_f(t.ci0 + cil, p.gw_in, p.gwp_in, inv_gi), sstride, j.nsplit, S);
+            }
+        }
+        __syncthreads();
+    }
+    for (int col = ty; col < t.nco_t; col += 4) {
+        const size_t base = ((size_t)(t.co0 + col) * p.Cin + t.ci0) * t.taps;
+        for (int r = tx; r < t.run; r += 64) {
+            const size_t i = base + r;
+            float g = j.nsplit > 0 ? (j.accumulate ? j.g[i] + tile[col * t.rs + r] : tile[col * t.rs + r]) : j.g[i];
+            float w = j.w[i], m = j.m[i], v = j.v[i];
+            adam_elem(w, g, m, v, c);
+            j.g[i] = g; j.w[i] = w; j.m[i] = m; j.v[i] = v;
+            tile[col * t.rs + r] = w;
+        }
+    }
+    __syncthreads();
+    for (int k = 0; k < j.npack; ++k) {
+        const pn2_pack_job pj = packs[j.pack0 + k];
+        pack_tile_store<T>(tile, pj.d, reinterpret_cast<T*>(pj.wp), t);
+    }
+}
+
 constexpr int TUNE_KS2 = 0x40, TUNE_KS4 = 0x80;
 constexpr int TILE_KS2 = 0x100;
 inline int conv_tune(const pn2_conv_desc& d) { return (d.flags >> 8) & 0xff; }
@@ -2571,6 +2666,22 @@
 }
 
 
+int pn2_step_tail_blocks(const pn2_tail_job* j) {
+    if (!j) return -1;
+    if (j->n > 0) return (int)((j->n + STEP_TAIL_RANGE - 1) / STEP_TAIL_RANGE);
+    return j->d.KH * j->d.KW <= 225 ? pack_blocks(j->d) : -1;
+}
+
+int pn2_step_tail(int dtype, const pn2_tail_job* jobs_dev, const pn2_pack_job* packs_dev, const int* block_start_dev, int njobs, int total_blocks,
+                  float lr, float beta1, float beta2, float eps, float clip, float grad_scale, const float* bias_corr, float weight_decay, void* stream) {
+    if (!jobs_dev || !packs_dev || !block_start_dev || !bias_corr || njobs < 1 || total_blocks < 1) return -1;
+    if (dtype == PN2_BF16) hipLaunchKernelGGL(step_tail<bf16_t>, dim3(total_blocks), dim3(256), 0, (hipStream_t)stream, jobs_dev, packs_dev, block_start_dev, njobs, lr, beta1, beta2, eps, clip, grad_scale, bias_corr, weight_decay);
+    else if (dtype == PN2_F32) hipLaunchKernelGGL(step_tail<float>, dim3(total_blocks), dim3(256), 0, (hipStream_t)stream, jobs_dev, packs_dev, block_start_dev, njobs, lr, beta1, beta2, eps, clip, grad_scale, bias_corr, weight_decay);
+    else return -3;
+    PN2_CHECK_LAUNCH();
+    return 0;
+}
+
 int pn2_pack_patch_weight(int dtype, const float* w_oihw, void* wp, int Cout, int Cin, int KH, int KW, int Cin_p, int Rp, int Kp, void* stream) {
     if (!w_oihw || !wp || Cin_p < Cin || Rp < KH * KW * Cin_p || Kp < Cout) return -1;
     const size_t total = (size_t)Rp * Kp;
diff --git a/pranet-v2_amd/csrc/pn2_tail.hip b/pranet-v2_amd/csrc/pn2_tail.hip
--- a/pranet-v2_amd/csrc/pn2_tail.hip
+++ b/pranet-v2_amd/csrc/pn2_tail.hip
@@ -1098,29 +1098,7 @@
 
 __global__ __launch_bounds__(256) void clamp_adam_k(float* __restrict__ p, float* __restrict__ g, float* __restrict__ m, float* __restrict__ v, long long n,
                                                     float lr, float b1, float b2, float eps, float clip, float gsc, const float* __restrict__ bc, float wd) {
-    if (bc[7] != 0.f) { lr = bc[4]; clip = bc[5]; wd = bc[6]; }
-    const float step = lr / bc[0], rs2 = 1.f / sqrtf(bc[1]), keep = 1.f - lr * wd;
-    const long long n4 = n >> 2;
-    for (long long i = (long long)blockIdx.x * 256 + threadIdx.x; i < n4; i += (long long)gridDim.x * 256) {
-        float4 P = reinterpret_cast<float4*>(p)[i], G = reinterpret_cast<float4*>(g)[i], Mv = reinterpret_cast<float4*>(m)[i], V = reinterpret_cast<float4*>(v)[i];
-        float* pp = &P.x; float* gg = &G.x; float* mm = &Mv.x; float* vv = &V.x;
-#pragma unroll
-        for (int e = 0; e < 4; ++e) {
-            const float ge = fminf(fmaxf(gg[e] * gsc, -clip), clip);
-            gg[e] = ge;
-            mm[e] = b1 * mm[e] + (1.f - b1) * ge;
-            vv[e] = b2 * vv[e] + (1.f - b2) * ge * ge;
-            pp[e] = pp[e] * keep - step * mm[e] / (sqrtf(vv[e]) * rs2 + eps);
-        }
-        reinterpret_cast<float4*>(p)[i] = P; reinterpret_cast<float4*>(g)[i] = G; reinterpret_cast<float4*>(m)[i] = Mv; reinterpret_cast<float4*>(v)[i] = V;
-    }
-    for (long long i = (n4 << 2) + (long long)blockIdx.x * 256 + threadIdx.x; i < n; i += (long long)gridDim.x * 256) {
-        const float ge = fminf(fmaxf(g[i] * gsc, -clip), clip);
-        g[i] = ge;
-        m[i] = b1 * m[i] + (1.f - b1) * ge;
-        v[i] = b2 * v[i] + (1.f - b2) * ge * ge;
-        p[i] = p[i] * keep - step * m[i] / (sqrtf(v[i]) * rs2 + eps);
-    }
+    clamp_adam_range(p, g, m, v, n, blockIdx.x, gridDim.x, adam_setup(lr, b1, b2, eps, clip, gsc, bc, wd));
 }
 
 __global__ __launch_bounds__(256) void eval_hist_k(const unsigned char* __restrict__ pred, const float* __restrict__ gt, long long n, unsigned* __restrict__ hist) {
diff --git a/pranet-v2_amd/pn2/capi.py b/pranet-v2_amd/pn2/capi.py
--- a/pranet-v2_amd/pn2/capi.py
+++ b/pranet-v2_amd/pn2/capi.py
@@ -36,6 +36,11 @@
 
 class ReduceJob(C.Structure):
     _fields_ = [("slab", C.c_void_p), ("gw", C.c_void_p), ("d", PackDesc), ("nsplit", C.c_int), ("accumulate", C.c_int)]
+
+
+class TailJob(C.Structure):
+    _fields_ = [("slab", C.c_void_p), ("g", C.c_void_p), ("w", C.c_void_p), ("m", C.c_void_p), ("v", C.c_void_p), ("d", PackDesc),
+                ("nsplit", C.c_int), ("accumulate", C.c_int), ("pack0", C.c_int), ("npack", C.c_int), ("n", C.c_longlong)]
 
 
 class ColsumInJob(C.Structure):
@@ -151,6 +156,8 @@
     "pn2_pack_weights_multi": [I, P, P, I, I, P],
     "pn2_wgrad_reduce_blocks": [C.POINTER(PackDesc)],
     "pn2_wgrad_reduce_multi": [P, P, I, I, P],
+    "pn2_step_tail_blocks": [C.POINTER(TailJob)],
+    "pn2_step_tail": [I, P, P, P, I, I, FL, FL, FL, FL, FL, FL, P, FL, P],
     "pn2_bn_finalize": [P, P, I, C.POINTER(BnDesc), P, P, P, P, P, P, P, P, P],
     "pn2_bn_eval_prepare": [C.POINTER(BnDesc), P, P, P, P, P, P, P],
     "pn2_bn_eval_prepare_multi": [P, P, I, I, P],
@@ -264,7 +271,7 @@
 }
 _VALUE_FUNCS = {"pn2_copy_job_blocks", "pn2_conv_gemm_tile", "pn2_conv_gemm_job_blocks", "pn2_bn_finalize_job_blocks", "pn2_affine_job_blocks", "pn2_bn_bwd_finalize_job_blocks",
                 "pn2_bn_bwd_apply_job_blocks", "pn2_bn_bwd_reduce_job_blocks", "pn2_dwconv3x3_colsum_blocks", "pn2_resize_ksize", "pn2_colsum_job_blocks", "pn2_colsum_finalize_blocks", "pn2_dwconv3x3_wgrad_blocks", "pn2_conv_tile_n", "pn2_wgrad_tile_co", "pn2_conv_stat_blocks", "pn2_conv_tile_m", "pn2_bn_bwd_blocks", "pn2_loss_blocks",
-                "pn2_pack_blocks", "pn2_wgrad_reduce_blocks", "pn2_conv_wgrad_variant", "pn2_conv_wgrad_blocks",
+                "pn2_pack_blocks", "pn2_wgrad_reduce_blocks", "pn2_step_tail_blocks", "pn2_conv_wgrad_variant", "pn2_conv_wgrad_blocks",
                 "pn2_dsra_tail_blocks", "pn2_dsra_tail_scratch", "pn2_dsra_tail_fused_ok", "pn2_dsra_tail_fused_scratch", "pn2_ln_slots", "pn2_rows_blocks", "pn2_colsum_unit", "pn2_attn_bwd_blocks", "pn2_mutation_loss_blocks", "pn2_mutation_loss_width", "pn2_seg_loss_width",
                 "pn2_dwconv_blocks", "pn2_pairconv_blocks", "pn2_gate_blocks", "pn2_eval_wfm_blocks", "pn2_seg_surface_hist_len"}
 
diff --git a/pranet-v2_amd/pn2/core.py b/pranet-v2_amd/pn2/core.py
--- a/pranet-v2_amd/pn2/core.py
+++ b/pranet-v2_amd/pn2/core.py
@@ -398,9 +398,11 @@
         self.levels[gw.data_ptr()] = lvl + 1
         self.rjobs.append((slab.data_ptr(), gw.data_ptr(), rd, nsplit, accumulate, lvl))
 
-    def _build(self):
+    def _build(self, hold=None):
         launches = []
         groups = {}
+        last = {j[1]: i for i, j in enumerate(self.rjobs) if hold and j[1] in hold}
+        held = set(last.values())
         for dt, dy, x, slab, wd, ns, fl in self.wjobs:
             v = call.pn2_conv_wgrad_variant(dt, C.byref(wd))
             if v < 0:
@@ -442,10 +444,10 @@
                 arr.append(j)
             table, bstart, nblocks = _job_table(capi.WgradJob, arr, [call.pn2_conv_wgrad_blocks(C.byref(j.d), j.nsplit) for j in arr])
             launches.append(("w", dt, v, table, bstart, len(arr), nblocks, sum(j[5] for j in js)))
-        for lvl in sorted({j[5] for j in self.rjobs}):
+        for lvl in sorted({j[5] for i, j in enumerate(self.rjobs) if i not in held}):
             arr = []
-            for slab, gw, rd, ns, acc, l_ in self.rjobs:
-                if l_ != lvl:
+            for i, (slab, gw, rd, ns, acc, l_) in enumerate(self.rjobs):
+                if l_ != lvl or i in held:
                     continue
                 j = capi.ReduceJob()
                 j.slab, j.gw, j.nsplit, j.accumulate = slab, gw, ns, acc
@@ -453,19 +455,21 @@
                 arr.append(j)
             table, bstart, nblocks = _job_table(capi.ReduceJob, arr, [call.pn2_wgrad_reduce_blocks(C.byref(j.d)) for j in arr])
             launches.append(("r", 0, 0, table, bstart, len(arr), nblocks, 0))
+        launches.append(("h", [self.rjobs[i] for i in sorted(held)]))
         return launches
 
-    def flush(self):
+    def flush(self, hold=None):
         if not self.wjobs and not self.rjobs:
-            return
-        sig = (tuple(j[:4] + (j[5],) for j in self.wjobs), tuple(j[:2] + j[3:] for j in self.rjobs))
-        hit = self.cache.get(self.seg)
+            return []
+        sig = (tuple(j[:4] + (j[5],) for j in self.wjobs), tuple(j[:2] + j[3:] for j in self.rjobs), hold)
+        key = (self.seg, hold is not None)
+        hit = self.cache.get(key)
         if hit is None or hit[0] != sig:
             if torch.cuda.is_current_stream_capturing():
                 raise RuntimeError("run two eager steps before capturing (the deferred-launch tables are built then)")
-            hit = self.cache[self.seg] = (sig, self._build())
+            hit = self.cache[key] = (sig, self._build(hold))
         st = _stream()
-        for kind, dt, v, table, bstart, njobs, nblocks, flops in hit[1]:
+        for kind, dt, v, table, bstart, njobs, nblocks, flops in hit[1][:-1]:
             if kind == "w":
                 capi.WORK.update(flops=flops, tag="", shape=f"variant{v} jobs{njobs}")
                 call.pn2_conv_wgrad_multi(dt, v, _p(table), _p(bstart), njobs, nblocks, st)
@@ -474,3 +478,4 @@
         self.seg += 1
         self.wjobs, self.rjobs, self.keep = [], [], []
         self.levels = {}
+        return hit[1][-1][1]
diff --git a/pranet-v2_amd/pn2/profile.py b/pranet-v2_amd/pn2/profile.py
--- a/pranet-v2_amd/pn2/profile.py
+++ b/pranet-v2_amd/pn2/profile.py
@@ -47,6 +47,8 @@
             return N * HW * 4 * (4 * P + 2)
         if name == "pn2_clamp_adam":
             return int(a[4]) * 4 * 7
+        if name == "pn2_step_tail":
+            return capi.WORK.get("step_tail_bytes", 0)
         if name == "pn2_binary":
             dt, M, C = a[0], a[8], a[9]
             return M * C * _EL[dt] * 3
diff --git a/pranet-v2_amd/pn2/trainer.py b/pranet-v2_amd/pn2/trainer.py
--- a/pranet-v2_amd/pn2/trainer.py
+++ b/pranet-v2_amd/pn2/trainer.py
@@ -3,7 +3,9 @@
 
 import torch
 
-from .capi import call, F32
+from . import capi
+from .capi import call, F32, BF16
+from .core import _job_table
 from .engine import Engine, Act, PackCache, GradQueue, StepArena, TUNER, _p, _stream
 from .graph import get_compute_dtype
 from .dp import GradBuckets
@@ -91,6 +93,10 @@
         self._states = {}
         self._cur = None
         self.fuse_tail = os.environ.get("PN2_FUSED_TAIL", "1") == "1"
+        self.fuse_opt_tail = os.environ.get("PN2_FUSED_OPT_TAIL", "1") == "1" and not self.dp
+        self._tail_plan_cache = (None, None)
+        self._panels_rev = None
+        self._panel_params = ()
         self.tuner = TUNER if os.environ.get("PN2_AUTOTUNE", "1") == "1" else None
         self._tuned = len(self.tuner) if self.tuner is not None else 0
 
@@ -112,6 +118,94 @@
                 if k == 'lr':
                     tr.set_lr(v)
         return [_Group(lr=self.lr, params=self.hot, betas=self.betas, eps=self.eps, weight_decay=self.weight_decay)]
+
+    def invalidate_panels(self):
+        self._panels_rev = None
+
+    def _weights_rev(self):
+        return (self.flat._version, sum(p._version for p in self._panel_params))
+
+    def _tail_plan(self):
+        pc = self.pack_cache
+        if self._tail_plan_cache[0] == pc.version:
+            return self._tail_plan_cache[1]
+        plan = None
+        if pc.jobs and pc.dt in (BF16, F32):
+            base, hot_off = self.flat.data_ptr(), {self.off[id(p)][0]: p for p in self.hot}
+            groups = {}
+            for k, j in enumerate(pc.jobs):
+                groups.setdefault(j.w - base, []).append(k)
+            ok = True
+            for byte_off, ks in groups.items():
+                p = hot_off.get(byte_off // 4) if byte_off % 4 == 0 else None
+                d0 = pc.jobs[ks[0]].d
+                geo = (d0.Cout, d0.Cin, d0.KH, d0.KW)
+                if p is None or p.numel() != geo[0] * geo[1] * geo[2] * geo[3] or any((pc.jobs[k].d.Cout, pc.jobs[k].d.Cin, pc.jobs[k].d.KH, pc.jobs[k].d.KW) != geo for k in ks):
+                    ok = False
+                    break
+            if ok:
+                convs = sorted((b // 4, hot_off[b // 4].numel(), ks) for b, ks in groups.items())
+                plan = (frozenset(self.gflat.data_ptr() + o * 4 for o, _n, _k in convs), convs)
+                self._panel_params = tuple(hot_off[o] for o, _n, _k in convs)
+        self._tail_plan_cache = (pc.version, plan)
+        return plan
+
+    def _tail_table(self, st, plan, held):
+        sig = (self.pack_cache.version, tuple(j[:2] + j[3:5] for j in held))
+        if st.tail_table is not None and st.tail_table[0] == sig:
+            return st.tail_table[1]
+        if torch.cuda.is_current_stream_capturing():
+            raise RuntimeError("run two eager steps before capturing (the step-tail table is built then)")
+        pc = self.pack_cache
+        arenas = [t.data_ptr() for t in (self.gflat, self.flat, self.exp_avg, self.exp_avg_sq)]
+        by_gw = {j[1]: j for j in held}
+        jobs, packs, pos = [], [], 0
+
+        def ptrs(j, o):
+            j.g, j.w, j.m, j.v = (a + o * 4 for a in arenas)
+
+        def range_job(o, n):
+            if n > 0:
+                j = capi.TailJob()
+                ptrs(j, o)
+                j.n = n
+                jobs.append(j)
+        for o, n, ks in plan[1]:
+            range_job(pos, o - pos)
+            j = capi.TailJob()
+            ptrs(j, o)
+            h = by_gw.get(arenas[0] + o * 4)
+            if h is not None:
+                j.slab, j.nsplit, j.accumulate = h[0], h[3], h[4]
+            C.memmove(C.byref(j.d), C.byref(h[2] if h is not None else pc.jobs[ks[0]].d), C.sizeof(capi.PackDesc))
+            j.pack0, j.npack = len(packs), len(ks)
+            packs.extend(pc.jobs[k] for k in ks)
+            jobs.append(j)
+            pos = o + _r4(n)
+        range_job(pos, self.n_hot - pos)
+        table, bstart, nblocks = _job_table(capi.TailJob, jobs, [call.pn2_step_tail_blocks(C.byref(j)) for j in jobs])
+        parr = (capi.PackJob * len(packs))(*packs)
+        ptab = torch.frombuffer(bytearray(bytes(memoryview(parr).cast("B"))), dtype=torch.uint8).to(self.flat.device)
+        if st.tail_table is not None:
+            st.tail_retired.append(st.tail_table)
+        esz = 2 if pc.dt == BF16 else 4
+        nbytes = self.n_hot * 4 * 7 + sum(n * (4 * by_gw[arenas[0] + o * 4][3] if arenas[0] + o * 4 in by_gw else 0) + n * esz * len(ks) for o, n, ks in plan[1])
+        st.tail_table = (sig, (table, ptab, bstart, len(jobs), nblocks, nbytes))
+        return st.tail_table[1]
+
+    def _step_tail(self, st, plan, held):
+        table, ptab, bstart, njobs, nblocks, nbytes = self._tail_table(st, plan, held)
+        capi.WORK["step_tail_bytes"] = nbytes
+        s_ = _stream()
+        call.pn2_adam_tick(_p(self.bias_corr), self.betas[0], self.betas[1], s_)
+        call.pn2_step_tail(self.pack_cache.dt, _p(table), _p(ptab), _p(bstart), njobs, nblocks, self.lr, self.betas[0], self.betas[1], self.eps, self.clip,
+                           1.0 / self.world, _p(self.bias_corr), self.weight_decay, s_)
+        self._panels_rev = self._weights_rev()
+
+    def _sync_panels(self):
+        if self._panels_rev is None or self._panels_rev != self._weights_rev():
+            self.pack_cache.refresh()
+            self._panels_rev = self._weights_rev()
 
     def _grad_view(self, p):
         off, n = self.off[id(p)]
@@ -126,7 +220,7 @@
             mode = os.environ.get("PN2_DEFER_WGRAD", "2")
             st = self._states[key] = SimpleNamespace(
                 key=key, steps_run=0, graph=None, graph_opt=None, segments=None, s_images=None, s_gts=None, s_loss=None,
-                lock_cache={},
+                lock_cache={}, tail_table=None, tail_retired=[], graph_tail=False,
                 grad_queue=GradQueue(defer_wgrad=mode == "2") if mode in ("1", "2") else None,
                 arena=StepArena() if os.environ.get("PN2_STEP_ARENA", "1") == "1" else None)
         self._cur = st
@@ -136,9 +230,16 @@
     grad_queue = property(lambda self: self._cur.grad_queue if self._cur else None)
     steps_run = property(lambda self: self._cur.steps_run if self._cur else 0)
 
-    def forward_backward(self, images, gts, reduce_hook=True, size=None):
+    def forward_backward(self, images, gts, reduce_hook=True, size=None, _tail=False):
         st = self._state(images, size)
-        self.pack_cache.refresh()
+        self._held = None
+        plan = self._tail_plan() if _tail and st.grad_queue is not None else None
+        if plan is not None:
+            self._sync_panels()
+        else:
+            self.pack_cache.refresh()
+            self._panels_rev = None
+        self._plan_now = plan
         if st.arena is not None:
             st.arena.begin_step(self.flat.device)
         st.steps_run += 1
@@ -193,10 +294,9 @@
         if rq is not None:
             rq.begin_step()
 
-        def grads_complete():
+        def grads_complete(hold=None):
             eng.flush_colsum()
-            if rq is not None:
-                rq.flush()
+            return rq.flush(hold) if rq is not None else []
         hook = self.dp and reduce_hook
         expected = self._expected
         if hook and expected is not None:
@@ -221,7 +321,14 @@
         if len(eng.pgrads.written) != len(self.hot):
             missing = [n for n, p in self.model.named_parameters() if id(p) in {id(q) for q in self.hot} and id(p) not in eng.pgrads.written]
             raise RuntimeError(f"{len(missing)} trained parameters received no gradient this step (first: {missing[:3]}): exclude them from `hot`")
-        grads_complete()
+        plan = self._plan_now
+        if plan is not None and self._tail_plan() is not plan:
+            plan = self._tail_plan()
+            if plan is None:
+                raise RuntimeError("the pack cache took a weight outside the trained arena during the step: set PN2_FUSED_OPT_TAIL=0")
+        held = grads_complete(plan[0] if plan is not None else None)
+        if plan is not None:
+            self._held = (plan, held)
         if self.dp:
             if reduce_hook and expected is None:
                 self._expected = dict(eng.pgrads.counts)
@@ -242,10 +349,15 @@
         call.pn2_adam_tick(_p(self.bias_corr), self.betas[0], self.betas[1], st)
         call.pn2_clamp_adam(_p(self.flat), _p(self.gflat), _p(self.exp_avg), _p(self.exp_avg_sq), self.n_hot, self.lr, self.betas[0], self.betas[1],
                             self.eps, self.clip, 1.0 / self.world, _p(self.bias_corr), self.weight_decay, st)
+        self._panels_rev = None
 
     def step(self, images, gts, size=None):
-        loss = self.forward_backward(images, gts, size=size)
-        self.optimizer_step()
+        loss = self.forward_backward(images, gts, size=size, _tail=self.fuse_opt_tail)
+        if self._held is not None:
+            self._step_tail(self._cur, *self._held)
+            self._held = None
+        else:
+            self.optimizer_step()
         return loss
 
     def state_dict(self):
@@ -260,6 +372,7 @@
         if [tuple(x) for x in o["layout"]] != layout:
             raise RuntimeError("optimizer state was saved for a different parameter layout")
         self.model.load_state_dict(sd["model"], strict=True)
+        self.invalidate_panels()
         with torch.no_grad():
             self.exp_avg.copy_(o["exp_avg"]); self.exp_avg_sq.copy_(o["exp_avg_sq"]); self.bias_corr[:4].copy_(o["bias_corr"][:4])
         self.lr, self.betas, self.eps, self.clip, self.weight_decay = o["lr"], tuple(o["betas"]), o["eps"], o["clip"], o["weight_decay"]
@@ -291,9 +404,12 @@
         gc.disable()
         try:
             if not self.dp:
+                if self.fuse_opt_tail and self._tail_plan() is not None:
+                    self._sync_panels()
                 with torch.cuda.graph(st.graph, capture_error_mode=CAPTURE_MODE):
                     st.s_loss = self.step(st.s_images, st.s_gts, size=size)
                 st.graph_opt = None
+                st.graph_tail = self._panels_rev is not None
             elif self._agree(self._capture_with_collectives(st, size)):
                 st.graph_opt, st.segments = None, None
             else:
@@ -406,7 +522,10 @@
             else:
                 st.s_gts.copy_(gts, non_blocking=True)
         if st.graph_opt is None:
+            if st.graph_tail:
+                self._sync_panels()
             st.graph.replay()
+            self._panels_rev = self._weights_rev() if st.graph_tail else None
         elif st.segments:
             self.buckets.reset()
             for g, bs in st.segments:
```

After: 2262 images/sec. -2.6%, worse.
